# tusen-ai/RangeDet

Hardware: AMD Instinct MI355X
Metric: range-image frames/sec (64x2650, 8ch) at 1/2/4/8 GPU; Meta-Kernel HBM GB/s vs peak (higher is better)
Workload: dtype bf16

## Files before the change

### include/rangedet_hip.h

```cpp
#ifndef RANGEDET_HIP_H_
#define RANGEDET_HIP_H_
#include <stddef.h>
#include <stdint.h>

#ifdef __cplusplus
extern "C" {
#endif

#define RD_OK 0
#define RD_EINVAL (-1)
#define RD_ESHAPE (-2)
#define RD_EWORKSPACE (-3)
#define RD_EHIP (-4)

#define RD_F32 0
#define RD_BF16 1
#define RD_F16 2

#define RD_RELU_PRE 1
#define RD_ADD 2
#define RD_RELU_POST 4
#define RD_SCALE_FOLDED 8
#define RD_MFMA16 16

int rd_version(void);
const char* rd_last_error_string(void);

int rd_nchw_to_nhwc(const float* src, void* dst, int B, int C, int H, int W, int dst_cstride, int dst_coff,
                    int zero_pad, int dst_dtype, void* stream);
int rd_nhwc_to_nchw(const void* src, float* dst, int B, int C, int H, int W, int src_cstride, int src_coff,
                    int src_dtype, void* stream);

int rd_copy_rows(const void* src, long src_row_bytes, void* dst, long dst_row_bytes, long dst_offset_bytes, long bytes,
                 int rows, void* stream);

size_t rd_conv_packed_bytes(int ntaps, int cin, int cout, int dtype);
int rd_pack_conv_weight_host(const float* w_oihw_host, int cout, int cin, int kh, int kw, int dtype,
                             void* packed_host);
int rd_deconv_phase_taps(int kh, int kw, int stride_w, int pad_w, int phase);
int rd_pack_deconv_weight_host(const float* w_iohw_host, int cin, int cout, int kh, int kw, int stride_w,
                               int pad_w, int phase, int dtype, void* packed_host);
int rd_pack_deconv_weight_folded_host(const float* w_iohw_host, const float* fold_scale_host, int cin, int cout, int kh, int kw,
                                      int stride_w, int pad_w, int phase, int dtype, void* packed_host);

int rd_conv2d_bn_act(const void* x, int x_cstride, int x_coff, const void* w_packed, const float* scale,
                     const float* shift, const void* residual, int r_cstride, int r_coff, void* y,
                     int y_cstride, int y_coff, int B, int H, int Win, int cin, int cout, int kh, int kw,
                     int stride_w, int flags, int dtype, void* stream);
size_t rd_conv3x3_ex_packed_bytes(int cin, int cout, int stride_w, int x_cstride);
int rd_pack_conv3x3_ex_host(const float* w_oihw_host, const float* fold_scale_host, int cout, int cin, int stride_w,
                            int x_cstride, int dtype, void* packed_host);
int rd_pack_conv3x3_m16_host(const float* w_oihw_host, const float* fold_scale_host, int cout, int cin, int dtype, void* packed_host);
int rd_conv3x3_mfma16_ok(int cin, int cout, int stride_w, int W, int fused_output_conv);
size_t rd_conv1x1_sc_packed_bytes(int cin, int cout);
int rd_pack_conv1x1_sc_host(const float* w_oi_host, const float* fold_scale_host, int cout, int cin, int dtype,
                            void* packed_host);
int rd_conv3x3_bn_act_ex(const void* x, int x_cstride, int x_coff, const void* w_packed, const float* scale, const float* shift,
                         const void* residual, int r_cstride, int r_coff, const void* sc_x, int sc_cstride, int sc_coff,
                         int sc_cin, const void* sc_w_packed, void* y, int y_cstride, int y_coff, int B, int H, int Win, int cin,
                         int cout, int stride_w, int flags, int dtype, void* stream);
size_t rd_block64_packed_bytes(int cin);
int rd_pack_block64_host(const float* w1_oihw_host, const float* fold_scale1_host, const float* w2_oihw_host,
                         const float* fold_scale2_host, int cin, int dtype, void* packed_host);
int rd_block64_bn_act(const void* x, int x_cstride, int x_coff, int cin, const void* w_packed, const float* shift1, const float* shift2,
                      const void* sc_w_packed, void* y, int y_cstride, int y_coff, int B, int H, int W, int dtype, void* stream);
int rd_pack_block64_m16_host(const float* w1_oihw_host, const float* fold_scale1_host, const float* w2_oihw_host,
                             const float* fold_scale2_host, int dtype, void* packed_host);
int rd_pack_conv1x1_sc_m16_host(const float* w_oi_host, const float* fold_scale_host, int dtype, void* packed_host);
int rd_block64_m16_bn_act(const void* x, int x_cstride, int x_coff, const void* w_packed, const float* shift1, const float* shift2,
                          const void* sc_w_packed, void* y, int y_cstride, int y_coff, int B, int H, int W, int dtype, void* stream);

size_t rd_head_packed_bytes(void);
int rd_pack_head_weight_host(const float* w, int nout, int cin, int dtype, void* out_host);
size_t rd_head_m16_packed_bytes(void);
int rd_pack_head_weight_m16_host(const float* w, int nout, int cin, int dtype, void* out_host);
int rd_conv2d_bn_act_head_out(const void* x, int x_cstride, int x_coff, const void* w_packed, const float* scale,
                              const float* shift, int B, int H, int W, int cin, int flags, const void* head_w_packed,
                              const float* head_bias, float* out, long out_batch_stride, long n_off, int nout, int dtype,
                              void* stream);

int rd_conv3x3_bn_act_pair(const void* x0, int x0_coff, const void* w0_packed, const float* shift0, void* y0, int y0_coff,
                           const void* x1, int x1_coff, const void* w1_packed, const float* shift1, void* y1, int y1_coff,
                           int x_cstride, int y_cstride, int B, int H, int W, int cin, int flags, int dtype, void* stream);
int rd_conv2d_bn_act_head_out_pair(const void* x0, int x0_coff, const void* w0_packed, const float* shift0, const void* head_w0_packed,
                                   const float* head_bias0, float* out0, long out0_batch_stride, int nout0,
                                   const void* x1, int x1_coff, const void* w1_packed, const float* shift1, const void* head_w1_packed,
                                   const float* head_bias1, float* out1, long out1_batch_stride, int nout1,
                                   int x_cstride, long n_off, int B, int H, int W, int cin, int flags, int dtype, void* stream);

size_t rd_conv3x3_cat_packed_bytes(int cin1, int cin2, int cout);
int rd_pack_conv3x3_cat_host(const float* w, const float* fold_scale, int cout, int cin1, int cin2, int dtype, void* out_host);
int rd_conv3x3_bn_act_cat(const void* x1, int x1_cstride, int x1_coff, int cin1, const void* x2, int x2_cstride, int x2_coff, int cin2,
                          const void* w_packed, const float* shift, void* y, int y_cstride, int y_coff, int B, int H, int W, int cout,
                          int flags, int dtype, void* stream);

int rd_deconv2d_bn_act(const void* x, int x_cstride, int x_coff, const void* w_packed_phase,
                       const float* scale, const float* shift, const void* residual, int r_cstride,
                       int r_coff, void* y, int y_cstride, int y_coff, int B, int H, int Win, int cin,
                       int cout, int kh, int kw, int stride_w, int pad_w, int phase, int flags, int dtype,
                       void* stream);

int rd_deconv2d_all_phases_ok(int kh, int kw, int stride_w, int pad_w, int cout, int dtype);
int rd_deconv2d_bn_act_all(const void* x, int x_cstride, int x_coff, const void* w_packed_all, long w_phase_bytes,
                           const float* shift, const void* residual, int r_cstride, int r_coff, void* y, int y_cstride,
                           int y_coff, int B, int H, int Win, int cin, int cout, int kh, int kw, int stride_w, int pad_w,
                           int flags, int dtype, void* stream);

int rd_deconv2d_phase_pairs_ok(int kh, int kw, int stride_w, int pad_w, int cout, int dtype);
int rd_pack_deconv_phase_pair_host(const void* phase_a, const void* phase_b, int cin, int dtype, void* out);
int rd_deconv2d_bn_act_pairs(const void* x, int x_cstride, int x_coff, const void* w_packed_pairs, long w_pair_bytes,
                             const float* shift2, const void* residual, int r_cstride, int r_coff, void* y, int y_cstride,
                             int y_coff, int B, int H, int Win, int cin, int cout, int kh, int kw, int stride_w, int pad_w,
                             int flags, int dtype, void* stream);

int rd_head_out(const void* x, int x_cstride, int x_coff, const float* w, const float* bias, float* out,
                long out_batch_stride, long n_off, int B, int H, int W, int cin, int nout, int dtype,
                void* stream);

size_t rd_meta_packed_bytes(int dtype);
int rd_pack_meta_host(const float* w0, const float* b0, const float* w1, const float* b1, const float* s1,
                      const float* t1, const float* agg, const float* s2, const float* t2, int dtype,
                      void* packed_host);
int rd_meta_kernel_fwd(const void* data, int d_cstride, int d_coff, const float* coord_nchw,
                       const void* packed, void* y, int y_cstride, int y_coff, int B, int H, int W, int dtype,
                       void* stream);

size_t rd_sorted_foreground_workspace_bytes(long N, long k);
int rd_sorted_foreground(const float* cls_score, const float* bbox_delta, const float* pc, const float* mask,
                         int B, long N, long k, int D, int apply_sigmoid, float* out_score, float* out_delta,
                         float* out_pc, int* out_idx, void* ws, size_t ws_bytes, void* stream);

int rd_decode3d_bbox(const float* bbox_delta, const float* pc, float* out, int B, long N, int box_type,
                     int is_bin, void* stream);

size_t rd_score_filter_workspace_bytes(long n);
int rd_score_filter_dets(const float* scores, const float* boxes10, long n, float min_score, float* dets,
                         int* d_count, void* ws, size_t ws_bytes, void* stream);
int rd_score_filter_dets_batched(const float* scores, long scores_bstride, const float* boxes10, long boxes_bstride,
                                 long n, float min_score, float* dets, long dets_bstride, int* d_count, void* ws,
                                 size_t ws_bytes, int B, void* stream);

#define RD_WNMS_MAX_K 65536
#define RD_TIE_STABLE 0
#define RD_TIE_REFERENCE 1
#define RD_WNMS_DIAG_NO_SKIP 0x100
#define RD_WNMS_DIAG_TILE_W(n) (((n) & 0xff) << 16)
#define RD_WNMS_DIAG_MERGE_LDS(n) (((n) & 0x7f) << 24)
size_t rd_wnms_workspace_bytes(int Kcap);
int rd_wnms_4c(const float* dets, int Kcap, const int* d_count, const int* order, int tie_order, float thresh,
               float thresh_vote, int is3d, int hash_scale, float* out_dets, int* keep, int* d_nkeep, void* ws,
               size_t ws_bytes, void* stream);
int rd_wnms_4c_batched(const float* dets, long dets_bstride, int Kcap, const int* d_count, const int* order,
                       long order_bstride, int tie_order, float thresh, float thresh_vote, int is3d, int hash_scale,
                       float* out_dets, long out_bstride, int* keep, long keep_bstride, int* d_nkeep, void* ws,
                       size_t ws_bytes, int B, void* stream);
int rd_single_overlap(const float* dets_a, const float* dets_b, long n, int is3d, float* out, void* stream);
int rd_wnms_pair_skippable(const float* dets_a, const float* dets_b, long n, unsigned char* out, void* stream);

int rd_edge_atan2f(const float* y, const float* x, long n, float* out, void* stream);

int rd_wnms_order_host(const float* dets_host, int K, int* order_host);

int rd_dets12_to_8(const float* dets12, int Mcap, const int* d_count, float* out8, void* stream);
int rd_dets12_to_8_batched(const float* dets12, long dets12_bstride, int Mcap, const int* d_count, float* out8,
                           long out8_bstride, int B, void* stream);

int rd_rotated_iou_8pt(const float* boxes1, const float* boxes2, float* ious, long n1, long n2, void* stream);
int rd_batch_rotated_iou(const float* proposal, int p_stride, const float* gt_bbox, float* iou_map, int* argmax, int B, long N,
                         int n_gt, void* stream);
int rd_batch_rotated_iou_3d(const float* proposal, int p_stride, const float* gt_bbox7, float* iou_map, int* argmax, int B, long N,
                            int n_gt, void* stream);
int rd_rotated_iou_7(const float* boxes1, const float* boxes2, float* ious, long n1, long n2, void* stream);
int rd_batch_max_iou(const float* proposals, int p_stride, const float* gt8, float* out, long n, int n_gt,
                     void* stream);

size_t rd_nms3d_workspace_bytes(long N, int B);
int rd_gather_keep_scores(const float* score, long score_bstride, int k, const int* keep_idx, int max_keep, float* out, int B,
                          void* stream);
int rd_nms3d(const float* boxes, int B, long N, float iou_thres, int max_keep, int normal_iou, int* keep_idx,
             float* bbox_after_nms, void* ws, size_t ws_bytes, void* stream);

int rd_assign3d_v2(const float* pc, const float* bbox, const float* bbox_center, const float* bbox_radius, const float* mask,
                   const float* is_in_nlz, long N, int M, float max_x, float min_x, float max_y, float min_y, float max_z,
                   float min_z, float max_dist, int* out, void* stream);
size_t rd_get_point_num_workspace_bytes(void);
int rd_get_point_num(const float* bbox_inds, long N, float* out, void* ws, size_t ws_bytes, void* stream);

typedef struct {
  float clip_lo[7], clip_hi[7];
  float mean[8], sd[8];
  float interval_lo[3], interval_hi[3];
} rd_input_norm_t;
int rd_input_transform(const float* range_image, const float* pc_vehicle_frame, const float* inclination,
                       const rd_input_norm_t* norm_host, int B, int H, int W, int Hp, int Wp, float* input_data,
                       float* coord_s1, float* pc_s1, float* pc_s2, float* pc_s4, float* mask_s1, float* mask_s2,
                       float* mask_s4, void* stream);

typedef struct {
  float *input_data, *coord_s1;
  float *pc[3], *mask[3];
  float *reg_target[3], *reg_weight[3], *reg_normalize_weight[3], *cls_target[3];
  int* bbox3d_ind;
} rd_train_outputs_t;
size_t rd_train_transform_workspace_bytes(int B);
int rd_train_transform(const float* range_image, const float* pc_vehicle_frame, const float* inclination,
                       const rd_input_norm_t* norm_host, const float* gt_bbox_imu, const float* gt_bbox_center,
                       const float* gt_limits, const float* gt_bbox_csa, const int* num_gt_host, int Mmax, float radius,
                       float max_dist, const float* reg_weight_host, int B, int H, int W, int Hp, int Wp,
                       const rd_train_outputs_t* out_host, void* ws, size_t ws_bytes, void* stream);

#define RD_PROF_CONV 0
#define RD_PROF_META 1
#define RD_PROF_HEAD_OUT 2
#define RD_PROF_SORT 3
#define RD_PROF_DECODE 4
#define RD_PROF_WNMS 5
#define RD_PROF_LAYOUT 6
#define RD_PROF_CONV3 7
#define RD_PROF_BLOCK 8
#define RD_PROF_NKINDS 9
int rd_prof_enable(int on);
int rd_prof_reset(void);
int rd_prof_get(int kind, double* total_ms, long* launches);

#ifdef __cplusplus
}
#endif
#endif
```

### rangedet_amd/csrc/k_misc.h

```cpp
#pragma once
#include "rd_common.h"

namespace rd {

template <int DT>
__global__ __launch_bounds__(256) void nchw_to_nhwc_kernel(const float* __restrict__ src, void* __restrict__ dst_, int C,
                                                           long HW, int cs, int coff, int cpad, long total) {
  using E = Elem<DT>;
  typename E::T* dst = (typename E::T*)dst_;
  const int ctot = C + cpad;
  for (long i = blockIdx.x * 256L + threadIdx.x; i < total; i += (long)gridDim.x * 256) {
    long p = i % HW;
    long rest = i / HW;
    int c = (int)(rest % ctot);
    long b = rest / ctot;
    float v = c < C ? src[(b * C + c) * HW + p] : 0.f;
    dst[(b * HW + p) * cs + coff + c] = E::from_f32(v);
  }
}
template <int DT, int NSLOT>
__global__ __launch_bounds__(256) void nchw_to_nhwc_px_kernel(const float* __restrict__ src, void* __restrict__ dst_, int C,
                                                              long HW, int cs, int coff, long npix) {
  using E = Elem<DT>;
  typename E::T* dst = (typename E::T*)dst_;
  for (long i = blockIdx.x * 256L + threadIdx.x; i < npix; i += (long)gridDim.x * 256) {
    const long b = i / HW, p = i - b * HW;
    typename E::T v[NSLOT * E::CH];
#pragma unroll
    for (int c = 0; c < NSLOT * E::CH; ++c) v[c] = E::from_f32(c < C ? src[(b * C + c) * HW + p] : 0.f);
    Slot16 pk[NSLOT];
    memcpy(pk, v, sizeof(pk));
#pragma unroll
    for (int u = 0; u < NSLOT; ++u) *(Slot16*)(dst + i * cs + coff + u * E::CH) = pk[u];
  }
}
template <int DT>
__global__ __launch_bounds__(256) void nhwc_to_nchw_kernel(const void* __restrict__ src_, float* __restrict__ dst, int C,
                                                           long HW, int cs, int coff, long total) {
  using E = Elem<DT>;
  const typename E::T* src = (const typename E::T*)src_;
  for (long i = blockIdx.x * 256L + threadIdx.x; i < total; i += (long)gridDim.x * 256) {
    long p = i % HW;
    long rest = i / HW;
    int c = (int)(rest % C);
    long b = rest / C;
    dst[(b * C + c) * HW + p] = E::to_f32(src[(b * HW + p) * cs + coff + c]);
  }
}

template <int DT, int NOUT>
__global__ __launch_bounds__(256) void head_out_kernel(const void* __restrict__ x_, int cs, int coff,
                                                       const float* __restrict__ w, const float* __restrict__ bias,
                                                       float* __restrict__ out, long out_bs, long n_off, long HW,
                                                       int cin) {
  using E = Elem<DT>;
  using T = typename E::T;
  __shared__ float wl[8 * 128];
  const T* x = (const T*)x_ + (size_t)blockIdx.y * HW * cs;
  for (int i = threadIdx.x; i < NOUT * cin; i += 256) wl[i] = w[i];
  __syncthreads();
  const int sub = threadIdx.x & 7;
  const int per = cin >> 3;
  const long npix_iter = (long)gridDim.x * 32;
  for (long p0 = blockIdx.x * 32L; p0 < HW; p0 += npix_iter) {
    long p = p0 + (threadIdx.x >> 3);
    float acc[NOUT];
#pragma unroll
    for (int o = 0; o < NOUT; ++o) acc[o] = 0.f;
    if (p < HW) {
      const T* px = x + p * cs + coff + sub * per;
      if ((per % E::CH) == 0) {
        for (int c0 = 0; c0 < per; c0 += E::CH) {
          const Slot16 raw = *(const Slot16*)(px + c0);
          T el[E::CH];
          memcpy(el, &raw, 16);
#pragma unroll
          for (int e = 0; e < E::CH; ++e) {
            const float v = E::to_f32(el[e]);
#pragma unroll
            for (int o = 0; o < NOUT; ++o) acc[o] += v * wl[o * cin + sub * per + c0 + e];
          }
        }
      } else {
        for (int c = 0; c < per; ++c) {
          float v = E::to_f32(px[c]);
#pragma unroll
          for (int o = 0; o < NOUT; ++o) acc[o] += v * wl[o * cin + sub * per + c];
        }
      }
    }
#pragma unroll
    for (int o = 0; o < NOUT; ++o) {
      acc[o] += __shfl_xor(acc[o], 1);
      acc[o] += __shfl_xor(acc[o], 2);
      acc[o] += __shfl_xor(acc[o], 4);
    }
    if (p < HW && sub == 0) {
      float* o_ = out + (size_t)blockIdx.y * out_bs + (n_off + p) * NOUT;
#pragma unroll
      for (int o = 0; o < NOUT; ++o) o_[o] = acc[o] + bias[o];
    }
  }
}

template <int NOUT, int DT = RD_BF16>
__global__ __launch_bounds__(256) void head_out_mfma_kernel(const bf16_t* __restrict__ x, int cs, int coff,
                                                            const float* __restrict__ w, const float* __restrict__ bias,
                                                            float* __restrict__ out, long out_bs, long n_off, long HW,
                                                            int cin) {
  __shared__ __attribute__((aligned(16))) unsigned char lds[4 * 8192];
  const int lane = threadIdx.x & 63, m = lane & 31, hi = lane >> 5, wv = threadIdx.x >> 6;
  unsigned char* img = lds + wv * 8192;
  const int nks = cin >> 4, nsl = cin >> 3;
  x += (size_t)blockIdx.y * HW * cs + coff;
  out += (size_t)blockIdx.y * out_bs + n_off * NOUT;
  s16x8 wh[8], wl[8];
#pragma unroll
  for (int ks = 0; ks < 8; ++ks) {
    unsigned short h[8], l[8];
#pragma unroll
    for (int j = 0; j < 8; ++j) {
      const float v = (m < NOUT && ks < nks) ? w[m * cin + ks * 16 + hi * 8 + j] : 0.f;
      h[j] = H16<DT>::from_f32(v);
      l[j] = H16<DT>::from_f32(v - H16<DT>::to_f32(h[j]));
    }
    memcpy(&wh[ks], h, 16);
    memcpy(&wl[ks], l, 16);
  }
  float bs[4];
#pragma unroll
  for (int r = 0; r < 4; ++r) bs[r] = 4 * hi + r < NOUT ? bias[4 * hi + r] : 0.f;
  const long ntile = (HW + 31) / 32;
  const long wave0 = (long)blockIdx.x * 4 + wv, nwave = (long)gridDim.x * 4;
  const int lp = lane >> 4, ls = lane & 15;
  auto load = [&](long tile, Slot16 (&v)[8]) {
#pragma unroll
    for (int it = 0; it < 8; ++it) {
      const long p = min(tile * 32 + it * 4 + lp, HW - 1);
      v[it] = ls < nsl ? *(const Slot16*)(x + p * cs + ls * 8) : Slot16{0u, 0u, 0u, 0u};
    }
  };
  Slot16 cur[8], nxt[8];
  if (wave0 < ntile) load(wave0, cur);
  for (long tile = wave0; tile < ntile; tile += nwave) {
    const bool more = tile + nwave < ntile;
    if (more) load(tile + nwave, nxt);
#pragma unroll
    for (int it = 0; it < 8; ++it) {
      const int pr = it * 4 + lp;
      *(Slot16*)(img + pr * 256 + ((ls ^ (pr & 15)) << 4)) = cur[it];
    }
    __builtin_amdgcn_wave_barrier();
    f32x16 acc;
#pragma unroll
    for (int r = 0; r < 16; ++r) acc[r] = 0.f;
#pragma unroll
    for (int ks = 0; ks < 8; ++ks) {
      const s16x8 b = *(const s16x8*)(img + m * 256 + (((2 * ks + hi) ^ (m & 15)) << 4));
      acc = H16<DT>::mfma(wl[ks], b, acc);
      acc = H16<DT>::mfma(wh[ks], b, acc);
    }
    __builtin_amdgcn_wave_barrier();
    const long p = tile * 32 + m;
    if (p < HW) {
      float* o = out + p * NOUT + 4 * hi;
#pragma unroll
      for (int r = 0; r < 4; ++r)
        if (4 * hi + r < NOUT) o[r] = acc[r] + bs[r];
    }
    if (more) {
#pragma unroll
      for (int it = 0; it < 8; ++it) cur[it] = nxt[it];
    }
  }
}

__global__ __launch_bounds__(256) void decode3d_kernel(const float* __restrict__ delta, const float* __restrict__ pc,
                                                       float* __restrict__ out, long n, int box_type, int is_bin) {
  long idx = blockIdx.x * 256L + threadIdx.x;
  if (idx >= n) return;
  const float* d = delta + idx * box_type;
  float pc_x = pc[idx * 3 + 0], pc_y = pc[idx * 3 + 1], pc_z = pc[idx * 3 + 2];
  float az = atan2f(pc_y, pc_x);
  float ca = cosf(az), sa = sinf(az);
  float dx, dy, width, length, height, z0, yaw_l;
  if (is_bin) {
    dx = d[0];
    dy = d[1];
    width = expf(d[3]);
    length = expf(d[4]);
    height = expf(d[5]);
    float cz = pc_z + d[2];
    z0 = (float)((double)cz - (double)height / 2.0);
    yaw_l = d[6] + az;
  } else {
    dx = d[0] * fabsf(d[0]);
    dy = d[1] * fabsf(d[1]);
    width = expf(d[2]);
    length = expf(d[3]);
    height = expf(d[7]);
    z0 = d[6];
    yaw_l = atan2f(d[5], d[4]) + az;
  }
  float dxl = dx * ca - dy * sa;
  float dyl = dx * sa + dy * ca;
  float cx = pc_x + dxl, cy = pc_y + dyl;
  float sy = sinf(yaw_l), cyw = cosf(yaw_l);
  float hl = (float)(0.5 * (double)length), hw = (float)(0.5 * (double)width);
  float hx[4] = {hl, -hl, -hl, hl};
  float hy[4] = {-hw, -hw, hw, hw};
  float* o = out + idx * 10;
#pragma unroll
  for (int k = 0; k < 4; ++k) {
    o[2 * k] = (hx[k] * cyw - hy[k] * sy) + cx;
    o[2 * k + 1] = (hx[k] * sy + hy[k] * cyw) + cy;
  }
  o[8] = z0;
  o[9] = z0 + height;
}

__global__ __launch_bounds__(256) void filter_count_kernel(const float* __restrict__ scores, long n, float thr,
                                                           int* __restrict__ blk_cnt, long sc_bs, long blk_bs) {
  scores += blockIdx.y * sc_bs;
  blk_cnt += blockIdx.y * blk_bs;
  long i = blockIdx.x * 256L + threadIdx.x;
  int p = (i < n) && (scores[i] > thr);
  unsigned long long m = __ballot(p);
  __shared__ int wc[4];
  if ((threadIdx.x & 63) == 0) wc[threadIdx.x >> 6] = __popcll(m);
  __syncthreads();
  if (threadIdx.x == 0) blk_cnt[blockIdx.x] = wc[0] + wc[1] + wc[2] + wc[3];
}
__global__ __launch_bounds__(256) void filter_scan_kernel(int* __restrict__ blk_cnt, int nblk, int* __restrict__ total,
                                                          long blk_bs) {
  blk_cnt += blockIdx.x * blk_bs;
  total += blockIdx.x;
  __shared__ int part[256];
  __shared__ int carry;
  if (threadIdx.x == 0) carry = 0;
  __syncthreads();
  for (int base = 0; base < nblk; base += 256) {
    int i = base + threadIdx.x;
    int v = i < nblk ? blk_cnt[i] : 0;
    part[threadIdx.x] = v;
    __syncthreads();
    for (int off = 1; off < 256; off <<= 1) {
      int t = threadIdx.x >= off ? part[threadIdx.x - off] : 0;
      __syncthreads();
      part[threadIdx.x] += t;
      __syncthreads();
    }
    int incl = part[threadIdx.x];
    if (i < nblk) blk_cnt[i] = carry + incl - v;
    __syncthreads();
    if (threadIdx.x == 255) carry += incl;
    __syncthreads();
  }
  if (threadIdx.x == 0) *total = carry;
}
__global__ __launch_bounds__(256) void filter_scatter_kernel(const float* __restrict__ scores,
                                                             const float* __restrict__ boxes10, long n, float thr,
                                                             const int* __restrict__ blk_off, float* __restrict__ dets,
                                                             long sc_bs, long box_bs, long blk_bs, long dets_bs) {
  scores += blockIdx.y * sc_bs;
  boxes10 += blockIdx.y * box_bs;
  blk_off += blockIdx.y * blk_bs;
  dets += blockIdx.y * dets_bs;
  long i = blockIdx.x * 256L + threadIdx.x;
  int p = (i < n) && (scores[i] > thr);
  unsigned long long m = __ballot(p);
  __shared__ int wc[4];
  const int wv = threadIdx.x >> 6, ln = threadIdx.x & 63;
  if (ln == 0) wc[wv] = __popcll(m);
  __syncthreads();
  int off = blk_off[blockIdx.x];
  for (int w = 0; w < wv; ++w) off += wc[w];
  if (p) {
    int pos = off + __popcll(m & ((1ull << ln) - 1ull));
    const float* b = boxes10 + i * 10;
    float* d = dets + (size_t)pos * 12;
#pragma unroll
    for (int k = 0; k < 8; ++k) d[k] = b[k];
    d[8] = fdlibm_atan2f(b[1] - b[3], b[0] - b[2]);
    d[9] = b[8];
    d[10] = b[9] - b[8];
    d[11] = scores[i];
  }
}

__global__ __launch_bounds__(256) void dets12_to_8_kernel(const float* __restrict__ d12, int cap, const int* __restrict__ d_count,
                                                          float* __restrict__ o8, long d12_bs, long o8_bs) {
  d12 += blockIdx.y * d12_bs;
  o8 += blockIdx.y * o8_bs;
  int i = blockIdx.x * 256 + threadIdx.x;
  int n = d_count ? min(d_count[blockIdx.y], cap) : cap;
  if (i >= n) return;
  const float* d = d12 + (size_t)i * 12;
  float* o = o8 + (size_t)i * 8;
  o[0] = (d[0] + d[2] + d[4] + d[6]) / 4.f;
  o[1] = (d[1] + d[3] + d[5] + d[7]) / 4.f;
  o[2] = d[9] + d[10] / 2.f;
  float ax = d[2] - d[0], ay = d[3] - d[1];
  float bx = d[2] - d[4], by = d[3] - d[5];
  o[3] = sqrtf(ax * ax + ay * ay);
  o[4] = sqrtf(bx * bx + by * by);
  o[5] = d[10];
  o[6] = d[8];
  o[7] = d[11];
}

__global__ __launch_bounds__(256) void gather_keep_scores_kernel(const float* __restrict__ score, long score_bs, int k,
                                                                 const int* __restrict__ keep, int mk, float* __restrict__ out) {
  const int i = blockIdx.x * 256 + threadIdx.x;
  if (i >= mk) return;
  const int q = keep[(size_t)blockIdx.y * mk + i];
  out[(size_t)blockIdx.y * mk + i] = (q >= 0 && q < k) ? score[blockIdx.y * score_bs + q] : -__builtin_inff();
}

}
```

### rangedet_amd/csrc/k_sort.h

```cpp
#pragma once
#include "rd_common.h"

namespace rd {

constexpr int SORT_TILE = 2048;

__device__ __forceinline__ unsigned desc_key(float f) {
  unsigned u = __float_as_uint(f);
  unsigned asc = u ^ ((u >> 31) ? 0xFFFFFFFFu : 0x80000000u);
  return ~asc;
}
__device__ __forceinline__ float key_to_float(unsigned key) {
  unsigned asc = ~key;
  unsigned u = (asc >> 31) ? (asc ^ 0x80000000u) : ~asc;
  return __uint_as_float(u);
}

__global__ __launch_bounds__(256) void sort_keygen_kernel(const float* __restrict__ score, const float* __restrict__ mask,
                                                          long N, int apply_sigmoid, unsigned* __restrict__ keys,
                                                          unsigned* __restrict__ idx, long ws_stride) {
  long i = blockIdx.x * 256L + threadIdx.x;
  if (i >= N) return;
  const long b = blockIdx.y;
  float s = score[b * N + i];
  if (apply_sigmoid) s = 1.0f / (1.0f + expf(-s));
  if (mask) s = s * mask[b * N + i];
  keys[b * ws_stride + i] = desc_key(s);
  idx[b * ws_stride + i] = (unsigned)i;
}
__global__ __launch_bounds__(256) void sort_keygen_dets_kernel(const float* __restrict__ dets, int cap,
                                                               const int* __restrict__ d_count, unsigned* __restrict__ keys,
                                                               unsigned* __restrict__ idx) {
  int i = blockIdx.x * 256 + threadIdx.x;
  if (i >= cap) return;
  int n = d_count ? min(*d_count, cap) : cap;
  keys[i] = i < n ? desc_key(dets[(size_t)i * 12 + 11]) : 0xFFFFFFFFu;
  idx[i] = (unsigned)i;
}

__global__ __launch_bounds__(256) void sort_hist_kernel(const unsigned* __restrict__ keys, long N, int shift,
                                                        unsigned* __restrict__ hist, unsigned* __restrict__ tot,
                                                        long ws_stride, const unsigned* __restrict__ d_n) {
  if (d_n) N = min(N, (long)d_n[blockIdx.y * ws_stride]);
  keys += blockIdx.y * ws_stride;
  hist += blockIdx.y * ws_stride;
  tot += blockIdx.y * ws_stride;
  __shared__ unsigned h[256];
  h[threadIdx.x] = 0;
  __syncthreads();
  long base = (long)blockIdx.x * SORT_TILE;
  for (int r = 0; r < SORT_TILE / 256; ++r) {
    long i = base + r * 256 + threadIdx.x;
    if (i < N) atomicAdd(&h[(keys[i] >> shift) & 255u], 1u);
  }
  __syncthreads();
  unsigned v = h[threadIdx.x];
  hist[(size_t)blockIdx.x * 256 + threadIdx.x] = v;
  if (v) atomicAdd(&tot[threadIdx.x], v);
}

__global__ __launch_bounds__(256) void sort_scatter_kernel(const unsigned* __restrict__ keys_in,
                                                           const unsigned* __restrict__ idx_in, long N, int shift,
                                                           const unsigned* __restrict__ hist,
                                                           const unsigned* __restrict__ tot,
                                                           unsigned* __restrict__ keys_out, unsigned* __restrict__ idx_out,
                                                           long ws_stride, const unsigned* __restrict__ d_n) {
  if (d_n) {
    N = min(N, (long)d_n[blockIdx.y * ws_stride]);
    if ((long)blockIdx.x * SORT_TILE >= N) return;
  }
  {
    const long o = blockIdx.y * ws_stride;
    keys_in += o; idx_in += o; hist += o; tot += o; keys_out += o; idx_out += o;
  }
  __shared__ unsigned wcnt[4][256];
  __shared__ unsigned gbase[256];
  __shared__ unsigned scan[256];
  const int tid = threadIdx.x, lane = tid & 63, wv = tid >> 6;
  for (int w = 0; w < 4; ++w) wcnt[w][tid] = 0;
  {
    unsigned t = tot[tid];
    scan[tid] = t;
    __syncthreads();
    for (int off = 1; off < 256; off <<= 1) {
      unsigned a = tid >= off ? scan[tid - off] : 0u;
      __syncthreads();
      scan[tid] += a;
      __syncthreads();
    }
    unsigned before = 0;
    for (unsigned b = 0; b < blockIdx.x; ++b) before += hist[(size_t)b * 256 + tid];
    gbase[tid] = scan[tid] - t + before;
  }
  __syncthreads();

  unsigned key[8], id[8], pos[8];
  const long base = (long)blockIdx.x * SORT_TILE + wv * 512;
  const unsigned long long lt = (1ull << lane) - 1ull;
#pragma unroll
  for (int r = 0; r < 8; ++r) {
    long i = base + r * 64 + lane;
    bool valid = i < N;
    key[r] = valid ? keys_in[i] : 0xFFFFFFFFu;
    id[r] = valid ? idx_in[i] : 0u;
    unsigned d = (key[r] >> shift) & 255u;
    unsigned long long peers = __ballot(valid);
#pragma unroll
    for (int bit = 0; bit < 8; ++bit) {
      unsigned long long bm = __ballot(valid && ((d >> bit) & 1u));
      peers &= ((d >> bit) & 1u) ? bm : ~bm;
    }
    unsigned rank = __popcll(peers & lt), cnt = __popcll(peers);
    unsigned prev = wcnt[wv][d];
    pos[r] = prev + rank;
    __builtin_amdgcn_wave_barrier();
    if (valid && rank == 0) wcnt[wv][d] = prev + cnt;
    __builtin_amdgcn_wave_barrier();
  }
  __syncthreads();
  {
    unsigned c0 = wcnt[0][tid], c1 = wcnt[1][tid], c2 = wcnt[2][tid];
    wcnt[0][tid] = 0;
    wcnt[1][tid] = c0;
    wcnt[2][tid] = c0 + c1;
    wcnt[3][tid] = c0 + c1 + c2;
  }
  __syncthreads();
#pragma unroll
  for (int r = 0; r < 8; ++r) {
    long i = base + r * 64 + lane;
    if (i < N) {
      unsigned d = (key[r] >> shift) & 255u;
      unsigned dst = gbase[d] + wcnt[wv][d] + pos[r];
      keys_out[dst] = key[r];
      idx_out[dst] = id[r];
    }
  }
}

__global__ __launch_bounds__(256) void sort_gather_kernel(const unsigned* __restrict__ keys, const unsigned* __restrict__ idx,
                                                          long k, int D, const float* __restrict__ delta,
                                                          const float* __restrict__ pc, float* __restrict__ out_score,
                                                          float* __restrict__ out_delta, float* __restrict__ out_pc,
                                                          int* __restrict__ out_idx, long ws_stride, long N) {
  long i = blockIdx.x * 256L + threadIdx.x;
  if (i >= k) return;
  {
    const long b = blockIdx.y;
    keys += b * ws_stride; idx += b * ws_stride;
    delta += b * N * D; pc += b * N * 3;
    out_score += b * k; out_delta += b * k * D; out_pc += b * k * 3;
    if (out_idx) out_idx += b * k;
  }
  unsigned j = idx[i];
// ... 18 lines not shown
    if (i < N) atomicAdd(&h[keys[i] >> SEL_SHIFT], 1u);
  }
  __syncthreads();
  for (int i = threadIdx.x; i < SEL_BINS; i += 256)
    if (h[i]) atomicAdd(&h12[i], h[i]);
}
__global__ __launch_bounds__(256) void select_thresh_kernel(const unsigned* __restrict__ h12, long k, unsigned* __restrict__ sel,
                                                            long ws_stride) {
  h12 += blockIdx.y * ws_stride; sel += blockIdx.y * ws_stride;
  __shared__ unsigned part[256];
  const int tid = threadIdx.x;
  unsigned loc[SEL_BINS / 256], sum = 0;
#pragma unroll
  for (int j = 0; j < SEL_BINS / 256; ++j) { loc[j] = h12[tid * (SEL_BINS / 256) + j]; sum += loc[j]; }
  part[tid] = sum;
  __syncthreads();
  for (int off = 1; off < 256; off <<= 1) {
    const unsigned v = tid >= off ? part[tid - off] : 0u;
    __syncthreads();
    part[tid] += v;
    __syncthreads();
  }
  unsigned before = part[tid] - sum;
  if (tid == 255 && (k == 0 || part[255] < (unsigned)k)) { sel[0] = SEL_BINS - 1; sel[1] = part[255]; }
  if (before < (unsigned)k && before + sum >= (unsigned)k) {
#pragma unroll
    for (int j = 0; j < SEL_BINS / 256; ++j) {
      if (before < (unsigned)k && before + loc[j] >= (unsigned)k) { sel[0] = tid * (SEL_BINS / 256) + j; sel[1] = before + loc[j]; }
      before += loc[j];
    }
  }
}
__global__ __launch_bounds__(256) void select_count_kernel(const unsigned* __restrict__ keys, long N, const unsigned* __restrict__ sel,
                                                           unsigned* __restrict__ cnt, long ws_stride) {
  keys += blockIdx.y * ws_stride; sel += blockIdx.y * ws_stride; cnt += blockIdx.y * ws_stride;
  const unsigned T = sel[0];
  __shared__ unsigned c;
  if (threadIdx.x == 0) c = 0;
  __syncthreads();
  const long base = (long)blockIdx.x * SORT_TILE;
  unsigned mine = 0;
  for (int r = 0; r < SORT_TILE / 256; ++r) {
    const long i = base + r * 256 + threadIdx.x;
    if (i < N && (keys[i] >> SEL_SHIFT) <= T) ++mine;
  }
  if (mine) atomicAdd(&c, mine);
  __syncthreads();
  if (threadIdx.x == 0) cnt[blockIdx.x] = c;
}
__global__ __launch_bounds__(256) void select_compact_kernel(const unsigned* __restrict__ keys_in, const unsigned* __restrict__ idx_in,
                                                             long N, const unsigned* __restrict__ sel,
                                                             const unsigned* __restrict__ cnt, unsigned* __restrict__ keys_out,
                                                             unsigned* __restrict__ idx_out, long ws_stride) {
  {
    const long o = blockIdx.y * ws_stride;
    keys_in += o; idx_in += o; sel += o; cnt += o; keys_out += o; idx_out += o;
  }
  const unsigned T = sel[0];
  __shared__ unsigned wcnt[4][8], sbase;
  const int tid = threadIdx.x, lane = tid & 63, wv = tid >> 6;
  if (tid == 0) {
    unsigned b = 0;
    for (unsigned j = 0; j < blockIdx.x; ++j) b += cnt[j];
    sbase = b;
  }
  const long base = (long)blockIdx.x * SORT_TILE + wv * 512;
  unsigned key[8], id[8];
  unsigned long long m[8];
#pragma unroll
  for (int r = 0; r < 8; ++r) {
    const long i = base + r * 64 + lane;
    const bool valid = i < N;
    key[r] = valid ? keys_in[i] : 0xFFFFFFFFu;
    id[r] = valid ? idx_in[i] : 0u;
    m[r] = __ballot(valid && (key[r] >> SEL_SHIFT) <= T);
    if (lane == 0) wcnt[wv][r] = (unsigned)__popcll(m[r]);
  }
  __syncthreads();
  unsigned off = sbase;
  for (int w = 0; w < wv; ++w)
#pragma unroll
    for (int r = 0; r < 8; ++r) off += wcnt[w][r];
#pragma unroll
  for (int r = 0; r < 8; ++r) {
    if ((m[r] >> lane) & 1ull) {
      const unsigned dst = off + (unsigned)__popcll(m[r] & ((1ull << lane) - 1ull));
      keys_out[dst] = key[r];
      idx_out[dst] = id[r];
    }
    off += (unsigned)__popcll(m[r]);
  }
}

struct SortWs {
  unsigned *keysA, *keysB, *idxA, *idxB, *hist, *tot, *h12, *cnt, *sel;
  int nblk;
};
inline size_t sort_ws_bytes(long N) {
  long nblk = (N + SORT_TILE - 1) / SORT_TILE;
  return (size_t)(4 * N + nblk * 256 + 4 * 256 + SEL_BINS + nblk + 64) * 4 + 256;
}
inline SortWs sort_ws_carve(void* ws, long N) {
  SortWs s;
  s.nblk = (int)((N + SORT_TILE - 1) / SORT_TILE);
  unsigned* p = (unsigned*)ws;
  s.keysA = p; p += N;
  s.keysB = p; p += N;
  s.idxA = p; p += N;
  s.idxB = p; p += N;
  s.hist = p; p += (size_t)s.nblk * 256;
  s.tot = p; p += 4 * 256;
  s.h12 = p; p += SEL_BINS;
  s.cnt = p; p += s.nblk;
  s.sel = p;
  return s;
}
inline int sort_clear(const SortWs& s, hipStream_t st, int nb, long ws_stride, bool with_h12) {
  const size_t bytes = (size_t)(4 * 256 + (with_h12 ? SEL_BINS : 0)) * 4;
  const hipError_t e = nb > 1 ? hipMemset2DAsync(s.tot, (size_t)ws_stride * 4, 0, bytes, nb, st) : hipMemsetAsync(s.tot, 0, bytes, st);
  return e == hipSuccess ? RD_OK : fail(RD_EHIP, "sort: memset");
}
inline int radix_sort_pairs(const SortWs& s, long N, hipStream_t st, int nb = 1, long ws_stride = 0, const unsigned* d_n = nullptr,
                            bool cleared = false) {
  if (!cleared) { int rc = sort_clear(s, st, nb, ws_stride, false); if (rc != RD_OK) return rc; }
  unsigned *ki = s.keysA, *ko = s.keysB, *ii = s.idxA, *io = s.idxB;
  for (int pass = 0; pass < 4; ++pass) {
    hipLaunchKernelGGL(sort_hist_kernel, dim3(s.nblk, nb), dim3(256), 0, st, ki, N, pass * 8, s.hist, s.tot + pass * 256,
                       ws_stride, d_n);
    hipLaunchKernelGGL(sort_scatter_kernel, dim3(s.nblk, nb), dim3(256), 0, st, ki, ii, N, pass * 8, s.hist,
                       s.tot + pass * 256, ko, io, ws_stride, d_n);
    std::swap(ki, ko);
    std::swap(ii, io);
  }
  return check_launch("radix_sort_pairs");
}

inline int radix_topk_pairs(const SortWs& s, long N, long k, hipStream_t st, int nb, long ws_stride, unsigned** rk, unsigned** ri) {
  const bool off = dev_switches().sort_no_select;
  *rk = s.keysA; *ri = s.idxA;
  RD_REQUIRE(k > 0 && k <= N, RD_ESHAPE, "top-k: k %ld of N %ld", k, N);
  if (off || 2 * k > N) return radix_sort_pairs(s, N, st, nb, ws_stride);
  { int rc = sort_clear(s, st, nb, ws_stride, true); if (rc != RD_OK) return rc; }
  hipLaunchKernelGGL(select_hist_kernel, dim3(s.nblk, nb), dim3(256), 0, st, s.keysA, N, s.h12, ws_stride);
  hipLaunchKernelGGL(select_thresh_kernel, dim3(1, nb), dim3(256), 0, st, s.h12, k, s.sel, ws_stride);
  hipLaunchKernelGGL(select_count_kernel, dim3(s.nblk, nb), dim3(256), 0, st, s.keysA, N, s.sel, s.cnt, ws_stride);
  hipLaunchKernelGGL(select_compact_kernel, dim3(s.nblk, nb), dim3(256), 0, st, s.keysA, s.idxA, N, s.sel, s.cnt, s.keysB, s.idxB,
                     ws_stride);
  SortWs v = s;
  v.keysA = s.keysB; v.keysB = s.keysA; v.idxA = s.idxB; v.idxB = s.idxA;
  *rk = s.keysB; *ri = s.idxB;
  return radix_sort_pairs(v, N, st, nb, ws_stride, s.sel + 1, true);
}

}
```

### rangedet_amd/csrc/rd_api.hip

```cpp
#include "k_conv1.h"
#include "k_block.h"
#include "k_assign.h"
#include "k_input.h"
#include "k_target.h"
#include "k_nms3d.h"
#include "k_meta.h"
#include "k_misc.h"
#include "k_riou.h"
#include "k_sort.h"
#include "k_wnms.h"

#include <algorithm>
#include <string>
#include <numeric>

using namespace rd;

namespace rd {
inline size_t align256(size_t v) { return (v + 255) & ~(size_t)255; }
inline size_t wnms_ws_bytes(int cap) {
  const size_t nw = (size_t)(cap + 63) / 64;
  return align256((size_t)cap * PREP_F * 4) + 3 * align256((size_t)cap * nw * 8) + 4 * align256((size_t)cap * 4) +
         align256(((size_t)cap + 2) * 8 + 3 * ((size_t)cap / 32 + 2) * 4) + align256(nw * 8) + 256 + align256(sort_ws_bytes(cap)) + 256;
}
// ... 544 lines not shown
  allow_conv_lds();
  Conv3Phases ph;
  ph.nph = stride_w / 2; ph.ts_mask = 0; ph.y_pc = 2 * cout; ph.r_pc = 2 * cout; ph.w_pb = w_pair_bytes;
  for (int p = 0; p < stride_w; p += 2)
    if (deconv_tap_set(deconv_taps_sorted(kh, kw, stride_w, pad_w, p)) == 2) ph.ts_mask |= 1 << (p / 2);
  return launch_conv3(x, x_cstride, x_coff, w_packed_pairs, nullptr, shift2, residual, r_cstride * stride_w, r_coff, y, y_cstride * stride_w,
                      y_coff, B, H, Win, cin, 2 * cout, flags, 1, (hipStream_t)stream, 3, nullptr, dtype, nullptr, &ph);
}

int rd_head_out(const void* x, int x_cstride, int x_coff, const float* w, const float* bias, float* out,
                long out_batch_stride, long n_off, int B, int H, int W, int cin, int nout, int dtype, void* stream) {
  RD_REQUIRE(x && w && bias && out, RD_EINVAL, "head_out: null pointer");
  RD_REQUIRE(cin % 8 == 0 && cin <= 128 && cin > 0, RD_ESHAPE, "head_out: cin %d (multiple of 8, <= 128)", cin);
  RD_REQUIRE(nout == 1 || nout == 7 || nout == 8, RD_ESHAPE, "head_out: nout %d not in {1,7,8}", nout);
  RD_REQUIRE(dtype == RD_F32 || is_h16(dtype), RD_EINVAL, "head_out: dtype");
  hipStream_t st = (hipStream_t)stream;
  const long HW = (long)H * W;
  dim3 grid((unsigned)std::min<long>((HW + 31) / 32, 4096), B);
  ProfScope ps(RD_PROF_HEAD_OUT, st);
  if (is_h16(dtype) && nout > 1 && cin % 16 == 0 && x_cstride % 8 == 0 && x_coff % 8 == 0) {
    dim3 g2((unsigned)std::min<long>((HW + 127) / 128, 2048), B);
#define RD_HOM(NO, DT_) hipLaunchKernelGGL((head_out_mfma_kernel<NO, DT_>), g2, dim3(256), 0, st, (const bf16_t*)x, x_cstride, x_coff, w, bias, out, out_batch_stride, n_off, HW, cin)
    if (dtype == RD_F16) { if (nout == 7) RD_HOM(7, RD_F16); else RD_HOM(8, RD_F16); }
    else { if (nout == 7) RD_HOM(7, RD_BF16); else RD_HOM(8, RD_BF16); }
#undef RD_HOM
    return check_launch("head_out");
  }
#define RD_HO(DT, NO) hipLaunchKernelGGL((head_out_kernel<DT, NO>), grid, dim3(256), 0, st, x, x_cstride, x_coff, w, bias, out, out_batch_stride, n_off, HW, cin)
  if (dtype == RD_BF16) { if (nout == 1) RD_HO(RD_BF16, 1); else if (nout == 7) RD_HO(RD_BF16, 7); else RD_HO(RD_BF16, 8); }
  else if (dtype == RD_F16) { if (nout == 1) RD_HO(RD_F16, 1); else if (nout == 7) RD_HO(RD_F16, 7); else RD_HO(RD_F16, 8); }
  else { if (nout == 1) RD_HO(RD_F32, 1); else if (nout == 7) RD_HO(RD_F32, 7); else RD_HO(RD_F32, 8); }
#undef RD_HO
  return check_launch("head_out");
}

size_t rd_meta_packed_bytes(int dtype) { return meta_layout(dtype).total; }
int rd_pack_meta_host(const float* w0, const float* b0, const float* w1, const float* b1, const float* s1,
                      const float* t1, const float* agg, const float* s2, const float* t2, int dtype, void* out) {
  RD_REQUIRE(w0 && b0 && w1 && b1 && s1 && t1 && agg && s2 && t2 && out, RD_EINVAL, "pack_meta: null pointer");
  RD_REQUIRE(dtype == RD_F32 || is_h16(dtype), RD_EINVAL, "pack_meta: dtype");
  pack_meta(w0, b0, w1, b1, s1, t1, agg, s2, t2, dtype, out);
  return RD_OK;
}
int rd_meta_kernel_fwd(const void* data, int d_cstride, int d_coff, const float* coord_nchw, const void* packed,
                       void* y, int y_cstride, int y_coff, int B, int H, int W, int dtype, void* stream) {
  RD_REQUIRE(data && coord_nchw && packed && y, RD_EINVAL, "meta_kernel: null pointer");
  RD_REQUIRE(B > 0 && H > 0 && W > 0, RD_ESHAPE, "meta_kernel: empty shape");
  RD_REQUIRE(dtype == RD_F32 || is_h16(dtype), RD_EINVAL, "meta_kernel: dtype");
  const int ch = ch_per_slot(dtype);
  RD_REQUIRE(d_cstride % ch == 0 && d_coff % ch == 0 && y_cstride % ch == 0 && y_coff % ch == 0, RD_ESHAPE,
             "meta_kernel: channel strides/offsets must be 16-byte multiples");
  RD_REQUIRE(d_coff + 64 <= d_cstride && y_coff + 64 <= y_cstride, RD_ESHAPE, "meta_kernel: needs 64 channels");
  hipStream_t st = (hipStream_t)stream;
  MetaArgs a;
  a.data = data; a.d_cs = d_cstride; a.d_co = d_coff; a.coord = coord_nchw; a.packed = (const unsigned char*)packed;
  a.y = y; a.y_cs = y_cstride; a.y_co = y_coff; a.B = B; a.H = H; a.W = W;
  constexpr int WAVES = 8;
  a.tiles_h = (H + WAVES - 1) / WAVES;
  a.tiles_w = (W + 31) / 32;
  a.ntiles = B * a.tiles_h * a.tiles_w;
  a.r0 = 0; a.m0 = a.m1 = a.m2 = 0;
  const size_t consts = 9 * 64 * 4 * 2 + 1024;
  ProfScope ps(RD_PROF_META, st);
  if (is_h16(dtype)) {
    const size_t lds = meta_layout(dtype).wbytes + consts + (size_t)(WAVES + 2) * 34 * 128 + 4096;
    static std::atomic<unsigned long long> seen{0};
    once_per_device(seen, [] { allow_big_lds(meta16_kernel<WAVES, RD_BF16>); allow_big_lds(meta16_kernel<WAVES, RD_F16>); });
    const dim3 mgrid(std::min(a.ntiles, conv_num_cus())), mblock(WAVES * 64);
    const int strips = a.tiles_w * B;
    a.r0 = dev_switches().conv_xcd && strips % 8 == 0 ? 8 : strips;
    RD_REQUIRE((unsigned long long)a.ntiles * (unsigned)std::max(a.r0, std::max(a.tiles_h, a.tiles_w)) < (1ull << 32), RD_ESHAPE,
               "meta_kernel: %d tiles exceed the range of the tile decode", a.ntiles);
    a.m0 = meta_magic(a.r0); a.m1 = meta_magic(a.tiles_h); a.m2 = meta_magic(a.tiles_w);
    RD_REQUIRE((long)H * W < (1l << 23) && (long)H * W * d_cstride < (1l << 31) && W < (1 << 23) && d_cstride < (1 << 23), RD_ESHAPE,
               "meta_kernel: image of %d x %d pixels x %d channels exceeds the 32-bit halo offsets", H, W, d_cstride);
    if (dtype == RD_F16) hipLaunchKernelGGL((meta16_kernel<WAVES, RD_F16>), mgrid, mblock, lds, st, a);
    else hipLaunchKernelGGL((meta16_kernel<WAVES, RD_BF16>), mgrid, mblock, lds, st, a);
  } else {
    const size_t lds = consts + (size_t)(WAVES + 2) * 34 * 256;
    static std::atomic<unsigned long long> seen32{0};
    once_per_device(seen32, [] { allow_big_lds(meta_kernel<RD_F32, WAVES>); });
    hipLaunchKernelGGL((meta_kernel<RD_F32, WAVES>), dim3(std::min(a.ntiles, 512)), dim3(WAVES * 64), lds, st, a);
  }
  return check_launch("meta_kernel");
}

size_t rd_sorted_foreground_workspace_bytes(long N, long k) { (void)k; return (sort_ws_bytes(N) + 256 + 255) & ~(size_t)255; }
int rd_sorted_foreground(const float* cls_score, const float* bbox_delta, const float* pc, const float* mask, int B,
                         long N, long k, int D, int apply_sigmoid, float* out_score, float* out_delta, float* out_pc,
                         int* out_idx, void* ws, size_t ws_bytes, void* stream) {
  RD_REQUIRE(cls_score && bbox_delta && pc && out_score && out_delta && out_pc && ws, RD_EINVAL, "sorted_foreground: null pointer");
  RD_REQUIRE(B > 0 && N > 0 && k > 0 && D > 0, RD_ESHAPE, "sorted_foreground: empty shape");
  RD_REQUIRE(N >= k, RD_ESHAPE, "sorted_foreground: N (%ld) < num_fgs (%ld)", N, k);
  RD_REQUIRE(N < (1L << 31), RD_ESHAPE, "sorted_foreground: N too large");
  RD_REQUIRE(ws_bytes >= rd_sorted_foreground_workspace_bytes(N, k), RD_EWORKSPACE, "sorted_foreground: workspace %zu < %zu",
             ws_bytes, rd_sorted_foreground_workspace_bytes(N, k));
  hipStream_t st = (hipStream_t)stream;
  void* wsa = (void*)(((uintptr_t)ws + 255) & ~(uintptr_t)255);
  SortWs s = sort_ws_carve(wsa, N);
  ProfScope ps(RD_PROF_SORT, st);
  const size_t per = rd_sorted_foreground_workspace_bytes(N, k);
  const bool wide = ws_bytes >= per * (size_t)B;
  const long stride = wide ? (long)(per / 4) : 0;
  const int nb = wide ? B : 1;
  for (int b0 = 0; b0 < B; b0 += nb) {
    hipLaunchKernelGGL(sort_keygen_kernel, dim3((unsigned)((N + 255) / 256), nb), dim3(256), 0, st, cls_score + (size_t)b0 * N,
                       mask ? mask + (size_t)b0 * N : nullptr, N, apply_sigmoid, s.keysA, s.idxA, stride);
    unsigned *rk, *ri;
    int rc = radix_topk_pairs(s, N, k, st, nb, stride, &rk, &ri);
    if (rc != RD_OK) return rc;
    hipLaunchKernelGGL(sort_gather_kernel, dim3((unsigned)((k + 255) / 256), nb), dim3(256), 0, st, rk, ri, k, D,
                       bbox_delta + (size_t)b0 * N * D, pc + (size_t)b0 * N * 3, out_score + (size_t)b0 * k,
                       out_delta + (size_t)b0 * k * D, out_pc + (size_t)b0 * k * 3, out_idx ? out_idx + (size_t)b0 * k : nullptr,
                       stride, N);
  }
  return check_launch("sorted_foreground");
}

int rd_decode3d_bbox(const float* bbox_delta, const float* pc, float* out, int B, long N, int box_type, int is_bin,
                     void* stream) {
  RD_REQUIRE(bbox_delta && pc && out, RD_EINVAL, "decode3d: null pointer");
  RD_REQUIRE(B > 0 && N > 0, RD_ESHAPE, "decode3d: empty shape");
  RD_REQUIRE((is_bin && box_type == 7) || (!is_bin && box_type == 8), RD_ESHAPE,
             "decode3d: box_type %d with is_bin=%d (8 for regular, 7 for bin)", box_type, is_bin);
  hipStream_t st = (hipStream_t)stream;
  const long n = (long)B * N;
  ProfScope ps(RD_PROF_DECODE, st);
  hipLaunchKernelGGL(decode3d_kernel, dim3((unsigned)((n + 255) / 256)), dim3(256), 0, st, bbox_delta, pc, out, n, box_type, is_bin);
  return check_launch("decode3d");
}

size_t rd_score_filter_workspace_bytes(long n) { return (size_t)((n + 255) / 256 + 8) * 4 + 256; }
int rd_score_filter_dets_batched(const float* scores, long scores_bstride, const float* boxes10, long boxes_bstride,
                                 long n, float min_score, float* dets, long dets_bstride, int* d_count, void* ws,
                                 size_t ws_bytes, int B, void* stream) {
  RD_REQUIRE(scores && boxes10 && dets && d_count && ws, RD_EINVAL, "score_filter: null pointer");
  RD_REQUIRE(n > 0 && B > 0, RD_ESHAPE, "score_filter: empty input");
  const size_t per = rd_score_filter_workspace_bytes(n);
  RD_REQUIRE(ws_bytes >= per * (size_t)B, RD_EWORKSPACE, "score_filter: workspace %zu < %zu", ws_bytes, per * (size_t)B);
  hipStream_t st = (hipStream_t)stream;
  int* blk = (int*)(((uintptr_t)ws + 255) & ~(uintptr_t)255);
  const int nblk = (int)((n + 255) / 256);
  const long blk_bs = nblk + 8;
  ProfScope ps(RD_PROF_WNMS, st);
  hipLaunchKernelGGL(filter_count_kernel, dim3(nblk, B), dim3(256), 0, st, scores, n, min_score, blk, scores_bstride, blk_bs);
  hipLaunchKernelGGL(filter_scan_kernel, dim3(B), dim3(256), 0, st, blk, nblk, d_count, blk_bs);
  hipLaunchKernelGGL(filter_scatter_kernel, dim3(nblk, B), dim3(256), 0, st, scores, boxes10, n, min_score, blk, dets,
                     scores_bstride, boxes_bstride, blk_bs, dets_bstride);
  return check_launch("score_filter");
}
int rd_score_filter_dets(const float* scores, const float* boxes10, long n, float min_score, float* dets, int* d_count,
                         void* ws, size_t ws_bytes, void* stream) {
  return rd_score_filter_dets_batched(scores, 0, boxes10, 0, n, min_score, dets, 0, d_count, ws, ws_bytes, 1, stream);
}

size_t rd_wnms_workspace_bytes(int Kcap) { return Kcap > 0 ? wnms_ws_bytes(Kcap) : 0; }
int rd_wnms_4c_batched(const float* dets, long dets_bstride, int Kcap, const int* d_count, const int* order,
                       long order_bstride, int tie_order, float thresh, float thresh_vote, int is3d, int hash_scale,
                       float* out_dets, long out_bstride, int* keep, long keep_bstride, int* d_nkeep, void* ws,
                       size_t ws_bytes, int B, void* stream) {
  RD_REQUIRE(dets && out_dets && keep && d_nkeep && ws, RD_EINVAL, "wnms_4c: null pointer");
  RD_REQUIRE(Kcap > 0 && Kcap <= RD_WNMS_MAX_K, RD_ESHAPE, "wnms_4c: Kcap %d not in [1, %d]", Kcap, RD_WNMS_MAX_K);
  RD_REQUIRE(B > 0, RD_ESHAPE, "wnms_4c: batch %d", B);
  const int diag = tie_order & ~0xff;
  tie_order &= 0xff;
  RD_REQUIRE(tie_order == RD_TIE_STABLE || tie_order == RD_TIE_REFERENCE, RD_EINVAL, "wnms_4c: tie_order %d", tie_order);
  RD_REQUIRE(!(diag & ~(RD_WNMS_DIAG_NO_SKIP | (0xff << 16) | (0x7f << 24))), RD_EINVAL, "wnms_4c: unknown diagnostic bits 0x%x", diag);
  const size_t per = rd_wnms_workspace_bytes(Kcap);
  RD_REQUIRE(ws_bytes >= per * (size_t)B, RD_EWORKSPACE, "wnms_4c: workspace %zu < %zu", ws_bytes, per * (size_t)B);
  RD_REQUIRE(order || B == 1 || tie_order == RD_TIE_REFERENCE, RD_EINVAL,
             "wnms_4c: the batched call needs an explicit processing order or RD_TIE_REFERENCE");
  hipStream_t st = (hipStream_t)stream;
  static std::atomic<unsigned long long> seen_lds{0};
  once_per_device(seen_lds, [] {
    allow_big_lds(wnms_tie_order_kernel); allow_big_lds(wnms_scan_kernel); allow_big_lds(wnms_scan4_kernel); allow_big_lds(wnms_merge_kernel);
  });
  WnmsWs w = wnms_ws_carve(ws, Kcap);
  ProfScope ps(RD_PROF_WNMS, st);
  WnmsBatch bs;
  bs.dets = dets_bstride; bs.order = order_bstride; bs.prep = (long)(per / 4); bs.words = (long)(per / 8);
  bs.ints = (long)(per / 4); bs.keep = keep_bstride; bs.out = out_bstride;
  const int* ord = order;
  if (!ord && tie_order == RD_TIE_REFERENCE) {
    const size_t lds = TIE_STACK_BYTES + (Kcap <= TIE_LDS_K ? (size_t)Kcap * 8 + 3 * ((size_t)Kcap / 32 + 2) * 4 : 0);
    hipLaunchKernelGGL(wnms_tie_order_kernel, dim3(1, 1, B), dim3(256), lds, st, dets, Kcap, d_count, w.order, bs, (long)(per / 4),
                       w.scratch);
    ord = w.order;
    bs.order = (long)(per / 4);
  } else if (!ord) {
    void* swa = (void*)(((uintptr_t)w.sort_ws + 255) & ~(uintptr_t)255);
    SortWs s = sort_ws_carve(swa, Kcap);
    hipLaunchKernelGGL(sort_keygen_dets_kernel, dim3((Kcap + 255) / 256), dim3(256), 0, st, dets, Kcap, d_count, s.keysA, s.idxA);
    int rc = radix_sort_pairs(s, Kcap, st);
    if (rc != RD_OK) return rc;
    if (hipMemcpyAsync(w.order, s.idxA, (size_t)Kcap * 4, hipMemcpyDeviceToDevice, st) != hipSuccess)
      return rd::fail(RD_EHIP, "wnms_4c: order copy");
    ord = w.order;
    bs.order = 0;
  }
  const int nb = (Kcap + 63) / 64;
  hipLaunchKernelGGL(wnms_prep_kernel, dim3((Kcap + 255) / 256, 1, B), dim3(256), 0, st, dets, ord, Kcap, d_count, w.prep, bs,
                     (float)hash_scale, w.novf);
  const int e_tw = (diag >> 16) & 0xff, e_ml = (diag >> 24) & 0x7f;
  const int tile_w = std::min(w.nwcap, e_tw ? std::max(1, e_tw) : 256);
  const size_t scan_lds = ((size_t)w.nwcap + (size_t)64 * tile_w) * 8;
  const int R1 = 256, nb1 = R1 / 64;
  const bool one_round = dev_switches().wnms_one_round;
  const bool two = Kcap >= 4 * R1 && !one_round;
  const int ct = dev_switches().wnms_ct == 32 ? 32 : dev_switches().wnms_ct == 16 ? 16 : 8;
  const int pgrid = std::min(2048, std::max(64, nb * (64 / ct) * std::min(nb, 16)));
  const int allow_skip = thresh >= 1e-3f && thresh_vote >= 1e-3f && !is3d && !dev_switches().wnms_no_skip && !(diag & RD_WNMS_DIAG_NO_SKIP);
  auto pairs = [&](const int* rows, const int* nrows, const unsigned long long* supp, int rb_end) {
    auto k = dev_switches().wnms_bal ? (ct == 8 ? wnms_pairs_kernel<8, true> : ct == 16 ? wnms_pairs_kernel<16, true> : wnms_pairs_kernel<32, true>)
                                     : (ct == 8 ? wnms_pairs_kernel<8, false> : ct == 16 ? wnms_pairs_kernel<16, false> : wnms_pairs_kernel<32, false>);
    hipLaunchKernelGGL(k, dim3(pgrid, 1, B), dim3(64), 0, st, w.prep, Kcap, d_count, thresh, thresh_vote, is3d, w.thr, w.vote,
                       w.nwcap, bs, rows, nrows, supp, 0, rb_end, allow_skip);
  };
  pairs(nullptr, nullptr, nullptr, two ? nb1 : nb);
  const bool scan4 = w.nwcap <= 128 && !e_tw && !dev_switches().wnms_scan1;
  const int tile_words = 64 * 128;
  const size_t scan4_lds = ((size_t)w.nwcap + tile_words) * 8;
  auto scan = [&](int c_begin, int c_end, unsigned long long* state) {
    if (scan4)
      hipLaunchKernelGGL(wnms_scan4_kernel, dim3(1, 1, B), dim3(256), scan4_lds, st, w.thr, w.snap, Kcap, d_count, w.nwcap, ord,
                         w.keep_q, keep, d_nkeep, bs, c_begin, c_end, state, tile_words);
    else
      hipLaunchKernelGGL(wnms_scan_kernel, dim3(1, 1, B), dim3(64), scan_lds, st, w.thr, w.snap, Kcap, d_count, w.nwcap, ord,
                         w.keep_q, keep, d_nkeep, bs, c_begin, c_end, state, tile_w);
  };
  scan(0, two ? nb1 : nb, two ? w.supp_state : (unsigned long long*)nullptr);
  if (two) {
    hipLaunchKernelGGL(wnms_alive_kernel, dim3(1, 1, B), dim3(256), 0, st, w.supp_state, Kcap, d_count, R1, w.alive, w.nalive, bs);
    pairs((const int*)w.alive, (const int*)w.nalive, (const unsigned long long*)w.supp_state, 0);
    scan(nb1, nb, w.supp_state);
  }
  const int lds_cap = std::min(Kcap + 2, e_ml ? std::max(4, e_ml) : 2048);
  hipLaunchKernelGGL(wnms_merge_kernel, dim3(std::min(Kcap, 4096), 1, B), dim3(64), (size_t)lds_cap * 8, st, dets, ord, w.vote,
                     w.snap, Kcap, d_count, w.nwcap, w.keep_q, d_nkeep, out_dets, bs, lds_cap, w.ovf, w.novf);
  if (Kcap + 2 > lds_cap)
    hipLaunchKernelGGL(wnms_merge_big_kernel, dim3(1, 1, B), dim3(64), 0, st, dets, ord, w.vote, w.snap, Kcap, d_count, w.nwcap,
                       w.keep_q, out_dets, bs, (const int*)w.ovf, (const int*)w.novf, w.scratch);
  return check_launch("wnms_4c");
}
int rd_wnms_4c(const float* dets, int Kcap, const int* d_count, const int* order, int tie_order, float thresh,
               float thresh_vote, int is3d, int hash_scale, float* out_dets, int* keep, int* d_nkeep, void* ws,
               size_t ws_bytes, void* stream) {
  return rd_wnms_4c_batched(dets, 0, Kcap, d_count, order, 0, tie_order, thresh, thresh_vote, is3d, hash_scale, out_dets, 0,
                            keep, 0, d_nkeep, ws, ws_bytes, 1, stream);
}
int rd_single_overlap(const float* dets_a, const float* dets_b, long n, int is3d, float* out, void* stream) {
  RD_REQUIRE(n >= 0 && (n == 0 || (dets_a && dets_b && out)), RD_EINVAL, "single_overlap: bad arguments");
  if (n == 0) return RD_OK;
  hipLaunchKernelGGL(single_overlap_kernel, dim3((unsigned)((n + 63) / 64)), dim3(64), 0, (hipStream_t)stream, dets_a, dets_b, n,
                     is3d, out);
  return check_launch("single_overlap");
}
int rd_wnms_pair_skippable(const float* dets_a, const float* dets_b, long n, unsigned char* out, void* stream) {
  RD_REQUIRE(dets_a && dets_b && out && n >= 0, RD_EINVAL, "wnms_pair_skippable: null pointer");
  if (n == 0) return RD_OK;
  hipLaunchKernelGGL(pair_skippable_kernel, dim3((unsigned)((n + 63) / 64)), dim3(64), 0, (hipStream_t)stream, dets_a, dets_b, n, out);
  return check_launch("wnms_pair_skippable");
}
namespace rd {
__global__ void atan2f_kernel(const float* y, const float* x, long n, float* out) {
  const long i = (long)blockIdx.x * blockDim.x + threadIdx.x;
  if (i < n) out[i] = fdlibm_atan2f(y[i], x[i]);
}
}
int rd_edge_atan2f(const float* y, const float* x, long n, float* out, void* stream) {
  RD_REQUIRE(y && x && out && n >= 0, RD_EINVAL, "edge_atan2f: null pointer");
  if (n == 0) return RD_OK;
  hipLaunchKernelGGL(atan2f_kernel, dim3((unsigned)((n + 255) / 256)), dim3(256), 0, (hipStream_t)stream, y, x, n, out);
  return check_launch("edge_atan2f");
}
int rd_wnms_order_host(const float* dets_host, int K, int* order_host) {
  RD_REQUIRE(K >= 0 && (K == 0 || (dets_host && order_host)), RD_EINVAL, "wnms_order_host: bad arguments");
  std::iota(order_host, order_host + K, 0);
  std::sort(order_host, order_host + K, [&](int i, int j) { return dets_host[i * 12 + 11] > dets_host[j * 12 + 11]; });
  return RD_OK;
}

int rd_dets12_to_8_batched(const float* dets12, long dets12_bstride, int Mcap, const int* d_count, float* out8,
                           long out8_bstride, int B, void* stream) {
  RD_REQUIRE(dets12 && out8, RD_EINVAL, "dets12_to_8: null pointer");
  RD_REQUIRE(Mcap > 0 && B > 0, RD_ESHAPE, "dets12_to_8: empty input");
  hipLaunchKernelGGL(dets12_to_8_kernel, dim3((Mcap + 255) / 256, B), dim3(256), 0, (hipStream_t)stream, dets12, Mcap, d_count,
                     out8, dets12_bstride, out8_bstride);
  return check_launch("dets12_to_8");
}
int rd_dets12_to_8(const float* dets12, int Mcap, const int* d_count, float* out8, void* stream) {
  return rd_dets12_to_8_batched(dets12, 0, Mcap, d_count, out8, 0, 1, stream);
}

int rd_gather_keep_scores(const float* score, long score_bstride, int k, const int* keep_idx, int max_keep, float* out, int B,
                          void* stream) {
  RD_REQUIRE(score && keep_idx && out, RD_EINVAL, "gather_keep_scores: null pointer");
  RD_REQUIRE(k > 0 && max_keep > 0 && B > 0, RD_ESHAPE, "gather_keep_scores: empty input");
  hipLaunchKernelGGL(gather_keep_scores_kernel, dim3((max_keep + 255) / 256, B), dim3(256), 0, (hipStream_t)stream, score,
                     score_bstride, k, keep_idx, max_keep, out);
  return check_launch("gather_keep_scores");
}

int rd_rotated_iou_8pt(const float* boxes1, const float* boxes2, float* ious, long n1, long n2, void* stream) {
  RD_REQUIRE(boxes1 && boxes2 && ious, RD_EINVAL, "rotated_iou: null pointer");
  RD_REQUIRE(n1 > 0 && n2 > 0, RD_ESHAPE, "rotated_iou: empty input");
  hipLaunchKernelGGL(riou8_kernel, dim3((unsigned)((n1 * n2 + 255) / 256)), dim3(256), 0, (hipStream_t)stream, boxes1, boxes2, ious, n1, n2);
// ... 184 lines not shown
```

### rangedet_amd/lib.py

```python
import ctypes
import os

import numpy as np

RD_OK, RD_EINVAL, RD_ESHAPE, RD_EWORKSPACE, RD_EHIP = 0, -1, -2, -3, -4
RD_F32, RD_BF16, RD_F16 = 0, 1, 2
H16 = (RD_BF16, RD_F16)
RD_RELU_PRE, RD_ADD, RD_RELU_POST, RD_SCALE_FOLDED, RD_MFMA16 = 1, 2, 4, 8, 16
RD_WNMS_MAX_K = 65536
RD_WNMS_DIAG_NO_SKIP = 0x100


def RD_WNMS_DIAG_TILE_W(n):
    return (n & 0xff) << 16


def RD_WNMS_DIAG_MERGE_LDS(n):
    return (n & 0x7f) << 24

RD_TIE_STABLE, RD_TIE_REFERENCE = 0, 1
PROF_KINDS = {"conv": 0, "meta": 1, "head_out": 2, "sort": 3, "decode": 4, "wnms": 5, "layout": 6, "conv3": 7, "block": 8}

_HERE = os.path.dirname(os.path.abspath(__file__))
DEFAULT_PATH = os.environ.get("RANGEDET_HIP_LIB") or os.path.join(_HERE, "librangedet_hip.so")

c_int, c_long, c_float, c_size_t, c_void_p = ctypes.c_int, ctypes.c_long, ctypes.c_float, ctypes.c_size_t, ctypes.c_void_p

SIGNATURES = {
    "rd_version": (c_int, []),
    "rd_last_error_string": (ctypes.c_char_p, []),
    "rd_nchw_to_nhwc": (c_int, [c_void_p, c_void_p, c_int, c_int, c_int, c_int, c_int, c_int, c_int, c_int, c_void_p]),
    "rd_nhwc_to_nchw": (c_int, [c_void_p, c_void_p, c_int, c_int, c_int, c_int, c_int, c_int, c_int, c_void_p]),
    "rd_copy_rows": (c_int, [c_void_p, c_long, c_void_p, c_long, c_long, c_long, c_int, c_void_p]),
    "rd_conv_packed_bytes": (c_size_t, [c_int, c_int, c_int, c_int]),
    "rd_pack_conv_weight_host": (c_int, [c_void_p, c_int, c_int, c_int, c_int, c_int, c_void_p]),
    "rd_deconv_phase_taps": (c_int, [c_int, c_int, c_int, c_int, c_int]),
    "rd_pack_deconv_weight_host": (c_int, [c_void_p, c_int, c_int, c_int, c_int, c_int, c_int, c_int, c_int, c_void_p]),
    "rd_pack_deconv_weight_folded_host": (c_int, [c_void_p, c_void_p, c_int, c_int, c_int, c_int, c_int, c_int, c_int, c_int, c_void_p]),
    "rd_conv2d_bn_act": (c_int, [c_void_p, c_int, c_int, c_void_p, c_void_p, c_void_p, c_void_p, c_int, c_int, c_void_p,
                                 c_int, c_int, c_int, c_int, c_int, c_int, c_int, c_int, c_int, c_int, c_int, c_int, c_void_p]),
    "rd_conv3x3_ex_packed_bytes": (c_size_t, [c_int, c_int, c_int, c_int]),
    "rd_pack_conv3x3_ex_host": (c_int, [c_void_p, c_void_p, c_int, c_int, c_int, c_int, c_int, c_void_p]),
    "rd_pack_conv3x3_m16_host": (c_int, [c_void_p, c_void_p, c_int, c_int, c_int, c_void_p]),
    "rd_conv3x3_mfma16_ok": (c_int, [c_int, c_int, c_int, c_int, c_int]),
    "rd_conv1x1_sc_packed_bytes": (c_size_t, [c_int, c_int]),
    "rd_pack_conv1x1_sc_host": (c_int, [c_void_p, c_void_p, c_int, c_int, c_int, c_void_p]),
    "rd_conv3x3_bn_act_ex": (c_int, [c_void_p, c_int, c_int, c_void_p, c_void_p, c_void_p, c_void_p, c_int, c_int, c_void_p, c_int,
                                     c_int, c_int, c_void_p, c_void_p, c_int, c_int, c_int, c_int, c_int, c_int, c_int, c_int,
                                     c_int, c_int, c_void_p]),
    "rd_deconv2d_bn_act": (c_int, [c_void_p, c_int, c_int, c_void_p, c_void_p, c_void_p, c_void_p, c_int, c_int, c_void_p,
                                   c_int, c_int, c_int, c_int, c_int, c_int, c_int, c_int, c_int, c_int, c_int, c_int,
                                   c_int, c_int, c_void_p]),
    "rd_conv3x3_cat_packed_bytes": (c_size_t, [c_int, c_int, c_int]),
    "rd_pack_conv3x3_cat_host": (c_int, [c_void_p, c_void_p, c_int, c_int, c_int, c_int, c_void_p]),
    "rd_conv3x3_bn_act_cat": (c_int, [c_void_p, c_int, c_int, c_int, c_void_p, c_int, c_int, c_int, c_void_p, c_void_p, c_void_p, c_int, c_int,
                                      c_int, c_int, c_int, c_int, c_int, c_int, c_void_p]),
    "rd_deconv2d_all_phases_ok": (c_int, [c_int, c_int, c_int, c_int, c_int, c_int]),
    "rd_deconv2d_bn_act_all": (c_int, [c_void_p, c_int, c_int, c_void_p, c_long, c_void_p, c_void_p, c_int, c_int, c_void_p,
                                       c_int, c_int, c_int, c_int, c_int, c_int, c_int, c_int, c_int, c_int, c_int, c_int,
                                       c_int, c_void_p]),
    "rd_deconv2d_phase_pairs_ok": (c_int, [c_int, c_int, c_int, c_int, c_int, c_int]),
    "rd_pack_deconv_phase_pair_host": (c_int, [c_void_p, c_void_p, c_int, c_int, c_void_p]),
    "rd_deconv2d_bn_act_pairs": (c_int, [c_void_p, c_int, c_int, c_void_p, c_long, c_void_p, c_void_p, c_int, c_int, c_void_p,
                                         c_int, c_int, c_int, c_int, c_int, c_int, c_int, c_int, c_int, c_int, c_int, c_int,
                                         c_int, c_void_p]),
    "rd_block64_packed_bytes": (c_size_t, [c_int]),
    "rd_pack_block64_host": (c_int, [c_void_p, c_void_p, c_void_p, c_void_p, c_int, c_int, c_void_p]),
    "rd_pack_block64_m16_host": (c_int, [c_void_p, c_void_p, c_void_p, c_void_p, c_int, c_void_p]),
    "rd_pack_conv1x1_sc_m16_host": (c_int, [c_void_p, c_void_p, c_int, c_void_p]),
    "rd_block64_m16_bn_act": (c_int, [c_void_p, c_int, c_int, c_void_p, c_void_p, c_void_p, c_void_p, c_void_p, c_int, c_int, c_int, c_int,
                                      c_int, c_int, c_void_p]),
    "rd_block64_bn_act": (c_int, [c_void_p, c_int, c_int, c_int, c_void_p, c_void_p, c_void_p, c_void_p, c_void_p, c_int, c_int, c_int, c_int,
                                  c_int, c_int, c_void_p]),
    "rd_head_packed_bytes": (c_size_t, []),
    "rd_head_m16_packed_bytes": (c_size_t, []),
    "rd_pack_head_weight_host": (c_int, [c_void_p, c_int, c_int, c_int, c_void_p]),
    "rd_pack_head_weight_m16_host": (c_int, [c_void_p, c_int, c_int, c_int, c_void_p]),
    "rd_conv2d_bn_act_head_out": (c_int, [c_void_p, c_int, c_int, c_void_p, c_void_p, c_void_p, c_int, c_int, c_int, c_int, c_int,
                                          c_void_p, c_void_p, c_void_p, c_long, c_long, c_int, c_int, c_void_p]),
    "rd_conv3x3_bn_act_pair": (c_int, [c_void_p, c_int, c_void_p, c_void_p, c_void_p, c_int] * 2 +
                               [c_int, c_int, c_int, c_int, c_int, c_int, c_int, c_int, c_void_p]),
    "rd_conv2d_bn_act_head_out_pair": (c_int, [c_void_p, c_int, c_void_p, c_void_p, c_void_p, c_void_p, c_void_p, c_long, c_int] * 2 +
                                       [c_int, c_long, c_int, c_int, c_int, c_int, c_int, c_int, c_void_p]),
    "rd_head_out": (c_int, [c_void_p, c_int, c_int, c_void_p, c_void_p, c_void_p, c_long, c_long, c_int, c_int, c_int,
                            c_int, c_int, c_int, c_void_p]),
    "rd_meta_packed_bytes": (c_size_t, [c_int]),
    "rd_pack_meta_host": (c_int, [c_void_p] * 9 + [c_int, c_void_p]),
    "rd_meta_kernel_fwd": (c_int, [c_void_p, c_int, c_int, c_void_p, c_void_p, c_void_p, c_int, c_int, c_int, c_int,
                                   c_int, c_int, c_void_p]),
    "rd_sorted_foreground_workspace_bytes": (c_size_t, [c_long, c_long]),
    "rd_sorted_foreground": (c_int, [c_void_p, c_void_p, c_void_p, c_void_p, c_int, c_long, c_long, c_int, c_int,
                                     c_void_p, c_void_p, c_void_p, c_void_p, c_void_p, c_size_t, c_void_p]),
    "rd_decode3d_bbox": (c_int, [c_void_p, c_void_p, c_void_p, c_int, c_long, c_int, c_int, c_void_p]),
    "rd_score_filter_workspace_bytes": (c_size_t, [c_long]),
    "rd_score_filter_dets": (c_int, [c_void_p, c_void_p, c_long, c_float, c_void_p, c_void_p, c_void_p, c_size_t, c_void_p]),
    "rd_score_filter_dets_batched": (c_int, [c_void_p, c_long, c_void_p, c_long, c_long, c_float, c_void_p, c_long, c_void_p,
                                             c_void_p, c_size_t, c_int, c_void_p]),
    "rd_wnms_workspace_bytes": (c_size_t, [c_int]),
    "rd_wnms_4c_batched": (c_int, [c_void_p, c_long, c_int, c_void_p, c_void_p, c_long, c_int, c_float, c_float, c_int, c_int,
                                   c_void_p, c_long, c_void_p, c_long, c_void_p, c_void_p, c_size_t, c_int, c_void_p]),
    "rd_dets12_to_8_batched": (c_int, [c_void_p, c_long, c_int, c_void_p, c_void_p, c_long, c_int, c_void_p]),
    "rd_wnms_4c": (c_int, [c_void_p, c_int, c_void_p, c_void_p, c_int, c_float, c_float, c_int, c_int, c_void_p, c_void_p,
                           c_void_p, c_void_p, c_size_t, c_void_p]),
    "rd_single_overlap": (c_int, [c_void_p, c_void_p, c_long, c_int, c_void_p, c_void_p]),
    "rd_wnms_order_host": (c_int, [c_void_p, c_int, c_void_p]),
    "rd_edge_atan2f": (c_int, [c_void_p, c_void_p, c_long, c_void_p, c_void_p]),
    "rd_wnms_pair_skippable": (c_int, [c_void_p, c_void_p, c_long, c_void_p, c_void_p]),
    "rd_dets12_to_8": (c_int, [c_void_p, c_int, c_void_p, c_void_p, c_void_p]),
    "rd_rotated_iou_8pt": (c_int, [c_void_p, c_void_p, c_void_p, c_long, c_long, c_void_p]),
    "rd_batch_rotated_iou": (c_int, [c_void_p, c_int, c_void_p, c_void_p, c_void_p, c_int, c_long, c_int, c_void_p]),
    "rd_batch_rotated_iou_3d": (c_int, [c_void_p, c_int, c_void_p, c_void_p, c_void_p, c_int, c_long, c_int, c_void_p]),
    "rd_rotated_iou_7": (c_int, [c_void_p, c_void_p, c_void_p, c_long, c_long, c_void_p]),
    "rd_batch_max_iou": (c_int, [c_void_p, c_int, c_void_p, c_void_p, c_long, c_int, c_void_p]),
    "rd_gather_keep_scores": (c_int, [c_void_p, c_long, c_int, c_void_p, c_int, c_void_p, c_int, c_void_p]),
    "rd_nms3d_workspace_bytes": (c_size_t, [c_long, c_int]),
    "rd_nms3d": (c_int, [c_void_p, c_int, c_long, c_float, c_int, c_int, c_void_p, c_void_p, c_void_p, c_size_t, c_void_p]),
    "rd_assign3d_v2": (c_int, [c_void_p] * 6 + [c_long, c_int] + [c_float] * 7 + [c_void_p, c_void_p]),
    "rd_get_point_num_workspace_bytes": (c_size_t, []),
    "rd_get_point_num": (c_int, [c_void_p, c_long, c_void_p, c_void_p, c_size_t, c_void_p]),
    "rd_input_transform": (c_int, [c_void_p, c_void_p, c_void_p, c_void_p, c_int, c_int, c_int, c_int, c_int] + [c_void_p] * 8 + [c_void_p]),
    "rd_train_transform_workspace_bytes": (c_size_t, [c_int]),
    "rd_train_transform": (c_int, [c_void_p] * 9 + [c_int, c_float, c_float, c_void_p, c_int, c_int, c_int, c_int, c_int,
                                   c_void_p, c_void_p, c_size_t, c_void_p]),
    "rd_prof_enable": (c_int, [c_int]),
    "rd_prof_reset": (c_int, []),
    "rd_prof_get": (c_int, [c_int, ctypes.POINTER(ctypes.c_double), ctypes.POINTER(c_long)]),
}


class RangeDetError(RuntimeError):
    def __init__(self, code, msg):
        super().__init__("librangedet_hip error %d: %s" % (code, msg))
        self.code = code


def ptr(x):
    if x is None:
        return None
    if isinstance(x, int):
        return x
    if isinstance(x, np.ndarray):
        return x.ctypes.data
    if hasattr(x, "data_ptr"):
        return x.data_ptr()
    raise TypeError("cannot take the address of %r" % type(x))


class Lib:
    def __init__(self, path=DEFAULT_PATH):
        if not os.path.exists(path):
            raise RuntimeError(
                "%s not found: the HIP extension is not built (run `python -m rangedet_amd.build`). "
                "There is no CPU fallback." % path)
        self.path = path
        if os.path.basename(path).startswith("librangedet_hip"):
            try:
                import torch
            except ImportError:
                pass
        self.cdll = ctypes.CDLL(path)
        for name, (res, args) in SIGNATURES.items():
            fn = getattr(self.cdll, name)
            fn.restype = res
            fn.argtypes = args
        self.rd_last_error_string = self.cdll.rd_last_error_string

    def call(self, name, *args):
        rc = getattr(self.cdll, name)(*args)
        if rc < 0:
            raise RangeDetError(rc, self.cdll.rd_last_error_string().decode())
        return rc

    def raw(self, name):
        return getattr(self.cdll, name)

    def pack_conv_weight(self, w_oihw, dtype):
        w = np.ascontiguousarray(w_oihw, dtype=np.float32)
        cout, cin, kh, kw = w.shape
        out = np.zeros(self.cdll.rd_conv_packed_bytes(kh * kw, cin, cout, dtype), dtype=np.uint8)
        self.call("rd_pack_conv_weight_host", w.ctypes.data, cout, cin, kh, kw, dtype, out.ctypes.data)
        return out

    def pack_conv3x3_ex(self, w_oihw, stride_w, x_cstride, fold_scale=None, dtype=RD_BF16):
        w = np.ascontiguousarray(w_oihw, dtype=np.float32)
        cout, cin = w.shape[:2]
        assert w.shape[2:] == (3, 3)
        fs = None if fold_scale is None else np.ascontiguousarray(fold_scale, dtype=np.float32)
        out = np.zeros(self.cdll.rd_conv3x3_ex_packed_bytes(cin, cout, stride_w, x_cstride), dtype=np.uint8)
        self.call("rd_pack_conv3x3_ex_host", w.ctypes.data, None if fs is None else fs.ctypes.data, cout, cin, stride_w,
                  x_cstride, dtype, out.ctypes.data)
        return out

    def pack_conv3x3_m16(self, w_oihw, fold_scale, dtype=RD_BF16):
        w = np.ascontiguousarray(w_oihw, dtype=np.float32)
        cout, cin = w.shape[:2]
        assert w.shape[2:] == (3, 3)
        fs = np.ascontiguousarray(fold_scale, dtype=np.float32)
        out = np.zeros(self.cdll.rd_conv3x3_ex_packed_bytes(cin, cout, 1, cin), dtype=np.uint8)
        self.call("rd_pack_conv3x3_m16_host", w.ctypes.data, fs.ctypes.data, cout, cin, dtype, out.ctypes.data)
        return out

    def pack_conv3x3_cat(self, w_oihw, cin1, cin2, fold_scale=None, dtype=RD_BF16):
        w = np.ascontiguousarray(w_oihw, dtype=np.float32)
        cout = w.shape[0]
        assert w.shape[1:] == (cin1 + cin2, 3, 3)
        fs = None if fold_scale is None else np.ascontiguousarray(fold_scale, dtype=np.float32)
        out = np.zeros(self.cdll.rd_conv3x3_cat_packed_bytes(cin1, cin2, cout), dtype=np.uint8)
        self.call("rd_pack_conv3x3_cat_host", w.ctypes.data, None if fs is None else fs.ctypes.data, cout, cin1, cin2, dtype, out.ctypes.data)
        return out

    def pack_conv1x1_sc(self, w_oi, fold_scale=None, dtype=RD_BF16):
        w = np.ascontiguousarray(w_oi, dtype=np.float32).reshape(w_oi.shape[0], -1)
        cout, cin = w.shape
        fs = None if fold_scale is None else np.ascontiguousarray(fold_scale, dtype=np.float32)
        out = np.zeros(self.cdll.rd_conv1x1_sc_packed_bytes(cin, cout), dtype=np.uint8)
        self.call("rd_pack_conv1x1_sc_host", w.ctypes.data, None if fs is None else fs.ctypes.data, cout, cin, dtype, out.ctypes.data)
        return out

    def pack_block64(self, w1_oihw, scale1, w2_oihw, scale2, dtype=RD_BF16, m16=False):
        w1, w2 = (np.ascontiguousarray(w, dtype=np.float32) for w in (w1_oihw, w2_oihw))
        s1, s2 = (np.ascontiguousarray(v, dtype=np.float32) for v in (scale1, scale2))
        cin = w1.shape[1]
        assert w1.shape == (64, cin, 3, 3) and w2.shape == (64, 64, 3, 3) and s1.shape == (64,) and s2.shape == (64,)
        out = np.zeros(self.cdll.rd_block64_packed_bytes(cin), dtype=np.uint8)
        if m16:
            assert cin == 64
            self.call("rd_pack_block64_m16_host", w1.ctypes.data, s1.ctypes.data, w2.ctypes.data, s2.ctypes.data, dtype, out.ctypes.data)
        else:
            self.call("rd_pack_block64_host", w1.ctypes.data, s1.ctypes.data, w2.ctypes.data, s2.ctypes.data, cin, dtype, out.ctypes.data)
        return out

    def pack_conv1x1_sc_m16(self, w_oi, fold_scale, dtype=RD_BF16):
        w = np.ascontiguousarray(w_oi, dtype=np.float32).reshape(64, 64)
        fs = np.ascontiguousarray(fold_scale, dtype=np.float32)
        out = np.zeros(self.cdll.rd_conv1x1_sc_packed_bytes(64, 64), dtype=np.uint8)
        self.call("rd_pack_conv1x1_sc_m16_host", w.ctypes.data, fs.ctypes.data, dtype, out.ctypes.data)
        return out

    def pack_deconv_weight(self, w_iohw, stride_w, pad_w, phase, dtype, fold_scale=None):
        w = np.ascontiguousarray(w_iohw, dtype=np.float32)
        cin, cout, kh, kw = w.shape
        nt = self.cdll.rd_deconv_phase_taps(kh, kw, stride_w, pad_w, phase)
        if nt < 0:
            raise RangeDetError(nt, "deconv phase taps")
        out = np.zeros(self.cdll.rd_conv_packed_bytes(nt, cin, cout, dtype), dtype=np.uint8)
        fs = None if fold_scale is None else np.ascontiguousarray(fold_scale, dtype=np.float32)
        self.call("rd_pack_deconv_weight_folded_host", w.ctypes.data, None if fs is None else fs.ctypes.data, cin, cout, kh, kw,
                  stride_w, pad_w, phase, dtype, out.ctypes.data)
        return out

# ... 44 lines not shown
```

### rangedet_amd/lower.py

```python
import os
from dataclasses import dataclass, field

from . import devswitch
from .lib import H16, RD_ADD, RD_BF16, RD_F16, RD_F32, RD_RELU_POST, RD_RELU_PRE


@dataclass
class TRef:
    buf: int
    C: int
    H: int
    W: int
    cs: int
    co: int = 0
    cmap: tuple = None
    tail: "TRef" = None


@dataclass
class FlatRef:
    buf: int
    shape: tuple


@dataclass
class Plan:
    dtype: int
    batch: int
    steps: list = field(default_factory=list)
    buffers: dict = field(default_factory=dict)
    outputs: list = field(default_factory=list)
    input_vars: dict = field(default_factory=dict)
    num_classes: int = 1


def conv_steps(steps):
    for st in steps:
        if st["kind"] in ("conv_pair", "block"):
            yield st["a"], 0.5
            yield st["b"], 0.5
        elif st["kind"] == "conv":
            yield st, 1
        elif st["kind"] == "deconv":
            yield st, 1 if st.get("one_launch") else st["stride_w"]


def _strip_cast(s):
    while s.op == "cast":
        s = s.inputs[0]
    return s


def _is(s, op, **attrs):
    return s.op == op and all(s.attrs.get(k) == v for k, v in attrs.items())


class Lowering:
    def __init__(self, group, input_shapes, dtype, batch):
        assert dtype in (RD_F32, RD_BF16, RD_F16)
        self.dtype = dtype
        self.h16 = dtype in H16
        self.esz = 2 if self.h16 else 4
        self.gran = 16 if self.h16 else 8
        self.B = batch
        self.shapes = dict(input_shapes)
        self.plan = Plan(dtype=dtype, batch=batch)
        self.memo = {}
        self.nbuf = 0
        self.consumers = {}
        self._count_consumers(group)
        for out in group.inputs:
            self.plan.outputs.append(self.emit_value(out))
        self._fuse_head_out()
        self._fuse_blocks()
        self._pair_equal_convs()
        self._mark_mfma16()

    def _mark_mfma16(self):
        if not self.h16 or devswitch.get("RD_NO_MFMA16"):
            return
        for st in self.plan.steps:
            if st["kind"] == "block" and st["a"]["cin"] == 64 and not devswitch.get("RD_NO_MFMA16_BLOCK"):
                st["m16"] = True
            if st["kind"] == "conv" and tuple(st["k"]) == (3, 3) and st["cout"] == 128 and st["stride_w"] == 1 and st.get("ex") and \
                    st.get("fold") and not st.get("sc") and st.get("x2") is None and not st.get("s2view"):
                cin = len(st["cmap"]) if st.get("cmap") else st["cin"]
                if cin % 32 == 0 and cin >= 32:
                    st["m16"] = True

    def _pair_equal_convs(self):
        if not self.h16 or devswitch.get("RD_PAIR", "0") in ("", "0"):
            return
        max_w = int(devswitch.get("RD_PAIR_MAXW", "100000"))
        same_input_only = devswitch.get("RD_PAIR", "0") == "2"

        def sig(st):
            if st["kind"] != "conv" or not st.get("ex") or not st.get("fold") or st.get("sc") or st.get("s2view") or st.get("x2") is not None:
                return None
            if st["res"] is not None or st["cout"] != 128 or st["stride_w"] != 1 or tuple(st["k"]) != (3, 3) or st["flags"] != RD_RELU_POST:
                return None
            x, o, h = st["x"], st["out"], st.get("head")
            if x.W > max_w:
                return None
            return (x.H, x.W, x.cs, len(st["cmap"]) if st.get("cmap") else st["cin"], o.cs if not h else None,
                    (h["n_off"], h["N"]) if h else None)

        def is_write(key):
            return key in ("out", "out1", "head_out", "head_out1", "keep") or key.startswith("out_")

        out, written, touched, open_ = [], {}, {}, {}
        for st in self.plan.steps:
            k = sig(st)
            if k is not None:
                ready = written.get(st["x"].buf, -1)
                clear = max((touched.get(v.buf, -1) for v in (st["out"], st.get("head_out")) if v is not None), default=-1)
                j = next((j for j in open_.get(k, []) if ready < j and clear < j and (not same_input_only or out[j]["x"] == st["x"])), None)
                if j is not None:
                    open_[k].remove(j)
                    a = out[j]
                    p = dict(kind="conv_pair", name=a["name"] + " + " + st["name"], a=a, b=st, x=a["x"], x1=st["x"], out=a["out"],
                             out1=st["out"])
                    if a.get("head"):
                        p["head_out"], p["head_out1"] = a["head_out"], st["head_out"]
                    out[j] = p
                    for v in (st["out"], st.get("head_out")):
                        if v is not None:
                            written[v.buf] = max(written.get(v.buf, -1), j)
                            touched[v.buf] = max(touched.get(v.buf, -1), j)
                    touched[st["x"].buf] = max(touched.get(st["x"].buf, -1), j)
                    continue
                open_.setdefault(k, []).append(len(out))
            def refs(key, v):
                if isinstance(v, (TRef, FlatRef)):
                    yield key, v
                    if isinstance(v, TRef) and v.tail is not None:
                        yield key, v.tail
                elif isinstance(v, dict):
                    for k2, v2 in v.items():
                        yield from refs(k2 if isinstance(k2, str) else key, v2)
                elif isinstance(v, (list, tuple)):
                    for v2 in v:
                        yield from refs(key, v2)
            for key, v in st.items():
                for k2, r in refs(key, v):
                    touched[r.buf] = len(out)
                    if is_write(k2):
                        written[r.buf] = len(out)
            out.append(st)
        self.plan.steps = out

    def _fuse_blocks(self):
        if not self.h16 or devswitch.get("RD_NO_FUSE_BLOCK"):
            return
        steps = self.plan.steps
        uses = {}

        def scan(i, key, v):
            if isinstance(v, (TRef, FlatRef)):
                uses.setdefault(v.buf, []).append((i, key))
                if isinstance(v, TRef) and v.tail is not None:
                    scan(i, key + ".tail", v.tail)
            elif isinstance(v, dict):
                for k2, v2 in v.items():
                    scan(i, key + "." + str(k2), v2)
            elif isinstance(v, (list, tuple)):
                for k2, v2 in enumerate(v):
                    scan(i, key + "." + str(k2), v2)
        for i, st in enumerate(steps):
            for key, v in st.items():
                scan(i, key, v)
        for o in (self.plan.outputs if isinstance(self.plan.outputs, (list, tuple)) else []):
            scan(-1, "output", o)

        def plain64(st, first=False):
            if not (st["kind"] == "conv" and tuple(st["k"]) == (3, 3) and st["stride_w"] == 1 and st["cout"] == 64 and st.get("ex") and
                    st.get("fold") and not st.get("head") and st.get("x2") is None and st["x"].tail is None):
                return False
            if first and st["x"].cs - st["x"].co == 16 and st["x"].C <= 16:
                return not devswitch.get("RD_NO_FUSE_FIRST")
            return st["cin"] == 64 and st["x"].C == 64 and not st.get("cmap")

        out, i = [], 0
        while i < len(steps):
            a = steps[i]
            b = steps[i + 1] if i + 1 < len(steps) else None
            ok = b is not None and plain64(a, first=True) and plain64(b) and a["flags"] == RD_RELU_POST and a["res"] is None and not a.get("sc") and \
                b["flags"] == (RD_ADD | RD_RELU_POST) and b["x"] == a["out"] and a["out"].co == 0 and a["out"].cs == 64 and \
                sorted(uses.get(a["out"].buf, [])) == [(i, "out"), (i + 1, "x")] and b["out"].buf != a["x"].buf
            if ok:
                small = a["x"].C <= 16
                if b.get("sc"):
                    ok = b["res"] is None and b["sc_x"] == a["x"] and (small or (b["sc"]["cin"] == 64 and not b["sc"].get("cmap")))
                else:
                    ok = b["res"] == a["x"] and not small
            if ok:
                blk = dict(kind="block", name=a["name"] + " + " + b["name"], a=a, b=b, x=a["x"], out=b["out"])
                a["in_block"] = b["in_block"] = True
                self.plan.buffers.pop(a["out"].buf, None)
                out.append(blk)
                i += 2
            else:
                out.append(a)
                i += 1
        self.plan.steps = out

    def _fuse_head_out(self):
        if not self.h16 or devswitch.get("RD_NO_FUSE_HEAD"):
            return
        steps = self.plan.steps
        uses = {}
        for i, st in enumerate(steps):
            for key, v in st.items():
                if isinstance(v, TRef):
                    uses.setdefault(v.buf, []).append((i, key))
        drop = set()
        for i, st in enumerate(steps):
            if st["kind"] != "head_out" or st["nout"] > 8:
                continue
            x = st["x"]
            refs = uses.get(x.buf, [])
            prod = [j for j, key in refs if key == "out"]
            if len(refs) != 2 or len(prod) != 1 or x.co != 0 or x.C != 128:
                continue
            c = steps[prod[0]]
            if not (c["kind"] == "conv" and tuple(c["k"]) == (3, 3) and c["cout"] == 128 and c["stride_w"] == 1 and
                    c["flags"] == RD_RELU_POST and c.get("res") is None and c["out"] == x and c.get("x2") is None):
                continue
            c["head"] = dict(name=st["name"], rows=st["rows"], nout=st["nout"], out=st["out"], n_off=st["n_off"], N=st["N"])
            c["head_out"] = st["out"]
            drop.add(i)
        self.plan.steps = [st for i, st in enumerate(steps) if i not in drop]

    def _count_consumers(self, root):
        seen = set()

        def walk(s):
            for i in s.inputs:
                self.consumers[i.uid] = self.consumers.get(i.uid, 0) + 1
                if i.uid not in seen:
                    seen.add(i.uid)
                    walk(i)
        walk(root)

    def new_buf(self, nbytes, persistent=False, zero=False):
        self.nbuf += 1
        self.plan.buffers[self.nbuf] = dict(nbytes=int(nbytes), persistent=persistent, zero=zero)
        return self.nbuf

    def new_act(self, C, H, W, persistent=False, zero=False, cs=None):
        cs = cs or -(-C // self.gran) * self.gran
        buf = self.new_buf(self.B * H * W * cs * self.esz, persistent or cs != C, zero or cs != C)
        return TRef(buf, C, H, W, cs, 0)

    def step(self, kind, **kw):
        kw["kind"] = kind
        for key, v in kw.items():
            if isinstance(v, TRef) and v.tail is not None and not (kind == "conv" and key == "x" and kw.get("x2") is v.tail and tuple(kw.get("k", ())) == (3, 3)):
                raise NotImplementedError("%s step %r: operand %r is a virtual concat [%d channels | %d more from another tensor]; only a "
                                          "3x3 stride-1 convolution can read it (set RD_CONCAT_BUFFER=1 for a materialised concat)" %
                                          (kind, kw.get("name", ""), key, v.C, v.tail.C))
        self.plan.steps.append(kw)

    def want_input(self, name):
        if name not in self.shapes:
            raise KeyError("lowering needs the shape of input variable %r" % name)
        self.plan.input_vars[name] = tuple(self.shapes[name])
        return tuple(self.shapes[name])

    def emit_act(self, s, dest=None):
        s = _strip_cast(s)
        key = s.uid
        if s.op == "var" and dest is not None:
            return self._emit_act(s, dest)
        if key in self.memo:
            if dest is not None:
                raise NotImplementedError("%s is needed both stand-alone and inside a concat buffer" % s.name)
            return self.memo[key]
        r = self._emit_act(s, dest)
        if dest is None:
            self.memo[key] = r
        return r

    def _out(self, C, H, W, dest):
        if dest is None:
            return self.new_act(C, H, W)
        buf, cs, co = dest
        return TRef(buf, C, H, W, cs, co)

    def _emit_act(self, s, dest):
        if s.op == "var":
            C, H, W = self.want_input(s.name)
            out = self._out(C, H, W, dest) if dest else self.new_act(C, H, W, persistent=True)
            pad = (out.cs - out.co - C) if dest is None else 0
            self.step("nchw_in", name=s.name, out=out, zero_pad=pad)
            return out
        if _is(s, "Activation", act_type="relu"):
            inner = s.inputs[0]
            if inner.op == "elemwise_add":
                return self._residual_block(inner, dest)
            if inner.op == "BatchNorm" and inner.inputs[0].op == "Convolution":
                conv = inner.inputs[0]
                meta = self._match_meta(conv)
                if meta is not None:
                    return self._emit_meta(meta, conv, inner, dest)
                return self._conv_bn(conv, inner, RD_RELU_POST, None, dest)
        if s.op == "BatchNorm" and s.inputs[0].op == "Convolution":
            return self._conv_bn(s.inputs[0], s, 0, None, dest)
        if s.op == "elemwise_add":
            return self._agg_add(s, dest)
        if _is(s, "concat", dim=1):
            return self._concat(s, dest)
        raise NotImplementedError("no HIP lowering for %r (op %s) as an activation" % (s.name, s.op))

    def _conv_geom(self, conv, x):
        k = conv.attrs["kernel"]
        st = conv.attrs["stride"]
        pad = conv.attrs["pad"]
        if k not in ((1, 1), (3, 3)) or st[0] != 1 or st[1] not in (1, 2) or pad != ((k[0] - 1) // 2, (k[1] - 1) // 2):
            raise NotImplementedError("Convolution %s: kernel %s stride %s pad %s" % (conv.name, k, st, pad))
        Wout = (x.W + 2 * pad[1] - k[1]) // st[1] + 1
        return k, st[1], Wout

    def _conv_bn(self, conv, bn, flags, residual, dest, sc=None):
        if not conv.attrs["no_bias"]:
            raise NotImplementedError("Convolution %s with bias followed by BatchNorm" % conv.name)
        x = self.emit_act(conv.inputs[0])
        k, sw, Wout = self._conv_geom(conv, x)
        cout_l = conv.attrs["num_filter"]
        cout = 64 if cout_l <= 64 else 128 if cout_l <= 128 else None
        if cout is None:
            raise NotImplementedError("Convolution %s: %d output channels.  The HIP conv kernels are instantiated for 64 and 128 output "
                                      "channels (other widths up to 128 run zero-padded on those); more than 128 channels per layer "
                                      "(dla_backbone.py num_filter) has no lowering" % (conv.name, cout_l))
        if cout != cout_l and dest is not None:
            raise NotImplementedError("Convolution %s: %d output channels inside a channel concat (only 64 / 128 there)" % (conv.name, cout_l))
        out = self._out(cout, x.H, Wout, dest) if cout == cout_l else self.new_act(cout_l, x.H, Wout, cs=cout)
        fold = self.h16 and k == (3, 3) and not devswitch.get("RD_NO_FOLD")
        s2view = sw == 2 and x.W % 2 == 0 and not devswitch.get("RD_NO_S2_VIEW")
        ex = self.h16 and k == (3, 3) and (sc is not None or s2view or (fold and sw == 1))
        kw_fold = dict(fold=bool(ex and (fold or sc is not None)), s2view=bool(ex and s2view))
        kw = {}
        if sc is not None:
            scx = self.emit_act(sc[0].inputs[0])
            kw["sc"] = dict(name=sc[0].name, bn=sc[1].name, eps=sc[1].attrs["eps"], cin=scx.C, cmap=scx.cmap)
            kw["sc_x"] = scx
        if x.tail is not None:
            kw["x2"] = x.tail
        self.step("conv", name=conv.name, bn=bn.name, eps=bn.attrs["eps"], x=x, out=out, res=residual,
                  cin=sum(1 for m in x.cmap if m >= 0) if x.tail is not None else x.C,
                  cout=cout, cout_logical=cout_l, k=k, stride_w=sw, flags=flags, cmap=x.cmap, ex=ex, **kw_fold, **kw)
        return out

    def _fusable_projection(self, main_conv, sc):
        if not self.h16 or devswitch.get("RD_NO_FUSE_SC"):
            return None
        if not (sc.op == "BatchNorm" and sc.inputs[0].op == "Convolution"):
            return None
        c = sc.inputs[0]
        if c.attrs["kernel"] != (1, 1) or not c.attrs["no_bias"] or c.attrs["stride"] != main_conv.attrs["stride"] or \
                c.attrs["num_filter"] != main_conv.attrs["num_filter"] or self.consumers.get(sc.uid, 0) != 1:
            return None
        x0 = self.emit_act(c.inputs[0])
        if x0.C > 128 or (c.attrs["stride"][1] == 2 and x0.W % 2) or c.attrs["stride"][1] not in (1, 2):
            return None
        return (c, sc)

    def _residual_block(self, add, dest):
        a, b = add.inputs
        main = sc = None
        for m, o in ((a, b), (b, a)):
            if m.op == "BatchNorm" and m.inputs[0].op == "Convolution" and m.inputs[0].attrs["kernel"] == (3, 3):
                main, sc = m, o
                break
        if main is None:
            raise NotImplementedError("relu(add) without a BN(conv3x3) branch at %s" % add.name)
        proj = self._fusable_projection(main.inputs[0], sc)
        if proj is not None:
            return self._conv_bn(main.inputs[0], main, RD_ADD | RD_RELU_POST, None, dest, sc=proj)
        res = self.emit_act(sc)
        return self._conv_bn(main.inputs[0], main, RD_ADD | RD_RELU_POST, res, dest)

    def _agg_add(self, add, dest):
        a, b = add.inputs
        for skip, up in ((a, b), (b, a)):
            if _is(up, "Activation", act_type="relu") and up.inputs[0].op == "BatchNorm" and \
                    up.inputs[0].inputs[0].op == "Deconvolution":
                bn = up.inputs[0]
                dc = bn.inputs[0]
                x = self.emit_act(dc.inputs[0])
                res = self.emit_act(skip)
                kh, kw = dc.attrs["kernel"]
                sh, sw = dc.attrs["stride"]
                ph, pw = dc.attrs["pad"]
                if kh != 3 or sh != 1 or ph != 1:
                    raise NotImplementedError("Deconvolution %s: kernel/stride/pad height" % dc.name)
# ... 41 lines not shown
                raise ValueError("concat %s: parts do not line up" % s.name)
            start = [0, cs_list[0]]
            cmap = list(range(start[ia], start[ia] + fa.C)) + list(range(start[iv], start[iv] + fv.C)) + [-1] * (fv.cs - fv.C)
            return TRef(fa.buf, fa.C, fa.H, fa.W, fa.cs, fa.co, tuple(cmap), fv)
        ref_hw = None
        for p, d in zip(parts, dims):
            if d is not None:
                ref_hw = (d[1], d[2])
        if ref_hw is None:
            raise NotImplementedError("concat without a variable input: spatial size unknown before emission")
        offs, cmap, co = [], [], 0
        align = max(1, self.gran // 2)
        for c in cs_list:
            pad = -co % align
            cmap += [-1] * pad
            co += pad
            offs.append(co)
            cmap += list(range(len([m for m in cmap if m >= 0]), len([m for m in cmap if m >= 0]) + c))
            co += c
        Cphys = co
        out = self.new_act(Cphys, ref_hw[0], ref_hw[1], persistent=True, zero=True)
        if Cphys != Ctot:
            out.cmap = tuple(cmap)
        for p, c, o in zip(parts, cs_list, offs):
            r = self.emit_act(p, dest=(out.buf, out.cs, o))
            if (r.H, r.W) != ref_hw:
                raise ValueError("concat %s: spatial mismatch" % s.name)
        return out

    def _match_meta(self, agg_conv):
        try:
            a = agg_conv.inputs[0]
            if not _is(a, "Activation", act_type="relu"):
                return None
            bn1 = a.inputs[0]
            if bn1.op != "BatchNorm" or bn1.inputs[0].op != "reshape":
                return None
            mul = bn1.inputs[0].inputs[0]
            if mul.op != "multiply":
                return None
        except (IndexError, AttributeError):
            return None
        ds, wts = mul.inputs
        if not (ds.op == "reshape" and ds.inputs[0].op == "im2col"):
            raise NotImplementedError("meta kernel: unexpected data-sample branch at %s" % mul.name)
        im_d = ds.inputs[0]
        data = im_d.inputs[0]
        if im_d.attrs != dict(kernel=(3, 3), stride=(1, 1), dilate=(1, 1), pad=(1, 1)):
            raise NotImplementedError("meta kernel: only 3x3/stride 1/pad 1 sampling")
        c1 = wts.inputs[0] if wts.op == "reshape" else None
        ok = c1 is not None and c1.op == "Convolution" and _is(c1.inputs[0], "Activation", act_type="relu")
        c0 = c1.inputs[0].inputs[0] if ok else None
        ok = ok and c0.op == "Convolution" and c0.inputs[0].op == "reshape" and c0.inputs[0].inputs[0].op == "broadcast_minus"
        if not ok:
            raise NotImplementedError("meta kernel: unexpected MLP branch (only fc+relu+fc without norm)")
        bm = c0.inputs[0].inputs[0]
        nb, ctr = bm.inputs
        if not (nb.op == "reshape" and nb.inputs[0].op == "im2col" and ctr.op == "expand_dims"):
            raise NotImplementedError("meta kernel: unexpected relative-coordinate branch")
        coord = _strip_cast(ctr.inputs[0])
        if _strip_cast(nb.inputs[0].inputs[0]).uid != coord.uid or coord.op != "var":
            raise NotImplementedError("meta kernel: coordinates must be one input variable")
        if (c0.attrs["num_filter"], c1.attrs["num_filter"], agg_conv.attrs["num_filter"]) != (32, 64, 64) or \
                c0.attrs["no_bias"] or c1.attrs["no_bias"] or not agg_conv.attrs["no_bias"]:
            raise NotImplementedError("meta kernel %s: MLP %d -> %d, aggregation to %d channels.  The fused Meta-Kernel is built for the shipped "
                                      "unit only: 3 -> 32 -> 64 MLP with biases (meta_kernel_units / fc channels of the reference config), "
                                      "64 data channels, 9 x 64 = 576 -> 64 aggregation without bias" %
                                      (agg_conv.name, c0.attrs["num_filter"], c1.attrs["num_filter"], agg_conv.attrs["num_filter"]))
        return dict(data=data, coord=coord.name, mlp0=c0.name, mlp1=c1.name, bn1=bn1.name, eps1=bn1.attrs["eps"])

    def _emit_meta(self, m, agg_conv, bn2, dest):
        x = self.emit_act(m["data"])
        if x.C != 64:
            raise NotImplementedError("meta kernel %s: %d data channels (the fused Meta-Kernel is built for 64)" % (agg_conv.name, x.C))
        cshape = self.want_input(m["coord"])
        if cshape != (3, x.H, x.W):
            raise ValueError("meta kernel: coord shape %s vs data %s" % (cshape, (x.H, x.W)))
        out = self._out(64, x.H, x.W, dest)
        self.step("meta", x=x, out=out, coord=m["coord"], mlp0=m["mlp0"], mlp1=m["mlp1"], bn1=m["bn1"], eps1=m["eps1"],
                  agg=agg_conv.name, bn2=bn2.name, eps2=bn2.attrs["eps"])
        return out

    def emit_value(self, s):
        s0 = s
        key = ("v", s.uid, s.index)
        if key in self.memo:
            return self.memo[key]
        if s.op == "var":
            self.plan.input_vars.setdefault(s.name, None)
            v = ("input", s.name)
        elif s.op == "zeros":
            v = ("zeros", s.attrs["shape"])
        elif s.op == "Custom" and s.attrs["op_type"] == "get_sorted_foreground":
            v = ("flat", self._sorted_fg(s)[s.index])
        elif s.op == "Custom" and s.attrs["op_type"] == "batch_rotated_iou":
            v = ("flat", self._batch_riou(s))
        elif s.op == "Decode3DBbox":
            v = ("flat", self._decode(s))
        elif s.op == "NMS3D":
            keep, final = self._nms3d(s)
            v = ("flat_i32", keep) if s.index == 0 else ("flat", final)
        else:
            raise NotImplementedError("graph output %r (op %s) has no HIP lowering" % (s0.name, s.op))
        self.memo[key] = v
        return v

    def _flat_levels(self, s, transposed):
        levels = s.inputs if s.op == "concat" else [s]
        out = []
        for lv in levels:
            q = lv
            if transposed:
                if not _is(q, "transpose", axes=(0, 2, 1)):
                    raise NotImplementedError("bbox_delta level is not transposed (0,2,1)")
                q = q.inputs[0]
            if q.op != "squeeze" or q.inputs[0].op != "slice_axis" or q.inputs[0].inputs[0].op != "reshape":
                raise NotImplementedError("per-class flatten chain not recognised at %s" % lv.name)
            sl = q.inputs[0]
            cls_i = sl.attrs["begin"]
            if sl.attrs["axis"] != 1 or sl.attrs["end"] != cls_i + 1:
                raise NotImplementedError("slice_axis %s" % sl.name)
            conv = _strip_cast(sl.inputs[0].inputs[0])
            if conv.op != "Convolution" or conv.attrs["kernel"] != (1, 1) or conv.attrs["no_bias"]:
                raise NotImplementedError("head output must be a 1x1 Convolution with bias at %s" % lv.name)
            out.append((conv, cls_i))
        return out

    def _sorted_fg(self, s):
        key = ("sfg", s.uid)
        if key in self.memo:
            return self.memo[key]
        score, delta, pc, mask = s.inputs
        apply_sigmoid = 0
        if _is(score, "Activation", act_type="sigmoid"):
            apply_sigmoid = 1
            score = score.inputs[0]
        lv_s = self._flat_levels(score, False)
        lv_d = self._flat_levels(delta, True)
        if len(lv_s) != len(lv_d):
            raise ValueError("score / delta level count")
        feats, N = [], 0
        for (cs_, ci), (cd_, di) in zip(lv_s, lv_d):
            fs = self.emit_act(cs_.inputs[0])
            fd = self.emit_act(cd_.inputs[0])
            feats.append((cs_, ci, fs, cd_, di, fd, N))
            N += fs.H * fs.W
        ncls = lv_s[0][0].attrs["num_filter"]
        D = lv_d[0][0].attrs["num_filter"] // ncls
        logit = FlatRef(self.new_buf(self.B * N * 4, persistent=True), (N,))
        dl = FlatRef(self.new_buf(self.B * N * D * 4, persistent=True), (N, D))
        for cs_, ci, fs, cd_, di, fd, off in feats:
            self.step("head_out", name=cs_.name, x=fs, out=logit, n_off=off, N=N, rows=(ci, ci + 1), nout=1)
            self.step("head_out", name=cd_.name, x=fd, out=dl, n_off=off, N=N, rows=(di * D, di * D + D), nout=D)
        pcs = self._concat_vars(pc, 3)
        msk = self._concat_vars(mask, None)
        k = int(s.attrs["num_fgs"])
        if N < k:
            raise ValueError("get_sorted_foreground: N (%d) < num_fgs (%d)" % (N, k))
        o_s = FlatRef(self.new_buf(self.B * k * 4, persistent=True), (k,))
        o_d = FlatRef(self.new_buf(self.B * k * D * 4), (k, D))
        o_p = FlatRef(self.new_buf(self.B * k * 3 * 4), (k, 3))
        self.step("sorted_fg", score=logit, delta=dl, pc=pcs, mask=msk, N=N, k=k, D=D, apply_sigmoid=apply_sigmoid,
                  out_score=o_s, out_delta=o_d, out_pc=o_p)
        self.memo[key] = (o_s, o_d, o_p)
        return self.memo[key]

    def _concat_vars(self, s, last):
        parts = s.inputs if s.op == "concat" else [s]
        names, n = [], 0
        for p in parts:
            p = _strip_cast(p)
            if p.op != "var":
                raise NotImplementedError("pc / mask inputs must be input variables")
            shp = self.want_input(p.name)
            names.append((p.name, shp[0]))
            n += shp[0]
        ref = FlatRef(self.new_buf(self.B * n * (last or 1) * 4, persistent=True), (n, last) if last else (n,))
        self.step("concat_in", names=names, out=ref, last=last or 1, N=n)
        return ref

    def _decode(self, s):
        d, p = s.inputs
        if not (d.op == "Custom" and p.op == "Custom" and d.uid == p.uid and d.index == 1 and p.index == 2):
            raise NotImplementedError("Decode3DBbox inputs must be outputs 1,2 of get_sorted_foreground")
        o_s, o_d, o_p = self._sorted_fg(d)
        k = o_d.shape[0]
        out = FlatRef(self.new_buf(self.B * k * 10 * 4, persistent=True), (k, 10))
        self.step("decode", delta=o_d, pc=o_p, out=out, k=k, box_type=o_d.shape[1], is_bin=int(s.attrs["is_bin"]))
        return out


    def _batch_riou(self, s):
        key = ("briou", s.uid)
        if key in self.memo:
            return self.memo[key]
        iou_type = s.attrs.get("iou_type", "bev")
        if iou_type not in ("bev", "3d"):
            raise ValueError("batch_rotated_iou: iou_type %r ('bev' or '3d')" % iou_type)
        gdim = 8 if iou_type == "bev" else 7
        prop, gt = s.inputs
        kind, boxes = self.emit_value(prop)
        gt = _strip_cast(gt)
        if kind != "flat" or len(boxes.shape) != 2 or boxes.shape[1] != 10 or gt.op != "var":
            raise NotImplementedError("batch_rotated_iou: proposal must be a (B,N,10) box tensor, gt_bbox an input variable")
        gshape = self.want_input(gt.name)
        if len(gshape) != 2 or gshape[1] != gdim or gshape[0] > 256:
            raise ValueError("batch_rotated_iou (%s): gt_bbox shape %s (need (n_gt <= 256, %d))" % (iou_type, gshape, gdim))
        out = FlatRef(self.new_buf(self.B * boxes.shape[0] * 4, persistent=True), (boxes.shape[0],))
        self.step("batch_riou", boxes=boxes, gt=gt.name, N=boxes.shape[0], n_gt=gshape[0], out=out, iou_type=iou_type)
        self.memo[key] = out
        return out

    def _nms3d(self, s):
        key = ("nms3d", s.uid)
        if key in self.memo:
            return self.memo[key]
        (bx,) = s.inputs
        if bx.op != "Decode3DBbox":
            raise NotImplementedError("NMS3D input must be the Decode3DBbox output (score-sorted boxes)")
        boxes = self._decode(bx)
        n, mk = boxes.shape[0], int(s.attrs["max_keep"])
        keep = FlatRef(self.new_buf(self.B * mk * 4, persistent=True), (mk,))
        final = FlatRef(self.new_buf(self.B * mk * 10 * 4, persistent=True), (mk, 10))
        self.step("nms3d", boxes=boxes, N=n, thr=float(s.attrs["iou_thres"]), max_keep=mk,
                  normal_iou=int(s.attrs["normal_iou"]), keep=keep, out=final)
        self.memo[key] = (keep, final)
        return self.memo[key]


def lower(test_symbol, input_shapes, dtype=RD_BF16, batch=1):
    return Lowering(test_symbol, input_shapes, dtype, batch).plan
```

### rangedet_amd/pipeline.py

```python
import os
import numpy as np

from . import devswitch, lib as rdlib
from .config import rangedet_veh_wo_aug_4_18e as cfgmod
from .lower import lower
from .runtime import Executor, TorchAllocator


def input_shapes(H, W, strides=(1, 2, 4), channels=8):
    shapes = {'input_data': (channels, H, W), 'coord_s1': (3, H, W)}
    for s in strides:
        shapes['pc_vehicle_frame_s%d' % s] = (H * W // s, 3)
        shapes['range_image_mask_s%d' % s] = (H * W // s,)
    return shapes



def _stream_prio(var):
    return int(devswitch.get(var, "0"))


class BatchPostProcessor:

    def __init__(self, B, k, min_score, thr_lo, thr_hi, is_3d_iou, lib, alloc, cap=4096, hash_scale=100, tie_order="reference", wnms_diag=0):
        self.B, self.k, self.cap = B, k, min(cap, k, rdlib.RD_WNMS_MAX_K)
        self.hash_scale, self.tie_order = int(hash_scale), tie_order
        self.wnms_diag = int(wnms_diag)
        self.min_score, self.thr_lo, self.thr_hi, self.is3d = min_score, thr_lo, thr_hi, int(is_3d_iou)
        self.L, self.A = lib, alloc
        A, L = alloc, lib
        self.dets = A.alloc(B * k * 12 * 4)
        self.count = A.alloc(max(16, 4 * B), zero=True)
        self.ws_f_bytes = L.raw("rd_score_filter_workspace_bytes")(k) * B
        self.ws_f = A.alloc(self.ws_f_bytes)
        self.ws_w_bytes = L.raw("rd_wnms_workspace_bytes")(self.cap) * B
        self.ws_w = A.alloc(self.ws_w_bytes)
        self.out = A.alloc(B * self.cap * 12 * 4)
        self.keep = A.alloc(B * self.cap * 4)
        self.nkeep = A.alloc(max(16, 4 * B), zero=True)
        self.out8 = A.alloc(B * self.cap * 8 * 4)
        self.identity = A.upload(np.arange(self.cap, dtype=np.int32))
        self._host = None

    def enqueue_filter(self, score_ptr, score_bs, box_ptr, box_bs, stream=None):
        L, A = self.L, self.A
        st = A.stream_ptr(stream) if hasattr(A, "stream_ptr") else A.stream
        L.call("rd_score_filter_dets_batched", score_ptr, score_bs, box_ptr, box_bs, self.k, self.min_score, A.ptr(self.dets),
               self.k * 12, A.ptr(self.count), A.ptr(self.ws_f), self.ws_f_bytes, self.B, st)

    def enqueue_nms(self, stream=None):
        L, A = self.L, self.A
        st = A.stream_ptr(stream) if hasattr(A, "stream_ptr") else A.stream
        order = A.ptr(self.identity) if self.tie_order == "stable" else None
        L.call("rd_wnms_4c_batched", A.ptr(self.dets), self.k * 12, self.cap, A.ptr(self.count), order, 0,
               rdlib.RD_TIE_REFERENCE | self.wnms_diag, self.thr_lo, self.thr_hi, self.is3d, self.hash_scale, A.ptr(self.out), self.cap * 12,
               A.ptr(self.keep), self.cap, A.ptr(self.nkeep), A.ptr(self.ws_w), self.ws_w_bytes, self.B, st)
        L.call("rd_dets12_to_8_batched", A.ptr(self.out), self.cap * 12, self.cap, A.ptr(self.nkeep), A.ptr(self.out8),
               self.cap * 8, self.B, st)

    def collect_all(self, done=None):
        A = self.A
        if done is not None and hasattr(done, "synchronize"):
            done.synchronize()
        else:
            A.sync()
        count = np.array(A.to_numpy(A.view_i32(self.count, (self.B,))))
        nkeep = np.array(A.to_numpy(A.view_i32(self.nkeep, (self.B,))))
        if int(count.max()) > self.cap:
            raise rdlib.RangeDetError(rdlib.RD_EWORKSPACE, "%d detections above min_score exceed the WNMS capacity %d" % (int(count.max()), self.cap))
        m = int(nkeep.max()) if self.B else 0
        rows = np.array(A.to_numpy(A.view_f32(self.out, (self.B, self.cap, 12))[:, :m]))
        keep = np.array(A.to_numpy(A.view_i32(self.keep, (self.B, self.cap))[:, :m]))
        d8 = np.array(A.to_numpy(A.view_f32(self.out8, (self.B, self.cap, 8))[:, :m]))
        return [dict(num_candidates=int(count[b]), wnms_rows=rows[b, :nkeep[b]].copy(), keep_inds=keep[b, :nkeep[b]].copy(),
                     det_xyzlwhyaws=d8[b, :nkeep[b]].copy()) for b in range(self.B)]

    def collect(self, b=0):
        return self.collect_all()[b]


class Nms3dPostProcessor:

    def __init__(self, B, k, max_keep, min_score, lib, alloc):
        self.B, self.k, self.mk, self.min_score, self.L, self.A = B, k, max_keep, min_score, lib, alloc
        A, L = alloc, lib
        self.cap = max_keep
        self.kscore = A.alloc(B * max_keep * 4)
        self.dets = A.alloc(B * max_keep * 12 * 4)
        self.count = A.alloc(max(16, 4 * B), zero=True)
        self.ws_bytes = L.raw("rd_score_filter_workspace_bytes")(max_keep) * B
        self.ws = A.alloc(self.ws_bytes)
        self.out8 = A.alloc(B * max_keep * 8 * 4)
        self._keep = None

    def enqueue(self, score_ptr, score_bs, final_ptr, keep_ptr, keep_view, stream=None):
        L, A, mk = self.L, self.A, self.mk
        st = A.stream_ptr(stream) if hasattr(A, "stream_ptr") else A.stream
        self._keep = keep_view
        L.call("rd_gather_keep_scores", score_ptr, score_bs, self.k, keep_ptr, mk, A.ptr(self.kscore), self.B, st)
        L.call("rd_score_filter_dets_batched", A.ptr(self.kscore), mk, final_ptr, mk * 10, mk, self.min_score, A.ptr(self.dets),
               mk * 12, A.ptr(self.count), A.ptr(self.ws), self.ws_bytes, self.B, st)
        L.call("rd_dets12_to_8_batched", A.ptr(self.dets), mk * 12, mk, A.ptr(self.count), A.ptr(self.out8), mk * 8, self.B, st)

    def collect_all(self, done=None):
        if done is not None and hasattr(done, "synchronize"):
            done.synchronize()
        else:
            self.A.sync()
        return [self._collect(b) for b in range(self.B)]

    def collect(self, b=0):
        self.A.sync()
        return self._collect(b)

    def _collect(self, b):
        A = self.A
        K = int(A.to_numpy(A.view_i32(self.count, (self.B,)))[b])
        rows = A.to_numpy(A.view_f32(self.dets, (self.B, self.mk, 12)))[b, :K].copy()
        d8 = A.to_numpy(A.view_f32(self.out8, (self.B, self.mk, 8)))[b, :K].copy()
        keep = np.array(A.to_numpy(self._keep))[b]
        sc = A.to_numpy(A.view_f32(self.kscore, (self.B, self.mk)))[b]
        keep = keep[(keep >= 0) & (sc > self.min_score)]
        return dict(num_candidates=K, wnms_rows=rows, keep_inds=keep, det_xyzlwhyaws=d8)


class _FrameView:

    def __init__(self, bp, b):
        self.bp, self.b = bp, b
        self.cap = bp.cap

    def collect(self):
        return self.bp.collect(self.b)

    def out_rows(self):
        A = self.bp.A
        return A.view_f32(self.bp.out, (self.bp.B, self.bp.cap, 12))[self.b]

    def nkeep_view(self):
        A = self.bp.A
        return A.view_i32(self.bp.nkeep, (self.bp.B,))[self.b:self.b + 1]


class RangeDetPipeline:
    def __init__(self, params, dtype=rdlib.RD_BF16, feat_size=(64, 2650), pad_field=(64, 2656), batch=1,
                 pre_nms_top_n=50000, wnms_cap=4096, variant="veh", lib=None, alloc=None, wnms=True, tie_order="reference",
                 hash_scale=100, wnms_diag=0, graph=False):
        topn = pre_nms_top_n if isinstance(pre_nms_top_n, dict) else {cfgmod.variant_classes(variant)[0]: pre_nms_top_n}
        self.cfg = cfgmod.get_config(False, variant=variant, feat_size=feat_size, pad_field=pad_field,
                                     batch_image=batch, pre_nms_top_n=topn, wnms=wnms)
        self.wnms = bool(wnms)
        General, RpnParam, ModelParam, TestParam = self.cfg[0], self.cfg[2], self.cfg[6], self.cfg[8]
        self.lib = lib or rdlib.get_lib()
        self.alloc = alloc or TorchAllocator()
        self.class_names = tuple(General.class_names)
        nch = cfgmod.KITTI_INPUT_CHANNELS if variant == "kitti" else 8
        self.plan = lower(ModelParam.test_symbol, input_shapes(*pad_field, channels=nch), dtype, batch)
        self.exe = Executor(self.plan, params, self.lib, self.alloc)
        self.ks = {c: RpnParam.all_proposal.rpn_pre_nms_top_n[c] for c in self.class_names}
        self.batch = batch
        self.use_graph = bool(graph) and hasattr(self.alloc, "torch")
        self._graphs = {}
        self._capture_stream = None
        self.max_graphs = 8
        self.graph_replays = 0
        self._post_stream = None
        self.post_on_launch_stream = not devswitch.get("RD_POST_SIDE_STREAM")
        self._filter_done = None
        self._post_done = None
        assert self.wnms or len(self.class_names) == 1, "the NMS3D branch is single-class (tools/test.py:182)"
        self.bposts = {}
        for c in self.class_names:
            if self.wnms:
                self.bposts[c] = BatchPostProcessor(batch, self.ks[c], TestParam.min_score[c], TestParam.nms.thr_lo,
                                                    TestParam.nms.thr_hi, TestParam.nms.is_3d_iou, self.lib, self.alloc, wnms_cap,
                                                    hash_scale=hash_scale, tie_order=tie_order, wnms_diag=wnms_diag)
            else:
                self.bposts[c] = Nms3dPostProcessor(batch, self.ks[c], RpnParam.all_proposal.rpn_post_nms_top_n[c],
                                                    TestParam.min_score[c], self.lib, self.alloc)
        self.k = self.ks[self.class_names[0]]
        self.bpost = self.bposts[self.class_names[0]]
        self.post = [_FrameView(self.bpost, b) for b in range(batch)]

    def forward(self, inputs):
        return self.exe.forward(inputs)

    def enqueue(self, inputs):
        if self.use_graph:
            outs = self._enqueue_graph(inputs)
            if outs is not None:
                return outs
        return self._enqueue_eager(inputs)

    def _record(self, inputs):
        outs = self.exe.forward(inputs)
        ptr = lambda t: self.alloc.ptr(t) if hasattr(t, "data_ptr") else t.ctypes.data
        if not self.wnms:
            self.bpost.enqueue(ptr(outs[1]), self.k, ptr(outs[2]), ptr(outs[3]), outs[3], stream=None)
            return outs
        for ci, c in enumerate(self.class_names):
            sc, bx = outs[1 + 3 * ci], outs[2 + 3 * ci]
            sc_bs = (ptr(sc[1]) - ptr(sc[0])) // 4 if self.batch > 1 else 0
            bx_bs = (ptr(bx[1]) - ptr(bx[0])) // 4 if self.batch > 1 else 0
            self.bposts[c].enqueue_filter(ptr(sc[0]), sc_bs, ptr(bx[0]), bx_bs, stream=None)
        for c in self.class_names:
            self.bposts[c].enqueue_nms(stream=None)
        return outs

    def _enqueue_graph(self, inputs):
        A = self.alloc
        t = A.torch
        key = []
        for name in sorted(inputs):
            v = inputs[name]
            if v is None:
                continue
            if not (hasattr(v, "data_ptr") and v.is_cuda and v.is_contiguous() and v.dtype == t.float32):
                return None
            key.append((name, v.data_ptr(), tuple(v.shape)))
        key = tuple(key)
        cur = t.cuda.current_stream(A.device)
        ent = self._graphs.get(key)
        if ent is None:
            if len(self._graphs) >= self.max_graphs:
                return None
            outs = self._enqueue_eager(inputs, side_ok=False)
            g = t.cuda.CUDAGraph()
            if self._capture_stream is None:
                self._capture_stream = t.cuda.Stream(device=A.device)
            cap = self._capture_stream
            cap.wait_stream(cur)
            with t.cuda.graph(g, stream=cap):
                gouts = self._record(inputs)
            cur.wait_stream(cap)
            self._graphs[key] = (g, gouts, dict(inputs))
            return outs
        g, outs, _ = ent
        g.replay()
        self.graph_replays += 1
        self._post_stream = cur
        self._filter_done = None
        self._post_done = A.record_event(cur)
        return outs

    def _enqueue_eager(self, inputs, side_ok=True):
        A = self.alloc
        side = hasattr(A, "new_stream")
        if side and (self.post_on_launch_stream or not side_ok):
            self._post_stream = A.torch.cuda.current_stream(A.device)
        elif side and self._post_stream is None:
            self._post_stream = A.new_stream(priority=_stream_prio("RD_POST_STREAM_PRIO"))
        if side and self._filter_done is not None:
            A.wait_event(self._filter_done)
        outs = self.exe.forward(inputs)
        if side:
            A.wait_event(A.record_event(), self._post_stream)
        ptr = lambda t: self.alloc.ptr(t) if hasattr(t, "data_ptr") else t.ctypes.data
        if not self.wnms:
            sc, bx = outs[1], outs[2]
            self.bpost.enqueue(ptr(sc), self.k, ptr(bx), ptr(outs[3]), outs[3], stream=self._post_stream)
            self._filter_done = A.record_event(self._post_stream) if side else None
            self._post_done = self._filter_done
            return outs
        for ci, c in enumerate(self.class_names):
            sc, bx = outs[1 + 3 * ci], outs[2 + 3 * ci]
            sc_bs = (ptr(sc[1]) - ptr(sc[0])) // 4 if self.batch > 1 else 0
            bx_bs = (ptr(bx[1]) - ptr(bx[0])) // 4 if self.batch > 1 else 0
            self.bposts[c].enqueue_filter(ptr(sc[0]), sc_bs, ptr(bx[0]), bx_bs, stream=self._post_stream)
        self._filter_done = A.record_event(self._post_stream) if side else None
        for c in self.class_names:
            self.bposts[c].enqueue_nms(stream=self._post_stream)
        self._post_done = A.record_event(self._post_stream) if side else None
        return outs

    def collect(self):
        per = {c: self.bposts[c].collect_all(self._post_done) for c in self.class_names}
        res = []
        for b in range(self.batch):
            r = dict(per[self.class_names[0]][b])
            if len(self.class_names) > 1:
                r["per_class"] = {c: per[c][b] for c in self.class_names}
            res.append(r)
        return res

    def run(self, inputs):
        outs = self.enqueue(inputs)
        res = self.collect()
        r0 = dict(res[0]) if self.batch == 1 else dict(frames=res)
        r0["fg_cls_score"], r0["decoded_bbox"] = outs[1], outs[2]
        return r0


class InterleavedPipelines:

    def __init__(self, params, n=2, **kw):
        self.pipes = [RangeDetPipeline(params, **kw) for _ in range(n)]
        for p in self.pipes:
            p.post_on_launch_stream = not devswitch.get("RD_POST_SIDE_STREAM")
        A = self.pipes[0].alloc
        self.streams = [A.new_stream(priority=_stream_prio("RD_LAUNCH_STREAM_PRIO")) for _ in range(n)] if hasattr(A, "new_stream") else [None] * n
        self._i = 0

    def stream_context(self, j):
        import contextlib
        st = self.streams[j]
        return self.pipes[j].alloc.torch.cuda.stream(st) if st is not None else contextlib.nullcontext()

    def enqueue(self, inputs):
        j = self._i % len(self.pipes)
        self._i += 1
        with self.stream_context(j):
            return j, self.pipes[j].enqueue(inputs)

    def collect(self, j):
        return self.pipes[j].collect()
```

### rangedet_amd/runtime.py

```python
import os

import numpy as np

from . import devswitch, lib as rdlib
from .lower import FlatRef, TRef


class TorchAllocator:

    def __init__(self, device="cuda:0", stream=None):
        import torch
        if not torch.cuda.is_available():
            raise RuntimeError("rangedet_amd needs a ROCm GPU (torch.cuda.is_available() is False); there is no CPU fallback")
        self.torch = torch
        self.device = torch.device(device)
        torch.cuda.set_device(self.device)
        self._stream = stream

    @property
    def stream(self):
        st = self._stream or self.torch.cuda.current_stream(self.device)
        return st.cuda_stream

    def alloc(self, nbytes, zero=False):
# ... 85 lines not shown
                    last_use[v.buf] = i
                    first_def.setdefault(v.buf, i)
        for kind, v in plan.outputs:
            if kind in ("flat", "flat_i32"):
                last_use[v.buf] = len(plan.steps) + 1
        free = {}
        release = {}
        for b, i in last_use.items():
            release.setdefault(i, []).append(b)
        order = sorted(plan.buffers, key=lambda b: first_def.get(b, 0))
        by_def = {}
        for b in order:
            by_def.setdefault(first_def.get(b, 0), []).append(b)
        for i in range(len(plan.steps) + 2):
            for b in by_def.get(i, []):
                info = plan.buffers[b]
                if reuse and not info["persistent"] and free.get(info["nbytes"]):
                    self._phys[b] = free[info["nbytes"]].pop()
                else:
                    self._phys[b] = self.alloc.alloc(info["nbytes"], zero=info["zero"])
            for b in release.get(i, []):
                info = plan.buffers[b]
                if reuse and not info["persistent"] and last_use[b] <= len(plan.steps):
                    free.setdefault(info["nbytes"], []).append(self._phys[b])
        self.device_bytes = sum(int(t.numel()) if hasattr(t, "numel") else len(t) for t in {id(v): v for v in self._phys.values()}.values())

    def p(self, ref):
        return self.alloc.ptr(self._phys[ref.buf])

    def _bind(self, st, P):
        L, A, dt = self.lib, self.alloc, self.dtype
        k = st["kind"]
        b = dict(st)
        if k == "conv_pair":
            b["a"], b["b"] = self._bind(st["a"], P), self._bind(st["b"], P)
            return b
        if k == "block":
            ca, cb = st["a"], st["b"]
            w1, w2 = (np.asarray(P[c["name"] + "_weight"], np.float32) for c in (ca, cb))
            if ca.get("cmap"):
                wp = np.zeros((w1.shape[0], len(ca["cmap"])) + w1.shape[2:], np.float32)
                for pc, lc in enumerate(ca["cmap"]):
                    if lc >= 0:
                        wp[:, pc] = w1[:, lc]
                w1 = wp
            (s1, t1), (s2, t2) = bn_affine(P, ca["bn"], ca["eps"]), bn_affine(P, cb["bn"], cb["eps"])
            m16 = bool(st.get("m16")) and w1.shape[1] == 64
            b["m16"] = m16
            b["w"] = A.upload(L.pack_block64(w1, s1, w2, s2, dtype=dt, m16=m16))
            b["shift1"] = A.upload(t1)
            b["sc_w"] = None
            if cb.get("sc"):
                sc = cb["sc"]
                wsc = np.asarray(P[sc["name"] + "_weight"], np.float32).reshape(64, -1)
                if sc.get("cmap"):
                    wq = np.zeros((64, len(sc["cmap"])), np.float32)
                    for pc, lc in enumerate(sc["cmap"]):
                        if lc >= 0:
                            wq[:, pc] = wsc[:, lc]
                    wsc = wq
                ss, ts = bn_affine(P, sc["bn"], sc["eps"])
                b["sc_w"] = A.upload(L.pack_conv1x1_sc_m16(wsc, ss, dtype=dt) if m16 else L.pack_conv1x1_sc(wsc, fold_scale=ss, dtype=dt))
                t2 = (t2.astype(np.float64) + ts).astype(np.float32)
            b["shift2"] = A.upload(t2)
            b["cin"] = w1.shape[1]
            return b
        if k == "conv":
            w = pad_rows(np.asarray(P[st["name"] + "_weight"], np.float32), st["cout"])
            if st.get("cmap"):
                wp = np.zeros((w.shape[0], len(st["cmap"])) + w.shape[2:], np.float32)
                for pc, lc in enumerate(st["cmap"]):
                    if lc >= 0:
                        wp[:, pc] = w[:, lc]
                w = wp
            s, t = bn_affine(P, st["bn"], st["eps"], pad_to=st["cout"])
            if st.get("sc"):
                sc = st["sc"]
                wsc = np.asarray(P[sc["name"] + "_weight"], np.float32)
                wsc = pad_rows(wsc.reshape(wsc.shape[0], -1), st["cout"])
                if sc.get("cmap"):
                    wq = np.zeros((w.shape[0], len(sc["cmap"])), np.float32)
                    for pc, lc in enumerate(sc["cmap"]):
                        if lc >= 0:
                            wq[:, pc] = wsc[:, lc]
                    wsc = wq
                ss, ts = bn_affine(P, sc["bn"], sc["eps"], pad_to=st["cout"])
                b["w"] = A.upload(L.pack_conv3x3_ex(w, st["stride_w"], st["x"].cs, fold_scale=s, dtype=dt))
                b["sc_w"] = A.upload(L.pack_conv1x1_sc(wsc, fold_scale=ss, dtype=dt))
                b["scale"], b["shift"] = None, A.upload((t.astype(np.float64) + ts).astype(np.float32))
            elif st.get("x2") is not None:
                b["w"] = A.upload(L.pack_conv3x3_cat(w, st["x"].C, st["x2"].cs, fold_scale=s, dtype=dt))
                b["scale"], b["shift"] = None, A.upload(t)
                b["flags"] = st["flags"] | rdlib.RD_SCALE_FOLDED
            elif st.get("ex") and st.get("fold") and st.get("m16") and \
                    L.raw("rd_conv3x3_mfma16_ok")(w.shape[1], st["cout"], 1, st["x"].W, 1 if st.get("head") else 0) == 1:
                b["w"] = A.upload(L.pack_conv3x3_m16(w, s, dtype=dt))
                b["scale"], b["shift"] = None, A.upload(t)
                b["flags"] = st["flags"] | rdlib.RD_SCALE_FOLDED | rdlib.RD_MFMA16
            elif st.get("ex") and st.get("fold"):
                b["w"] = A.upload(L.pack_conv3x3_ex(w, st["stride_w"], st["x"].cs, fold_scale=s, dtype=dt))
                b["scale"], b["shift"] = None, A.upload(t)
                b["flags"] = st["flags"] | rdlib.RD_SCALE_FOLDED
            elif st.get("ex"):
                b["w"] = A.upload(L.pack_conv3x3_ex(w, st["stride_w"], st["x"].cs, dtype=dt))
                b["scale"], b["shift"] = A.upload(s), A.upload(t)
            else:
                b["w"] = A.upload(L.pack_conv_weight(w, dt))
                b["scale"], b["shift"] = A.upload(s), A.upload(t)
        elif k == "deconv":
            w = pad_rows(np.asarray(P[st["name"] + "_weight"], np.float32), st["cout"], axis=1)
            s, t = bn_affine(P, st["bn"], st["eps"], pad_to=st["cout"])
            fs = s if st.get("fold") else None
            imgs = [L.pack_deconv_weight(w, st["stride_w"], st["pad_w"], ph, dt, fold_scale=fs) for ph in range(st["stride_w"])]
            b["all_phases"] = bool(st.get("one_launch")) and len({len(i) for i in imgs}) == 1 and \
                L.raw("rd_deconv2d_all_phases_ok")(st["k"][0], st["k"][1], st["stride_w"], st["pad_w"], st["cout"], dt) == 1
            if st.get("one_launch") and not b["all_phases"] and not L.raw("rd_deconv2d_all_phases_ok")(st["k"][0], st["k"][1], st["stride_w"], st["pad_w"], st["cout"], dt):
                b["one_launch"] = False
            if b["all_phases"]:
                b["w_all"], b["w_pb"] = A.upload(np.concatenate(imgs)), len(imgs[0])
            r_, o_ = st["res"], st["out"]
            b["pairs"] = b["all_phases"] and not devswitch.get("RD_DECONV_NO_PAIRS") and o_.cs == st["cout"] and o_.co == 0 and \
                (r_ is None or (r_.cs == st["cout"] and r_.co == 0)) and \
                L.raw("rd_deconv2d_phase_pairs_ok")(st["k"][0], st["k"][1], st["stride_w"], st["pad_w"], st["cout"], dt) == 1
            if b["pairs"]:
                pimgs = [L.pack_deconv_phase_pair(imgs[p], imgs[p + 1], st["cin"], dt) for p in range(0, st["stride_w"], 2)]
                b["w_pairs"], b["w_pairb"], b["shift2"] = A.upload(np.concatenate(pimgs)), len(pimgs[0]), A.upload(np.concatenate([t, t]))
            b["w"] = [A.upload(i) for i in imgs]
            b["scale"], b["shift"] = (None if st.get("fold") else A.upload(s)), A.upload(t)
            if st.get("fold"):
                b["flags"] = st["flags"] | rdlib.RD_SCALE_FOLDED
        elif k == "meta":
            s1, t1 = bn_affine(P, st["bn1"], st["eps1"])
            s2, t2 = bn_affine(P, st["bn2"], st["eps2"])
            pk = L.pack_meta(P[st["mlp0"] + "_weight"].reshape(32, 3), P[st["mlp0"] + "_bias"],
                             P[st["mlp1"] + "_weight"].reshape(64, 32), P[st["mlp1"] + "_bias"], s1, t1,
                             P[st["agg"] + "_weight"].reshape(64, 576), s2, t2, dt)
            b["packed"] = A.upload(pk)
        if k == "conv" and st.get("head"):
            h = st["head"]
            r0, r1 = h["rows"]
            hw = np.asarray(P[h["name"] + "_weight"], np.float32).reshape(-1, st["cout"])[r0:r1]
            b["head_w"] = A.upload(L.pack_head_weight(hw, dtype=dt, m16=bool(b.get("flags", 0) & rdlib.RD_MFMA16)))
            b["head_bias"] = A.upload(np.asarray(P[h["name"] + "_bias"], np.float32)[r0:r1])
        elif k == "head_out":
            r0, r1 = st["rows"]
            w = np.asarray(P[st["name"] + "_weight"], np.float32).reshape(-1, st["x"].C)[r0:r1]
            b["w"] = A.upload(w)
            b["bias"] = A.upload(np.asarray(P[st["name"] + "_bias"], np.float32)[r0:r1])
        elif k == "nms3d":
            nb = L.raw("rd_nms3d_workspace_bytes")(st["N"], self.B)
            b["ws"] = A.alloc(nb)
            b["ws_bytes"] = nb
        elif k == "sorted_fg":
            nb = L.raw("rd_sorted_foreground_workspace_bytes")(st["N"], st["k"]) * self.B
            b["ws"] = A.alloc(nb)
            b["ws_bytes"] = nb
            b["idx"] = A.alloc(self.B * st["k"] * 4) if self.keep_sorted_idx else None
        return b

    def forward(self, inputs, only=None, dev=None):
        L, A, dt, B = self.lib, self.alloc, self.dtype, self.B
        st_ = A.stream
        dev = {} if dev is None else dev

        def din(name):
            if name not in dev:
                dev[name] = A.as_device_f32(inputs[name])
            return dev[name]

        steps = self._bound if only is None else [self._bound[only]]
        for b in steps:
            k = b["kind"]
            if k == "nchw_in":
                o = b["out"]
                src = din(b["name"])
                assert tuple(src.shape) == (B, o.C, o.H, o.W), (b["name"], tuple(src.shape), (B, o.C, o.H, o.W))
                L.call("rd_nchw_to_nhwc", A.ptr(src), self.p(o), B, o.C, o.H, o.W, o.cs, o.co, b["zero_pad"], dt, st_)
            elif k == "block":
                x, o = b["x"], b["out"]
                if b.get("m16"):
                    L.call("rd_block64_m16_bn_act", self.p(x), x.cs, x.co, A.ptr(b["w"]), A.ptr(b["shift1"]), A.ptr(b["shift2"]),
                           A.ptr(b["sc_w"]) if b["sc_w"] is not None else None, self.p(o), o.cs, o.co, B, x.H, x.W, dt, st_)
                else:
                    L.call("rd_block64_bn_act", self.p(x), x.cs, x.co, b["cin"], A.ptr(b["w"]), A.ptr(b["shift1"]), A.ptr(b["shift2"]),
                           A.ptr(b["sc_w"]) if b["sc_w"] is not None else None, self.p(o), o.cs, o.co, B, x.H, x.W, dt, st_)
            elif k == "conv_pair":
                p, q = b["a"], b["b"]
                x0, x1 = p["x"], q["x"]
                cin = len(p["cmap"]) if p.get("cmap") else p["cin"]
                if p.get("head"):
                    h0, h1 = p["head"], q["head"]
                    L.call("rd_conv2d_bn_act_head_out_pair",
                           self.p(x0), x0.co, A.ptr(p["w"]), A.ptr(p["shift"]), A.ptr(p["head_w"]), A.ptr(p["head_bias"]),
                           self.p(h0["out"]), h0["N"] * h0["nout"], h0["nout"],
                           self.p(x1), x1.co, A.ptr(q["w"]), A.ptr(q["shift"]), A.ptr(q["head_w"]), A.ptr(q["head_bias"]),
                           self.p(h1["out"]), h1["N"] * h1["nout"], h1["nout"],
                           x0.cs, h0["n_off"], B, x0.H, x0.W, cin, p["flags"], dt, st_)
                else:
                    o0, o1 = p["out"], q["out"]
                    L.call("rd_conv3x3_bn_act_pair", self.p(x0), x0.co, A.ptr(p["w"]), A.ptr(p["shift"]), self.p(o0), o0.co,
                           self.p(x1), x1.co, A.ptr(q["w"]), A.ptr(q["shift"]), self.p(o1), o1.co, x0.cs, o0.cs, B, x0.H, x0.W, cin,
                           p["flags"], dt, st_)
            elif k == "conv" and b.get("head"):
                x, h = b["x"], b["head"]
                L.call("rd_conv2d_bn_act_head_out", self.p(x), x.cs, x.co, A.ptr(b["w"]),
                       A.ptr(b["scale"]) if b["scale"] is not None else None, A.ptr(b["shift"]), B,
                       x.H, x.W, b["cin"], b["flags"], A.ptr(b["head_w"]), A.ptr(b["head_bias"]), self.p(h["out"]),
                       h["N"] * h["nout"], h["n_off"], h["nout"], dt, st_)
            elif k == "conv" and b.get("x2") is not None:
                x, x2, o = b["x"], b["x2"], b["out"]
                L.call("rd_conv3x3_bn_act_cat", self.p(x), x.cs, x.co, x.C, self.p(x2), x2.cs, x2.co, x2.cs, A.ptr(b["w"]), A.ptr(b["shift"]),
                       self.p(o), o.cs, o.co, B, x.H, x.W, b["cout"], b["flags"], dt, st_)
            elif k == "conv" and b.get("ex"):
                x, o, r, sx = b["x"], b["out"], b["res"], b.get("sc_x")
                cin = len(b["cmap"]) if b.get("cmap") else b["cin"]
                L.call("rd_conv3x3_bn_act_ex", self.p(x), x.cs, x.co, A.ptr(b["w"]), A.ptr(b["scale"]) if b["scale"] is not None else None,
                       A.ptr(b["shift"]), self.p(r) if r else None, r.cs if r else 0, r.co if r else 0,
                       self.p(sx) if sx else None, sx.cs if sx else 0, sx.co if sx else 0,
                       (len(b["sc"]["cmap"]) if b["sc"].get("cmap") else b["sc"]["cin"]) if sx else 0,
                       A.ptr(b["sc_w"]) if sx else None, self.p(o), o.cs, o.co, B, x.H, x.W, cin, b["cout"], b["stride_w"],
                       b["flags"], dt, st_)
            elif k == "conv":
                x, o, r = b["x"], b["out"], b["res"]
                L.call("rd_conv2d_bn_act", self.p(x), x.cs, x.co, A.ptr(b["w"]), A.ptr(b["scale"]), A.ptr(b["shift"]),
                       self.p(r) if r else None, r.cs if r else 0, r.co if r else 0, self.p(o), o.cs, o.co, B, x.H, x.W,
                       b["cin"], b["cout"], b["k"][0], b["k"][1], b["stride_w"], b["flags"], dt, st_)
            elif k == "deconv":
                x, o, r = b["x"], b["out"], b["res"]
                if b.get("pairs"):
                    L.call("rd_deconv2d_bn_act_pairs", self.p(x), x.cs, x.co, A.ptr(b["w_pairs"]), b["w_pairb"], A.ptr(b["shift2"]), self.p(r), r.cs,
                           r.co, self.p(o), o.cs, o.co, B, x.H, x.W, b["cin"], b["cout"], b["k"][0], b["k"][1], b["stride_w"], b["pad_w"],
                           b["flags"], dt, st_)
                    continue
                if b.get("all_phases"):
                    L.call("rd_deconv2d_bn_act_all", self.p(x), x.cs, x.co, A.ptr(b["w_all"]), b["w_pb"], A.ptr(b["shift"]), self.p(r), r.cs,
                           r.co, self.p(o), o.cs, o.co, B, x.H, x.W, b["cin"], b["cout"], b["k"][0], b["k"][1], b["stride_w"], b["pad_w"],
                           b["flags"], dt, st_)
                    continue
                for ph in range(b["stride_w"]):
                    L.call("rd_deconv2d_bn_act", self.p(x), x.cs, x.co, A.ptr(b["w"][ph]),
                           A.ptr(b["scale"]) if b["scale"] is not None else None, A.ptr(b["shift"]), self.p(r), r.cs, r.co, self.p(o), o.cs, o.co, B, x.H, x.W, b["cin"],
                           b["cout"], b["k"][0], b["k"][1], b["stride_w"], b["pad_w"], ph, b["flags"], dt, st_)
            elif k == "meta":
                x, o = b["x"], b["out"]
                c = din(b["coord"])
                assert tuple(c.shape) == (B, 3, x.H, x.W)
                L.call("rd_meta_kernel_fwd", self.p(x), x.cs, x.co, A.ptr(c), A.ptr(b["packed"]), self.p(o), o.cs, o.co,
                       B, x.H, x.W, dt, st_)
            elif k == "head_out":
                x, o = b["x"], b["out"]
                L.call("rd_head_out", self.p(x), x.cs, x.co, A.ptr(b["w"]), A.ptr(b["bias"]), self.p(o),
                       b["N"] * b["nout"], b["n_off"], B, x.H, x.W, x.C, b["nout"], dt, st_)
            elif k == "concat_in":
                o = b["out"]
                row = b["N"] * b["last"] * 4
                off = 0
                for name, n in b["names"]:
                    src = din(name)
                    assert tuple(src.shape)[:2] == (B, n), (name, tuple(src.shape))
                    L.call("rd_copy_rows", A.ptr(src), n * b["last"] * 4, self.p(o), row, off * b["last"] * 4,
                           n * b["last"] * 4, B, st_)
                    off += n
            elif k == "sorted_fg":
                L.call("rd_sorted_foreground", self.p(b["score"]), self.p(b["delta"]), self.p(b["pc"]), self.p(b["mask"]),
                       B, b["N"], b["k"], b["D"], b["apply_sigmoid"], self.p(b["out_score"]), self.p(b["out_delta"]),
                       self.p(b["out_pc"]), A.ptr(b["idx"]) if b["idx"] is not None else None, A.ptr(b["ws"]), b["ws_bytes"], st_)
            elif k == "decode":
                L.call("rd_decode3d_bbox", self.p(b["delta"]), self.p(b["pc"]), self.p(b["out"]), B, b["k"],
                       b["box_type"], b["is_bin"], st_)
            elif k == "batch_riou":
                g = din(b["gt"])
                three_d = b.get("iou_type", "bev") == "3d"
                assert tuple(g.shape) == (B, b["n_gt"], 7 if three_d else 8), (b["gt"], tuple(g.shape))
                L.call("rd_batch_rotated_iou_3d" if three_d else "rd_batch_rotated_iou", self.p(b["boxes"]), 10, A.ptr(g), self.p(b["out"]),
                       None, B, b["N"], b["n_gt"], st_)
            elif k == "nms3d":
                L.call("rd_nms3d", self.p(b["boxes"]), B, b["N"], b["thr"], b["max_keep"], b["normal_iou"], self.p(b["keep"]),
                       self.p(b["out"]), A.ptr(b["ws"]), b["ws_bytes"], st_)
            else:
                raise RuntimeError("unknown plan step %r" % k)
        if only is not None:
            return None
        outs = []
        for kind, v in self.plan.outputs:
            if kind == "flat":
                outs.append(A.view_f32(self._phys[v.buf], (B,) + tuple(v.shape)))
            elif kind == "flat_i32":
                outs.append(A.view_i32(self._phys[v.buf], (B,) + tuple(v.shape)))
            elif kind == "input":
                outs.append(inputs.get(v))
            else:
                outs.append(np.zeros(v, np.float32))
        return outs

    def read_flat(self, ref):
        self.alloc.sync()
        return np.array(self.alloc.to_numpy(self.alloc.view_f32(self._phys[ref.buf], (self.B,) + tuple(ref.shape))))

    def sorted_idx(self, which=0):
        b = [x for x in self._bound if x["kind"] == "sorted_fg"][which]
        self.alloc.sync()
        return np.array(self.alloc.to_numpy(self.alloc.view_i32(b["idx"], (self.B, b["k"]))))

    def debug_tensor(self, ref):
        A, L = self.alloc, self.lib
        out = A.alloc(self.B * ref.C * ref.H * ref.W * 4)
        L.call("rd_nhwc_to_nchw", self.p(ref), A.ptr(out), self.B, ref.C, ref.H, ref.W, ref.cs, ref.co, self.dtype, A.stream)
        A.sync()
        return A.to_numpy(A.view_f32(out, (self.B, ref.C, ref.H, ref.W)))
```

Measured before the change: 1015.

## Fuse sorted-foreground selection, box decode and score filter into one tail path

```diff
diff --git a/include/rangedet_hip.h b/include/rangedet_hip.h
--- a/include/rangedet_hip.h
+++ b/include/rangedet_hip.h
@@ -140,6 +140,12 @@
                                  long n, float min_score, float* dets, long dets_bstride, int* d_count, void* ws,
                                  size_t ws_bytes, int B, void* stream);
 
+size_t rd_sorted_decode_filter_workspace_bytes(long N, long k);
+int rd_sorted_decode_filter(const float* cls_score, const float* bbox_delta, const float* const* pc_levels,
+                            const float* const* mask_levels, const long* level_n, int n_levels, int B, long N, long k, int D,
+                            int apply_sigmoid, int is_bin, float min_score, int cap, float* out_score, float* out_box, int* out_idx,
+                            float* dets, long dets_bstride, int* d_count, void* ws, size_t ws_bytes, void* stream);
+
 #define RD_WNMS_MAX_K 65536
 #define RD_TIE_STABLE 0
 #define RD_TIE_REFERENCE 1
diff --git a/rangedet_amd/csrc/k_misc.h b/rangedet_amd/csrc/k_misc.h
--- a/rangedet_amd/csrc/k_misc.h
+++ b/rangedet_amd/csrc/k_misc.h
@@ -175,12 +175,8 @@
   }
 }
 
-__global__ __launch_bounds__(256) void decode3d_kernel(const float* __restrict__ delta, const float* __restrict__ pc,
-                                                       float* __restrict__ out, long n, int box_type, int is_bin) {
-  long idx = blockIdx.x * 256L + threadIdx.x;
-  if (idx >= n) return;
-  const float* d = delta + idx * box_type;
-  float pc_x = pc[idx * 3 + 0], pc_y = pc[idx * 3 + 1], pc_z = pc[idx * 3 + 2];
+__device__ __forceinline__ void decode3d_point(const float* __restrict__ d, float pc_x, float pc_y, float pc_z, int is_bin,
+                                               float* __restrict__ o) {
   float az = atan2f(pc_y, pc_x);
   float ca = cosf(az), sa = sinf(az);
   float dx, dy, width, length, height, z0, yaw_l;
@@ -209,7 +205,6 @@
   float hl = (float)(0.5 * (double)length), hw = (float)(0.5 * (double)width);
   float hx[4] = {hl, -hl, -hl, hl};
   float hy[4] = {-hw, -hw, hw, hw};
-  float* o = out + idx * 10;
 #pragma unroll
   for (int k = 0; k < 4; ++k) {
     o[2 * k] = (hx[k] * cyw - hy[k] * sy) + cx;
@@ -218,7 +213,21 @@
   o[8] = z0;
   o[9] = z0 + height;
 }
-
+__global__ __launch_bounds__(256) void decode3d_kernel(const float* __restrict__ delta, const float* __restrict__ pc,
+                                                       float* __restrict__ out, long n, int box_type, int is_bin) {
+  long idx = blockIdx.x * 256L + threadIdx.x;
+  if (idx >= n) return;
+  decode3d_point(delta + idx * box_type, pc[idx * 3 + 0], pc[idx * 3 + 1], pc[idx * 3 + 2], is_bin, out + idx * 10);
+}
+
+__device__ __forceinline__ void dets_row_from_box10(const float* __restrict__ b, float score, float* __restrict__ d) {
+#pragma unroll
+  for (int k = 0; k < 8; ++k) d[k] = b[k];
+  d[8] = fdlibm_atan2f(b[1] - b[3], b[0] - b[2]);
+  d[9] = b[8];
+  d[10] = b[9] - b[8];
+  d[11] = score;
+}
 __global__ __launch_bounds__(256) void filter_count_kernel(const float* __restrict__ scores, long n, float thr,
                                                            int* __restrict__ blk_cnt, long sc_bs, long blk_bs) {
   scores += blockIdx.y * sc_bs;
@@ -277,14 +286,7 @@
   for (int w = 0; w < wv; ++w) off += wc[w];
   if (p) {
     int pos = off + __popcll(m & ((1ull << ln) - 1ull));
-    const float* b = boxes10 + i * 10;
-    float* d = dets + (size_t)pos * 12;
-#pragma unroll
-    for (int k = 0; k < 8; ++k) d[k] = b[k];
-    d[8] = fdlibm_atan2f(b[1] - b[3], b[0] - b[2]);
-    d[9] = b[8];
-    d[10] = b[9] - b[8];
-    d[11] = scores[i];
+    dets_row_from_box10(boxes10 + i * 10, scores[i], dets + (size_t)pos * 12);
   }
 }
 
diff --git a/rangedet_amd/csrc/k_sort.h b/rangedet_amd/csrc/k_sort.h
--- a/rangedet_amd/csrc/k_sort.h
+++ b/rangedet_amd/csrc/k_sort.h
@@ -1,5 +1,6 @@
 #pragma once
 #include "rd_common.h"
+#include "k_misc.h"
 
 namespace rd {
 
@@ -324,4 +325,271 @@
   return radix_sort_pairs(v, N, st, nb, ws_stride, s.sel + 1, true);
 }
 
-}
+constexpr int TAIL_MAX_LEVELS = 4;
+struct TailLevels {
+  const float* pc[TAIL_MAX_LEVELS];
+  const float* mask[TAIL_MAX_LEVELS];
+  long off[TAIL_MAX_LEVELS + 1];
+  int n;
+};
+struct TailAt { const float* pc; const float* mask; long off, n; };
+__device__ __forceinline__ TailAt tail_at(const TailLevels& lv, long i) {
+  TailAt a{lv.pc[0], lv.mask[0], lv.off[0], lv.off[1] - lv.off[0]};
+#pragma unroll
+  for (int q = 1; q < TAIL_MAX_LEVELS; ++q)
+    if (q < lv.n && i >= lv.off[q]) { a.pc = lv.pc[q]; a.mask = lv.mask[q]; a.off = lv.off[q]; a.n = lv.off[q + 1] - lv.off[q]; }
+  return a;
+}
+
+struct TailWs {
+  unsigned *keysA, *keysB, *idxA, *idxB, *hist, *h12, *cnt, *sel;
+  int nblk;
+};
+inline size_t tail_ws_bytes(long N) {
+  long nblk = (N + SORT_TILE - 1) / SORT_TILE;
+  return (size_t)(4 * N + 4 * nblk * 256 + SEL_BINS + nblk + 64) * 4 + 256;
+}
+inline TailWs tail_ws_carve(void* ws, long N) {
+  TailWs s;
+  s.nblk = (int)((N + SORT_TILE - 1) / SORT_TILE);
+  unsigned* p = (unsigned*)ws;
+  s.keysA = p; p += N;
+  s.keysB = p; p += N;
+  s.idxA = p; p += N;
+  s.idxB = p; p += N;
+  s.hist = p; p += (size_t)4 * s.nblk * 256;
+  s.h12 = p; p += SEL_BINS;
+  s.cnt = p; p += s.nblk;
+  s.sel = p;
+  return s;
+}
+
+__global__ __launch_bounds__(256) void tail_keyhist_kernel(const float* __restrict__ score, TailLevels lv, long N, int apply_sigmoid,
+                                                           unsigned* __restrict__ keys, unsigned* __restrict__ hist,
+                                                           unsigned* __restrict__ h12, long ws_stride) {
+  const long b = blockIdx.y;
+  keys += b * ws_stride; hist += b * ws_stride; h12 += b * ws_stride;
+  __shared__ unsigned h[SEL_BINS];
+  for (int i = threadIdx.x; i < SEL_BINS; i += 256) h[i] = 0;
+#pragma unroll
+  for (int p = 0; p < 4; ++p) hist[((size_t)p * gridDim.x + blockIdx.x) * 256 + threadIdx.x] = 0;
+  __syncthreads();
+  const long base = (long)blockIdx.x * SORT_TILE;
+  for (int r = 0; r < SORT_TILE / 256; ++r) {
+    const long i = base + r * 256 + threadIdx.x;
+    if (i < N) {
+      float s = score[b * N + i];
+      if (apply_sigmoid) s = 1.0f / (1.0f + expf(-s));
+      const TailAt a = tail_at(lv, i);
+      if (a.mask) s = s * a.mask[b * a.n + (i - a.off)];
+      const unsigned key = desc_key(s);
+      keys[i] = key;
+      atomicAdd(&h[key >> SEL_SHIFT], 1u);
+    }
+  }
+  __syncthreads();
+  for (int i = threadIdx.x; i < SEL_BINS; i += 256)
+    if (h[i]) atomicAdd(&h12[i], h[i]);
+}
+
+__global__ __launch_bounds__(256) void tail_count_kernel(const unsigned* __restrict__ keys, long N, long k, const unsigned* __restrict__ h12,
+                                                         unsigned* __restrict__ sel, unsigned* __restrict__ cnt, long ws_stride) {
+  keys += blockIdx.y * ws_stride; h12 += blockIdx.y * ws_stride; sel += blockIdx.y * ws_stride; cnt += blockIdx.y * ws_stride;
+  __shared__ unsigned part[256];
+  __shared__ unsigned sT, sM, c;
+  const int tid = threadIdx.x;
+  unsigned loc[SEL_BINS / 256], sum = 0;
+#pragma unroll
+  for (int j = 0; j < SEL_BINS / 256; ++j) { loc[j] = h12[tid * (SEL_BINS / 256) + j]; sum += loc[j]; }
+  part[tid] = sum;
+  if (tid == 0) c = 0;
+  __syncthreads();
+  for (int off = 1; off < 256; off <<= 1) {
+    const unsigned v = tid >= off ? part[tid - off] : 0u;
+    __syncthreads();
+    part[tid] += v;
+    __syncthreads();
+  }
+  unsigned before = part[tid] - sum;
+  if (tid == 255 && (k == 0 || part[255] < (unsigned)k)) { sT = SEL_BINS - 1; sM = part[255]; }
+  if (before < (unsigned)k && before + sum >= (unsigned)k) {
+#pragma unroll
+    for (int j = 0; j < SEL_BINS / 256; ++j) {
+      if (before < (unsigned)k && before + loc[j] >= (unsigned)k) { sT = tid * (SEL_BINS / 256) + j; sM = before + loc[j]; }
+      before += loc[j];
+    }
+  }
+  __syncthreads();
+  const unsigned T = sT;
+  if (blockIdx.x == 0 && tid == 0) { sel[0] = T; sel[1] = sM; }
+  const long base = (long)blockIdx.x * SORT_TILE;
+  unsigned mine = 0;
+  for (int r = 0; r < SORT_TILE / 256; ++r) {
+    const long i = base + r * 256 + tid;
+    if (i < N && (keys[i] >> SEL_SHIFT) <= T) ++mine;
+  }
+  if (mine) atomicAdd(&c, mine);
+  __syncthreads();
+  if (tid == 0) cnt[blockIdx.x] = c;
+}
+
+__global__ __launch_bounds__(256) void tail_compact_kernel(const unsigned* __restrict__ keys_in, long N, const unsigned* __restrict__ sel,
+                                                           const unsigned* __restrict__ cnt, unsigned* __restrict__ keys_out,
+                                                           unsigned* __restrict__ idx_out, unsigned* __restrict__ hist0, long ws_stride) {
+  {
+    const long o = blockIdx.y * ws_stride;
+    keys_in += o; sel += o; cnt += o; keys_out += o; idx_out += o; hist0 += o;
+  }
+  const unsigned T = sel[0];
+  __shared__ unsigned wcnt[4][8], sbase, dh[2][256];
+  const int tid = threadIdx.x, lane = tid & 63, wv = tid >> 6;
+  dh[0][tid] = 0; dh[1][tid] = 0;
+  if (tid == 0) {
+    unsigned b = 0;
+    for (unsigned j = 0; j < blockIdx.x; ++j) b += cnt[j];
+    sbase = b;
+  }
+  const long base = (long)blockIdx.x * SORT_TILE + wv * 512;
+  unsigned key[8];
+  unsigned long long m[8];
+#pragma unroll
+  for (int r = 0; r < 8; ++r) {
+    const long i = base + r * 64 + lane;
+    const bool valid = i < N;
+    key[r] = valid ? keys_in[i] : 0xFFFFFFFFu;
+    m[r] = __ballot(valid && (key[r] >> SEL_SHIFT) <= T);
+    if (lane == 0) wcnt[wv][r] = (unsigned)__popcll(m[r]);
+  }
+  __syncthreads();
+  const unsigned tile0 = sbase / SORT_TILE;
+  unsigned off = sbase;
+  for (int w = 0; w < wv; ++w)
+#pragma unroll
+    for (int r = 0; r < 8; ++r) off += wcnt[w][r];
+#pragma unroll
+  for (int r = 0; r < 8; ++r) {
+    if ((m[r] >> lane) & 1ull) {
+      const unsigned dst = off + (unsigned)__popcll(m[r] & ((1ull << lane) - 1ull));
+      keys_out[dst] = key[r];
+      idx_out[dst] = (unsigned)(base + r * 64 + lane);
+      atomicAdd(&dh[dst / SORT_TILE - tile0][key[r] & 255u], 1u);
+    }
+    off += (unsigned)__popcll(m[r]);
+  }
+  __syncthreads();
+#pragma unroll
+  for (int t = 0; t < 2; ++t)
+    if (dh[t][tid]) atomicAdd(&hist0[(size_t)(tile0 + t) * 256 + tid], dh[t][tid]);
+}
+
+__global__ __launch_bounds__(256) void tail_scatter_kernel(const unsigned* __restrict__ keys_in, const unsigned* __restrict__ idx_in,
+                                                           int shift, const unsigned* __restrict__ hist,
+                                                           unsigned* __restrict__ hist_next, unsigned* __restrict__ keys_out,
+                                                           unsigned* __restrict__ idx_out, const unsigned* __restrict__ sel,
+                                                           long ws_stride) {
+  const long N = (long)sel[blockIdx.y * ws_stride + 1];
+  if ((long)blockIdx.x * SORT_TILE >= N) return;
+  {
+    const long o = blockIdx.y * ws_stride;
+    keys_in += o; idx_in += o; hist += o; keys_out += o; idx_out += o;
+    if (hist_next) hist_next += o;
+  }
+  __shared__ unsigned wcnt[4][256];
+  __shared__ unsigned gbase[256];
+  __shared__ unsigned scan[256];
+  const int tid = threadIdx.x, lane = tid & 63, wv = tid >> 6;
+  for (int w = 0; w < 4; ++w) wcnt[w][tid] = 0;
+  {
+    const unsigned ntile = (unsigned)((N + SORT_TILE - 1) / SORT_TILE);
+    unsigned before = 0, t = 0;
+    for (unsigned b = 0; b < ntile; ++b) {
+      const unsigned v = hist[(size_t)b * 256 + tid];
+      if (b < blockIdx.x) before += v;
+      t += v;
+    }
+    scan[tid] = t;
+    __syncthreads();
+    for (int off = 1; off < 256; off <<= 1) {
+      unsigned a = tid >= off ? scan[tid - off] : 0u;
+      __syncthreads();
+      scan[tid] += a;
+      __syncthreads();
+    }
+    gbase[tid] = scan[tid] - t + before;
+  }
+  __syncthreads();
+
+  unsigned key[8], id[8], pos[8];
+  const long base = (long)blockIdx.x * SORT_TILE + wv * 512;
+  const unsigned long long lt = (1ull << lane) - 1ull;
+#pragma unroll
+  for (int r = 0; r < 8; ++r) {
+    long i = base + r * 64 + lane;
+    bool valid = i < N;
+    key[r] = valid ? keys_in[i] : 0xFFFFFFFFu;
+    id[r] = valid ? idx_in[i] : 0u;
+    unsigned d = (key[r] >> shift) & 255u;
+    unsigned long long peers = __ballot(valid);
+#pragma unroll
+    for (int bit = 0; bit < 8; ++bit) {
+      unsigned long long bm = __ballot(valid && ((d >> bit) & 1u));
+      peers &= ((d >> bit) & 1u) ? bm : ~bm;
+    }
+    unsigned rank = __popcll(peers & lt), cnt = __popcll(peers);
+    unsigned prev = wcnt[wv][d];
+    pos[r] = prev + rank;
+    __builtin_amdgcn_wave_barrier();
+    if (valid && rank == 0) wcnt[wv][d] = prev + cnt;
+    __builtin_amdgcn_wave_barrier();
+  }
+  __syncthreads();
+  {
+    unsigned c0 = wcnt[0][tid], c1 = wcnt[1][tid], c2 = wcnt[2][tid];
+    wcnt[0][tid] = 0;
+    wcnt[1][tid] = c0;
+    wcnt[2][tid] = c0 + c1;
+    wcnt[3][tid] = c0 + c1 + c2;
+  }
+  __syncthreads();
+#pragma unroll
+  for (int r = 0; r < 8; ++r) {
+    long i = base + r * 64 + lane;
+    if (i < N) {
+      unsigned d = (key[r] >> shift) & 255u;
+      unsigned dst = gbase[d] + wcnt[wv][d] + pos[r];
+      keys_out[dst] = key[r];
+      idx_out[dst] = id[r];
+      if (hist_next) atomicAdd(&hist_next[(size_t)(dst / SORT_TILE) * 256 + ((key[r] >> (shift + 8)) & 255u)], 1u);
+    }
+  }
+}
+
+__global__ __launch_bounds__(256) void tail_decode_filter_kernel(const unsigned* __restrict__ keys, const unsigned* __restrict__ idx,
+                                                                 long k, int D, int is_bin, const float* __restrict__ delta,
+                                                                 TailLevels lv, long N, float* __restrict__ out_score,
+                                                                 float* __restrict__ out_box, int* __restrict__ out_idx, float thr,
+                                                                 int cap, float* __restrict__ dets, long dets_bs,
+                                                                 int* __restrict__ d_count, long ws_stride) {
+  const long i = blockIdx.x * 256L + threadIdx.x;
+  if (i >= k) return;
+  const long b = blockIdx.y;
+  keys += b * ws_stride; idx += b * ws_stride;
+  const unsigned j = idx[i];
+  const float s = key_to_float(keys[i]);
+  const TailAt a = tail_at(lv, (long)j);
+  const float* p = a.pc + (b * a.n + ((long)j - a.off)) * 3;
+  float box[10];
+  decode3d_point(delta + ((size_t)b * N + j) * D, p[0], p[1], p[2], is_bin, box);
+  out_score[b * k + i] = s;
+  float* o = out_box + ((size_t)b * k + i) * 10;
+#pragma unroll
+  for (int c = 0; c < 10; ++c) o[c] = box[c];
+  if (out_idx) out_idx[b * k + i] = (int)j;
+  const bool keep = s > thr;
+  const bool next = i + 1 < k && key_to_float(keys[i + 1]) > thr;
+  if (keep && !next) d_count[b] = (int)(i + 1);
+  if (i == 0 && !keep) d_count[b] = 0;
+  if (keep && i < cap) dets_row_from_box10(box, s, dets + b * dets_bs + (size_t)i * 12);
+}
+
+}
diff --git a/rangedet_amd/csrc/rd_api.hip b/rangedet_amd/csrc/rd_api.hip
--- a/rangedet_amd/csrc/rd_api.hip
+++ b/rangedet_amd/csrc/rd_api.hip
@@ -720,6 +720,64 @@
 int rd_score_filter_dets(const float* scores, const float* boxes10, long n, float min_score, float* dets, int* d_count,
                          void* ws, size_t ws_bytes, void* stream) {
   return rd_score_filter_dets_batched(scores, 0, boxes10, 0, n, min_score, dets, 0, d_count, ws, ws_bytes, 1, stream);
+}
+
+size_t rd_sorted_decode_filter_workspace_bytes(long N, long k) { (void)k; return (tail_ws_bytes(N) + 256 + 255) & ~(size_t)255; }
+int rd_sorted_decode_filter(const float* cls_score, const float* bbox_delta, const float* const* pc_levels,
+                            const float* const* mask_levels, const long* level_n, int n_levels, int B, long N, long k, int D,
+                            int apply_sigmoid, int is_bin, float min_score, int cap, float* out_score, float* out_box, int* out_idx,
+                            float* dets, long dets_bstride, int* d_count, void* ws, size_t ws_bytes, void* stream) {
+  RD_REQUIRE(cls_score && bbox_delta && pc_levels && level_n && out_score && out_box && dets && d_count && ws, RD_EINVAL,
+             "sorted_decode_filter: null pointer");
+  RD_REQUIRE(B > 0 && N > 0 && k > 0, RD_ESHAPE, "sorted_decode_filter: empty shape");
+  RD_REQUIRE(N >= k, RD_ESHAPE, "sorted_decode_filter: N (%ld) < num_fgs (%ld)", N, k);
+  RD_REQUIRE(N < (1L << 31), RD_ESHAPE, "sorted_decode_filter: N too large");
+  RD_REQUIRE((is_bin && D == 7) || (!is_bin && D == 8), RD_ESHAPE, "sorted_decode_filter: D %d with is_bin=%d (8 for regular, 7 for bin)", D, is_bin);
+  RD_REQUIRE(n_levels >= 1 && n_levels <= TAIL_MAX_LEVELS, RD_ESHAPE, "sorted_decode_filter: %d levels (1..%d)", n_levels, TAIL_MAX_LEVELS);
+  RD_REQUIRE(cap > 0 && (B == 1 || dets_bstride >= (long)cap * 12), RD_ESHAPE, "sorted_decode_filter: cap %d / dets stride %ld", cap, dets_bstride);
+  TailLevels lv;
+  memset(&lv, 0, sizeof(lv));
+  lv.n = n_levels;
+  for (int l = 0; l < n_levels; ++l) {
+    RD_REQUIRE(level_n[l] > 0 && pc_levels[l] && (!mask_levels || mask_levels[l]), RD_EINVAL, "sorted_decode_filter: level %d is empty / null", l);
+    lv.off[l + 1] = lv.off[l] + level_n[l];
+  }
+  RD_REQUIRE(lv.off[n_levels] == N, RD_ESHAPE, "sorted_decode_filter: the levels hold %ld points, N is %ld", lv.off[n_levels], N);
+  const size_t per = rd_sorted_decode_filter_workspace_bytes(N, k);
+  RD_REQUIRE(ws_bytes >= per, RD_EWORKSPACE, "sorted_decode_filter: workspace %zu < %zu", ws_bytes, per);
+  hipStream_t st = (hipStream_t)stream;
+  void* wsa = (void*)(((uintptr_t)ws + 255) & ~(uintptr_t)255);
+  TailWs s = tail_ws_carve(wsa, N);
+  ProfScope ps(RD_PROF_SORT, st);
+  const bool wide = ws_bytes >= per * (size_t)B;
+  const long stride = wide ? (long)(per / 4) : 0;
+  const int nb = wide ? B : 1;
+  const size_t hpass = (size_t)s.nblk * 256;
+  for (int b0 = 0; b0 < B; b0 += nb) {
+    for (int l = 0; l < n_levels; ++l) {
+      lv.pc[l] = pc_levels[l] + (size_t)b0 * level_n[l] * 3;
+      lv.mask[l] = mask_levels ? mask_levels[l] + (size_t)b0 * level_n[l] : nullptr;
+    }
+    const hipError_t e = nb > 1 ? hipMemset2DAsync(s.h12, (size_t)stride * 4, 0, (size_t)SEL_BINS * 4, nb, st)
+                                : hipMemsetAsync(s.h12, 0, (size_t)SEL_BINS * 4, st);
+    if (e != hipSuccess) return rd::fail(RD_EHIP, "sorted_decode_filter: memset");
+    hipLaunchKernelGGL(tail_keyhist_kernel, dim3(s.nblk, nb), dim3(256), 0, st, cls_score + (size_t)b0 * N, lv, N, apply_sigmoid, s.keysA,
+                       s.hist, s.h12, stride);
+    hipLaunchKernelGGL(tail_count_kernel, dim3(s.nblk, nb), dim3(256), 0, st, s.keysA, N, k, s.h12, s.sel, s.cnt, stride);
+    hipLaunchKernelGGL(tail_compact_kernel, dim3(s.nblk, nb), dim3(256), 0, st, s.keysA, N, s.sel, s.cnt, s.keysB, s.idxB, s.hist, stride);
+    unsigned *ki = s.keysB, *ko = s.keysA, *ii = s.idxB, *io = s.idxA;
+    for (int pass = 0; pass < 4; ++pass) {
+      hipLaunchKernelGGL(tail_scatter_kernel, dim3(s.nblk, nb), dim3(256), 0, st, ki, ii, pass * 8, s.hist + pass * hpass,
+                         pass < 3 ? s.hist + (pass + 1) * hpass : nullptr, ko, io, s.sel, stride);
+      std::swap(ki, ko);
+      std::swap(ii, io);
+    }
+    hipLaunchKernelGGL(tail_decode_filter_kernel, dim3((unsigned)((k + 255) / 256), nb), dim3(256), 0, st, ki, ii, k, D, is_bin,
+                       bbox_delta + (size_t)b0 * N * D, lv, N, out_score + (size_t)b0 * k, out_box + (size_t)b0 * k * 10,
+                       out_idx ? out_idx + (size_t)b0 * k : nullptr, min_score, cap, dets + (size_t)b0 * dets_bstride, dets_bstride,
+                       d_count + b0, stride);
+  }
+  return check_launch("sorted_decode_filter");
 }
 
 size_t rd_wnms_workspace_bytes(int Kcap) { return Kcap > 0 ? wnms_ws_bytes(Kcap) : 0; }
diff --git a/rangedet_amd/lib.py b/rangedet_amd/lib.py
--- a/rangedet_amd/lib.py
+++ b/rangedet_amd/lib.py
@@ -96,6 +96,10 @@
     "rd_score_filter_dets": (c_int, [c_void_p, c_void_p, c_long, c_float, c_void_p, c_void_p, c_void_p, c_size_t, c_void_p]),
     "rd_score_filter_dets_batched": (c_int, [c_void_p, c_long, c_void_p, c_long, c_long, c_float, c_void_p, c_long, c_void_p,
                                              c_void_p, c_size_t, c_int, c_void_p]),
+    "rd_sorted_decode_filter_workspace_bytes": (c_size_t, [c_long, c_long]),
+    "rd_sorted_decode_filter": (c_int, [c_void_p, c_void_p, c_void_p, c_void_p, c_void_p, c_int, c_int, c_long, c_long, c_int, c_int, c_int,
+                                        c_float, c_int, c_void_p, c_void_p, c_void_p, c_void_p, c_long, c_void_p, c_void_p, c_size_t,
+                                        c_void_p]),
     "rd_wnms_workspace_bytes": (c_size_t, [c_int]),
     "rd_wnms_4c_batched": (c_int, [c_void_p, c_long, c_int, c_void_p, c_void_p, c_long, c_int, c_float, c_float, c_int, c_int,
                                    c_void_p, c_long, c_void_p, c_long, c_void_p, c_void_p, c_size_t, c_int, c_void_p]),
diff --git a/rangedet_amd/lower.py b/rangedet_amd/lower.py
--- a/rangedet_amd/lower.py
+++ b/rangedet_amd/lower.py
@@ -56,7 +56,7 @@
 
 
 class Lowering:
-    def __init__(self, group, input_shapes, dtype, batch):
+    def __init__(self, group, input_shapes, dtype, batch, fuse_tail=False):
         assert dtype in (RD_F32, RD_BF16, RD_F16)
         self.dtype = dtype
         self.h16 = dtype in H16
@@ -69,6 +69,7 @@
         self.nbuf = 0
         self.consumers = {}
         self._count_consumers(group)
+        self.tail_decode = self._find_tail_decodes(group) if (fuse_tail and self.h16 and not devswitch.get("RD_NO_TAIL_FUSE")) else {}
         for out in group.inputs:
             self.plan.outputs.append(self.emit_value(out))
         self._fuse_head_out()
@@ -241,6 +242,24 @@
                     seen.add(i.uid)
                     walk(i)
         walk(root)
+
+    def _find_tail_decodes(self, root):
+        readers, seen = {}, set()
+
+        def walk(s):
+            for i in s.inputs:
+                if i.op == "Custom" and i.attrs.get("op_type") == "get_sorted_foreground" and i.index in (1, 2):
+                    readers.setdefault(i.uid, []).append((s, i.index))
+                if i.uid not in seen:
+                    seen.add(i.uid)
+                    walk(i)
+        walk(root)
+        out = {}
+        for uid, rd in readers.items():
+            decs = {id(r): r for r, _ in rd}
+            if len(decs) == 1 and rd[0][0].op == "Decode3DBbox" and sorted(ix for _, ix in rd) == [1, 2]:
+                out[uid] = rd[0][0]
+        return out
 
     def new_buf(self, nbytes, persistent=False, zero=False):
         self.nbuf += 1
@@ -588,18 +607,38 @@
         for cs_, ci, fs, cd_, di, fd, off in feats:
             self.step("head_out", name=cs_.name, x=fs, out=logit, n_off=off, N=N, rows=(ci, ci + 1), nout=1)
             self.step("head_out", name=cd_.name, x=fd, out=dl, n_off=off, N=N, rows=(di * D, di * D + D), nout=D)
-        pcs = self._concat_vars(pc, 3)
-        msk = self._concat_vars(mask, None)
         k = int(s.attrs["num_fgs"])
         if N < k:
             raise ValueError("get_sorted_foreground: N (%d) < num_fgs (%d)" % (N, k))
         o_s = FlatRef(self.new_buf(self.B * k * 4, persistent=True), (k,))
+        dec = self.tail_decode.get(s.uid)
+        if dec is not None:
+            pcn, mkn = self._level_vars(pc), self._level_vars(mask)
+            if [n for _, n in pcn] == [n for _, n in mkn] and sum(n for _, n in pcn) == N and len(pcn) <= 4 and \
+                    (D, int(dec.attrs["is_bin"])) in ((8, 0), (7, 1)):
+                box = FlatRef(self.new_buf(self.B * k * 10 * 4, persistent=True), (k, 10))
+                self.step("sorted_fg", fused=True, score=logit, delta=dl, pc_names=pcn, mask_names=mkn, N=N, k=k, D=D,
+                          apply_sigmoid=apply_sigmoid, is_bin=int(dec.attrs["is_bin"]), out_score=o_s, out_box=box)
+                self.memo[key] = (o_s, None, None)
+                self.memo[("tail_box", s.uid)] = box
+                return self.memo[key]
+        pcs = self._concat_vars(pc, 3)
+        msk = self._concat_vars(mask, None)
         o_d = FlatRef(self.new_buf(self.B * k * D * 4), (k, D))
         o_p = FlatRef(self.new_buf(self.B * k * 3 * 4), (k, 3))
         self.step("sorted_fg", score=logit, delta=dl, pc=pcs, mask=msk, N=N, k=k, D=D, apply_sigmoid=apply_sigmoid,
                   out_score=o_s, out_delta=o_d, out_pc=o_p)
         self.memo[key] = (o_s, o_d, o_p)
         return self.memo[key]
+
+    def _level_vars(self, s):
+        out = []
+        for p in (s.inputs if s.op == "concat" else [s]):
+            p = _strip_cast(p)
+            if p.op != "var":
+                raise NotImplementedError("pc / mask inputs must be input variables")
+            out.append((p.name, self.want_input(p.name)[0]))
+        return out
 
     def _concat_vars(self, s, last):
         parts = s.inputs if s.op == "concat" else [s]
@@ -620,6 +659,8 @@
         if not (d.op == "Custom" and p.op == "Custom" and d.uid == p.uid and d.index == 1 and p.index == 2):
             raise NotImplementedError("Decode3DBbox inputs must be outputs 1,2 of get_sorted_foreground")
         o_s, o_d, o_p = self._sorted_fg(d)
+        if ("tail_box", d.uid) in self.memo:
+            return self.memo[("tail_box", d.uid)]
         k = o_d.shape[0]
         out = FlatRef(self.new_buf(self.B * k * 10 * 4, persistent=True), (k, 10))
         self.step("decode", delta=o_d, pc=o_p, out=out, k=k, box_type=o_d.shape[1], is_bin=int(s.attrs["is_bin"]))
@@ -664,5 +705,5 @@
         return self.memo[key]
 
 
-def lower(test_symbol, input_shapes, dtype=RD_BF16, batch=1):
-    return Lowering(test_symbol, input_shapes, dtype, batch).plan
+def lower(test_symbol, input_shapes, dtype=RD_BF16, batch=1, fuse_tail=False):
+    return Lowering(test_symbol, input_shapes, dtype, batch, fuse_tail=fuse_tail).plan
diff --git a/rangedet_amd/pipeline.py b/rangedet_amd/pipeline.py
--- a/rangedet_amd/pipeline.py
+++ b/rangedet_amd/pipeline.py
@@ -41,6 +41,11 @@
         self.out8 = A.alloc(B * self.cap * 8 * 4)
         self.identity = A.upload(np.arange(self.cap, dtype=np.int32))
         self._host = None
+        self.fused_filter = False
+
+    def bind_to_tail(self, exe, step):
+        exe.bind_tail_filter(step, self.min_score, self.cap, self.A.ptr(self.dets), self.k * 12, self.A.ptr(self.count))
+        self.fused_filter = True
 
     def enqueue_filter(self, score_ptr, score_bs, box_ptr, box_bs, stream=None):
         L, A = self.L, self.A
@@ -155,7 +160,7 @@
         self.alloc = alloc or TorchAllocator()
         self.class_names = tuple(General.class_names)
         nch = cfgmod.KITTI_INPUT_CHANNELS if variant == "kitti" else 8
-        self.plan = lower(ModelParam.test_symbol, input_shapes(*pad_field, channels=nch), dtype, batch)
+        self.plan = lower(ModelParam.test_symbol, input_shapes(*pad_field, channels=nch), dtype, batch, fuse_tail=bool(wnms))
         self.exe = Executor(self.plan, params, self.lib, self.alloc)
         self.ks = {c: RpnParam.all_proposal.rpn_pre_nms_top_n[c] for c in self.class_names}
         self.batch = batch
@@ -178,6 +183,13 @@
             else:
                 self.bposts[c] = Nms3dPostProcessor(batch, self.ks[c], RpnParam.all_proposal.rpn_post_nms_top_n[c],
                                                     TestParam.min_score[c], self.lib, self.alloc)
+        if self.wnms:
+            for ci, c in enumerate(self.class_names):
+                o_s = self.plan.outputs[1 + 3 * ci][1]
+                for stp in self.exe.tail_steps():
+                    if stp["out_score"].buf == o_s.buf:
+                        self.bposts[c].bind_to_tail(self.exe, stp)
+            assert all(stp["filter"] is not None for stp in self.exe.tail_steps())
         self.k = self.ks[self.class_names[0]]
         self.bpost = self.bposts[self.class_names[0]]
         self.post = [_FrameView(self.bpost, b) for b in range(batch)]
@@ -202,7 +214,8 @@
             sc, bx = outs[1 + 3 * ci], outs[2 + 3 * ci]
             sc_bs = (ptr(sc[1]) - ptr(sc[0])) // 4 if self.batch > 1 else 0
             bx_bs = (ptr(bx[1]) - ptr(bx[0])) // 4 if self.batch > 1 else 0
-            self.bposts[c].enqueue_filter(ptr(sc[0]), sc_bs, ptr(bx[0]), bx_bs, stream=None)
+            if not self.bposts[c].fused_filter:
+                self.bposts[c].enqueue_filter(ptr(sc[0]), sc_bs, ptr(bx[0]), bx_bs, stream=None)
         for c in self.class_names:
             self.bposts[c].enqueue_nms(stream=None)
         return outs
@@ -252,6 +265,9 @@
             self._post_stream = A.new_stream(priority=_stream_prio("RD_POST_STREAM_PRIO"))
         if side and self._filter_done is not None:
             A.wait_event(self._filter_done)
+        if side and self._post_done is not None and any(getattr(p, "fused_filter", False) for p in self.bposts.values()) and \
+                self._post_stream != A.torch.cuda.current_stream(A.device):
+            A.wait_event(self._post_done)
         outs = self.exe.forward(inputs)
         if side:
             A.wait_event(A.record_event(), self._post_stream)
@@ -266,7 +282,8 @@
             sc, bx = outs[1 + 3 * ci], outs[2 + 3 * ci]
             sc_bs = (ptr(sc[1]) - ptr(sc[0])) // 4 if self.batch > 1 else 0
             bx_bs = (ptr(bx[1]) - ptr(bx[0])) // 4 if self.batch > 1 else 0
-            self.bposts[c].enqueue_filter(ptr(sc[0]), sc_bs, ptr(bx[0]), bx_bs, stream=self._post_stream)
+            if not self.bposts[c].fused_filter:
+                self.bposts[c].enqueue_filter(ptr(sc[0]), sc_bs, ptr(bx[0]), bx_bs, stream=self._post_stream)
         self._filter_done = A.record_event(self._post_stream) if side else None
         for c in self.class_names:
             self.bposts[c].enqueue_nms(stream=self._post_stream)
diff --git a/rangedet_amd/runtime.py b/rangedet_amd/runtime.py
--- a/rangedet_amd/runtime.py
+++ b/rangedet_amd/runtime.py
@@ -261,7 +261,9 @@
             b["ws"] = A.alloc(nb)
             b["ws_bytes"] = nb
         elif k == "sorted_fg":
-            nb = L.raw("rd_sorted_foreground_workspace_bytes")(st["N"], st["k"]) * self.B
+            wsfn = "rd_sorted_decode_filter_workspace_bytes" if st.get("fused") else "rd_sorted_foreground_workspace_bytes"
+            nb = L.raw(wsfn)(st["N"], st["k"]) * self.B
+            b["filter"] = None
             b["ws"] = A.alloc(nb)
             b["ws_bytes"] = nb
             b["idx"] = A.alloc(self.B * st["k"] * 4) if self.keep_sorted_idx else None
@@ -370,6 +372,20 @@
                     L.call("rd_copy_rows", A.ptr(src), n * b["last"] * 4, self.p(o), row, off * b["last"] * 4,
                            n * b["last"] * 4, B, st_)
                     off += n
+            elif k == "sorted_fg" and b.get("fused"):
+                f = b["filter"]
+                if f is None:
+                    raise RuntimeError("the plan was lowered with fuse_tail: bind the score filter's buffers first (Executor.bind_tail_filter)")
+                pcs, mks = [din(n) for n, _ in b["pc_names"]], [din(n) for n, _ in b["mask_names"]]
+                for (name, n), t, m in zip(b["pc_names"], pcs, mks):
+                    assert tuple(t.shape) == (B, n, 3) and tuple(m.shape) == (B, n), (name, tuple(t.shape), tuple(m.shape))
+                pp = np.array([A.ptr(t) for t in pcs], np.uint64)
+                mp = np.array([A.ptr(t) for t in mks], np.uint64)
+                ln = np.array([n for _, n in b["pc_names"]], np.int64)
+                L.call("rd_sorted_decode_filter", self.p(b["score"]), self.p(b["delta"]), pp.ctypes.data, mp.ctypes.data, ln.ctypes.data,
+                       len(ln), B, b["N"], b["k"], b["D"], b["apply_sigmoid"], b["is_bin"], f["min_score"], f["cap"],
+                       self.p(b["out_score"]), self.p(b["out_box"]), A.ptr(b["idx"]) if b["idx"] is not None else None,
+                       f["dets"], f["dets_bstride"], f["count"], A.ptr(b["ws"]), b["ws_bytes"], st_)
             elif k == "sorted_fg":
                 L.call("rd_sorted_foreground", self.p(b["score"]), self.p(b["delta"]), self.p(b["pc"]), self.p(b["mask"]),
                        B, b["N"], b["k"], b["D"], b["apply_sigmoid"], self.p(b["out_score"]), self.p(b["out_delta"]),
@@ -402,6 +418,12 @@
                 outs.append(np.zeros(v, np.float32))
         return outs
 
+    def tail_steps(self):
+        return [b for b in self._bound if b["kind"] == "sorted_fg" and b.get("fused")]
+
+    def bind_tail_filter(self, step, min_score, cap, dets_ptr, dets_bstride, count_ptr):
+        step["filter"] = dict(min_score=float(min_score), cap=int(cap), dets=dets_ptr, dets_bstride=int(dets_bstride), count=count_ptr)
+
     def read_flat(self, ref):
         self.alloc.sync()
         return np.array(self.alloc.to_numpy(self.alloc.view_f32(self._phys[ref.buf], (self.B,) + tuple(ref.shape))))
```

New measurement: 1016 (median of 2 runs). No clear change (+0.0%).
